# ecker-lab/TreeLearn

Hardware: AMD Instinct MI355X
Metric: Mpoints/sec through sparse U-Net fwd (0.1 m voxel, 40x40 m tile) (higher is better)
Workload: dtype bf16; 1 GPU; config2: single 40x40 m tile, voxel 0.1 m, 1890607 points/tile, 7-level 32-ch sparse U-Net fwd (30.1 M params, random init), 1 tile per GPU; points_per_tile=1890607, tiles_in_flight=4

## Files before the change

### include/treelearn_hip.h

```cpp
#ifndef TREELEARN_HIP_H
#define TREELEARN_HIP_H

#include <stdint.h>

#ifdef __cplusplus
extern "C" {
#endif

typedef void* tl_stream_t;

enum {
  TL_OK = 0,
  TL_ERR_ARG = -1,
  TL_ERR_LAUNCH = -2,
  TL_ERR_UNSUPPORTED = -3
};

enum { TL_F32 = 0, TL_BF16 = 1, TL_F16 = 2 };

int tl_version(void);
int tl_set_tuning(const char* key, int64_t value);
const char* tl_error_string(int code);


// ... 48 lines not shown
  int32_t* inv_packed;
} tl_level;

int tl_rulebooks_build(const tl_level* levels, int num_levels, int32_t* minus_one, int64_t minus_one_words,
                       const int32_t* pcoords, int64_t N, int64_t* v2p, tl_stream_t stream);

#define TL_BLK_HALO_MAX 126
typedef struct tl_blk {
  int32_t* o2n; int32_t* perm; int32_t* coords_new;
  int32_t* unit; int32_t* counter; int32_t* halo; uint32_t* lrb; int32_t* pmask;
  int64_t cap_units;
  int32_t halo_max;
  int32_t reserved;
  int32_t* nn;
} tl_blk;
int64_t tl_blk_ws_words(const int32_t dims[4]);
int tl_blk_build(const uint64_t* bitmap, const uint32_t* prefix, const int32_t dims[4], int64_t n, const tl_blk* out, uint32_t* ws,
                 int phases, tl_stream_t stream);

int tl_rulebook_compact(const int32_t* table, int64_t n, int32_t* compact, tl_stream_t stream);

typedef struct tl_conv_args {
  const void* in;        int64_t in_ld;
  const void* weight;
  const int32_t* table;
  int64_t n_out;         int64_t n_in;
  int32_t K;             int32_t Cin;     int32_t Cout;   int32_t dtype;
  const float* in_scale; const float* in_shift;  int32_t in_relu;  int32_t out_relu;
  const void* residual;  int64_t res_ld;
  const float* out_scale; const float* out_shift;
  void* out;             int64_t out_ld;
  void* out2; int64_t out2_ld; const float* out2_scale; const float* out2_shift; int32_t out2_relu;
  void* out3; int64_t out3_ld; const float* out3_scale; const float* out3_shift; int32_t out3_relu;
  const void* weight_frag;
  int32_t table_one_hot;
  const int32_t* table_compact;
  int32_t in_all_ones;
  int32_t epi_mode;
  double* red_part;
  int32_t* red_nparts;
  const void* bn_x;      int64_t bn_x_ld;
  const float* bn_mean;  const float* bn_rstd;  const float* bn_scale;  const float* bn_shift;  int32_t bn_relu;
  const int32_t* blk_unit; const int32_t* blk_counter; const int32_t* blk_halo; const uint32_t* blk_lrb; const int32_t* blk_pmask;
  const int32_t* table_scatter;
  const void* weight_x3;
} tl_conv_args;

#define TL_EPI_NONE 0
#define TL_EPI_STATS 1
#define TL_EPI_BN_BWD 2
int64_t tl_conv_red_parts(int64_t n_out);

int tl_conv_fwd(const tl_conv_args* args, tl_stream_t stream);

int tl_pack_weight(const float* w_ref, int Cout, int K, int Cin, void* w_packed, int dtype, tl_stream_t stream);
int64_t tl_pack_weight_x3_bytes(int Cout, int K, int Cin);
int tl_pack_weight_x3(const float* w_ref, int Cout, int K, int Cin, void* w_x3, tl_stream_t stream);
int tl_pack_weight_dgrad(const float* w_ref, int Cout, int K, int Cin, int flip, void* w_t, int dtype, tl_stream_t stream);
typedef struct tl_pack_desc {
  const float* src;
  void* dst;
  int32_t Cout, K, Cin, form;
} tl_pack_desc;
int tl_pack_weights_batch(const tl_pack_desc* descs, const int32_t* blocks, int64_t n_blocks, int dtype, tl_stream_t stream);
int tl_pack_weight_frag(const float* w_ref, int Cout, int K, int Cin, void* w_frag, int dtype, tl_stream_t stream);

int64_t tl_conv_wgrad_ws_floats(int64_t n_out, int K, int Cin, int Cout);
int tl_conv_wgrad(const void* x, int64_t x_ld, const void* gout, int64_t g_ld, int dtype, const int32_t* table, int64_t n_out,
                  int64_t n_in, int K, int Cin, int Cout, float* gw, float* ws, tl_stream_t stream);
int tl_conv_wgrad_ref(const void* x, int64_t x_ld, const void* gout, int64_t g_ld, int dtype, const int32_t* table, int64_t n_out,
                      int64_t n_in, int K, int Cin, int Cout, float* gw, float* ws, tl_stream_t stream);

int64_t tl_conv_wgrad_blk_ws_floats(void);
int tl_conv_wgrad_blk(const void* x, int64_t x_ld, const void* gout, int64_t g_ld, int dtype, const int32_t* blk_unit, const int32_t* blk_counter,
                      const int32_t* blk_halo, const uint32_t* blk_lrb, int64_t n, int Cin, int Cout, float* gw, int ref_layout, float* ws,
                      tl_stream_t stream);

int tl_head_mlp(const void* feats, int64_t feats_ld, int dtype, int C, const int64_t* v2p, int64_t N,
                const float* pro_scale, const float* pro_shift,
                const float* w1, const float* b1, const float* w2, const float* b2,
                float* backbone, float* logits, float* offsets, tl_stream_t stream);

int tl_affine_relu(const void* in, int64_t in_ld, void* out, int64_t out_ld, int64_t n, int C, int dtype,
                   const float* scale, const float* shift, int relu, tl_stream_t stream);

int64_t tl_bn_ws_doubles(int64_t n, int C);
int tl_bn_train_stats(const void* x, int64_t ld, int64_t n, int C, int dtype, const float* gamma, const float* beta, float eps,
                      float momentum, double* ws, float* mean, float* rstd, float* scale, float* shift, float* running_mean,
                      float* running_var, int64_t* num_batches_tracked, tl_stream_t stream);
int tl_bn_train_bwd(const void* x, int64_t ld, int x_dtype, const void* dy, int64_t dld, int dy_dtype, int64_t n, int C,
                    const float* mean, const float* rstd, const float* scale, const float* shift, int relu, double* ws,
                    float* dgamma, float* dbeta, void* dx, int64_t xld, const void* dx_add, int64_t dx_add_ld, tl_stream_t stream);

int tl_bn_train_finish(const double* part, int64_t nparts, int64_t n, int C, const float* gamma, const float* beta, float eps, float momentum, float* mean,
                       float* rstd, float* scale, float* shift, float* running_mean, float* running_var, int64_t* num_batches_tracked, tl_stream_t stream);
int tl_bn_train_bwd_from_parts(const void* x, int64_t ld, int x_dtype, const void* g, int64_t gld, int g_dtype, int64_t n, int C, const float* mean,
                               const float* rstd, const float* scale, const float* shift, const double* part, int64_t nparts, float* dgamma, float* dbeta,
                               void* dx, int64_t xld, const void* dx_add, int64_t dx_add_ld, tl_stream_t stream);

int tl_linear_small_f32(const void* x, int64_t x_ld, int dtype, const void* w, int Cin, int Cout, int64_t n, float* out, int64_t out_ld,
                        tl_stream_t stream);

int tl_gather_rows(const void* in, int64_t in_ld, int dtype, int C, int64_t n_rows, const int64_t* idx, int64_t N, void* out, int64_t out_ld, tl_stream_t stream);
int tl_scatter_add_rows(const void* g, int64_t g_ld, int dtype, int C, const int64_t* order, const int64_t* sorted_idx, int64_t N, int64_t n_rows, void* gin,
                        int64_t gin_ld, tl_stream_t stream);

// ... 159 lines not shown
```

### treelearn_amd/_hip.py

```python
import ctypes
import os

import torch

_HERE = os.path.dirname(os.path.abspath(__file__))
LIB_PATH = os.path.join(_HERE, "lib", "libtreelearn_hip.so")

TL_F32, TL_BF16, TL_F16 = 0, 1, 2
TL_OK, TL_ERR_ARG, TL_ERR_UNSUPPORTED = 0, -1, -3
TL_EPI_NONE, TL_EPI_STATS, TL_EPI_BN_BWD = 0, 1, 2
_c = ctypes
_vp, _i64, _i32, _f32 = _c.c_void_p, _c.c_int64, _c.c_int32, _c.c_float


class ConvArgs(_c.Structure):
    _fields_ = [
        ("in_", _vp), ("in_ld", _i64), ("weight", _vp), ("table", _vp),
        ("n_out", _i64), ("n_in", _i64), ("K", _i32), ("Cin", _i32), ("Cout", _i32), ("dtype", _i32),
        ("in_scale", _vp), ("in_shift", _vp), ("in_relu", _i32), ("out_relu", _i32),
        ("residual", _vp), ("res_ld", _i64), ("out_scale", _vp), ("out_shift", _vp),
        ("out", _vp), ("out_ld", _i64),
        ("out2", _vp), ("out2_ld", _i64), ("out2_scale", _vp), ("out2_shift", _vp), ("out2_relu", _i32),
        ("out3", _vp), ("out3_ld", _i64), ("out3_scale", _vp), ("out3_shift", _vp), ("out3_relu", _i32),
        ("weight_frag", _vp), ("table_one_hot", _i32), ("table_compact", _vp),
        ("in_all_ones", _i32), ("epi_mode", _i32), ("red_part", _vp), ("red_nparts", _c.POINTER(_i32)),
        ("bn_x", _vp), ("bn_x_ld", _i64), ("bn_mean", _vp), ("bn_rstd", _vp), ("bn_scale", _vp), ("bn_shift", _vp), ("bn_relu", _i32),
        ("blk_unit", _vp), ("blk_counter", _vp), ("blk_halo", _vp), ("blk_lrb", _vp), ("blk_pmask", _vp), ("table_scatter", _vp),
        ("weight_x3", _vp),
    ]


class TileBox(_c.Structure):
    _fields_ = [("outer", _c.c_float * 4), ("inner", _c.c_double * 4), ("center", _c.c_double * 2), ("half_inner", _c.c_float)]


class Level(_c.Structure):
    _fields_ = [("dims", _c.c_int32 * 4), ("n", _c.c_int64), ("bitmap", _c.c_void_p), ("prefix", _c.c_void_p), ("coords", _c.c_void_p),
                ("nbr", _c.c_void_p), ("compact", _c.c_void_p), ("child", _c.c_void_p), ("parent", _c.c_void_p), ("inv", _c.c_void_p),
                ("o2n", _c.c_void_p), ("inv_packed", _c.c_void_p)]


class Blk(_c.Structure):
    _fields_ = [("o2n", _vp), ("perm", _vp), ("coords_new", _vp), ("unit", _vp), ("counter", _vp), ("halo", _vp), ("lrb", _vp), ("pmask", _vp),
                ("cap_units", _i64), ("halo_max", _i32), ("reserved", _i32), ("nn", _vp)]


class HdbGrid(_c.Structure):
    _fields_ = [("lo", _c.c_double * 2), ("h", _c.c_double), ("levels", _c.c_int32), ("reserved", _c.c_int32)]


TL_MAX_LEVELS = 8
TL_ERR_ARENA, TL_ERR_REACH_ZERO, TL_ERR_EXTENT, TL_ERR_BLK = -4, -5, -6, -7


class Affine(_c.Structure):
    _fields_ = [("scale", _vp), ("shift", _vp)]


class Weight(_c.Structure):
    _fields_ = [("w", _vp), ("frag", _vp), ("K", _i32), ("Cout", _i32), ("Cin", _i32), ("reserved", _i32), ("x3", _vp)]


class ResDesc(_c.Structure):
    _fields_ = [("bn0", Affine), ("w1", Weight), ("bn3", Affine), ("w2", Weight), ("w1x1", Weight), ("w1_half", Weight * 2)]


class UBlockDesc(_c.Structure):
    _fields_ = [("C", _i32), ("deeper", _i32), ("blocks", ResDesc * 2), ("bn_down", Affine), ("wd", Weight), ("bn_up", Affine), ("wu", Weight),
                ("tail", ResDesc * 2), ("bn_cat_l", Affine), ("bn_cat_r", Affine)]


class NetDesc(_c.Structure):
    _fields_ = [("dtype", _i32), ("num_levels", _i32), ("voxel_size", _f32), ("has_shape", _i32), ("spatial_shape", _i32 * 3), ("blocked", _i32),
                ("in_channels", _i32), ("use_coords", _i32), ("use_feats", _i32), ("max_points_per_voxel", _i32), ("reserved0", _i32),
                ("w_in", Weight), ("u", UBlockDesc * TL_MAX_LEVELS), ("out_bn", Affine),
                ("head_w1", _vp), ("head_b1", _vp), ("head_w2", _vp), ("head_b2", _vp)]


class LaunchRec(_c.Structure):
    _fields_ = [("level", _i32), ("kind", _i32), ("K", _i32), ("Cin", _i32), ("Cout", _i32), ("residual", _i32), ("esize", _i32), ("split_part", _i32),
                ("split_cin", _i32), ("in_prologue", _i32), ("n_out", _i64), ("n_in", _i64), ("ms", _f32)]


class ForwardArgs(_c.Structure):
    _fields_ = [("xyz", _vp), ("batch_ids", _vp), ("N", _i64), ("B", _i32), ("reserved", _i32), ("point_feats", _vp), ("arena", _vp), ("arena_bytes", _i64),
                ("backbone", _vp), ("logits", _vp), ("offsets", _vp), ("side_stream", _vp), ("needed_bytes", _i64),
                ("level_n", _i64 * TL_MAX_LEVELS), ("blocked_used", _i32), ("launches", _i32)]


_I4 = _i32 * 4
_I3 = _i32 * 3

PROTOTYPES = {
    "tl_version": (_i32, []),
    "tl_error_string": (_c.c_char_p, [_i32]),
    "tl_set_tuning": (_i32, [_c.c_char_p, _i64]),
    "tl_voxel_point_coords": (_i32, [_vp, _vp, _i64, _i32, _f32, _vp, _vp, _vp, _vp]),
    "tl_voxel_point_coords_one": (_i32, [_vp, _vp, _i64, _f32, _vp, _vp, _vp, _c.POINTER(_i32), _vp]),
    "tl_bitmap_from_points": (_i32, [_vp, _i64, _I4, _vp, _vp]),
    "tl_bitmap_down": (_i32, [_vp, _I4, _I3, _vp, _I4, _vp]),
    "tl_scan_ws_words": (_i64, [_i64]),
    "tl_bitmap_scan": (_i32, [_vp, _i64, _vp, _vp, _vp, _vp]),
    "tl_expand_coords": (_i32, [_vp, _vp, _I4, _vp, _vp]),
    "tl_point_rank": (_i32, [_vp, _i64, _vp, _vp, _I4, _vp, _vp]),
    "tl_voxel_mean_feats": (_i32, [_vp, _i32, _vp, _i64, _i64, _i32, _vp, _vp, _vp]),
    "tl_voxel_feats": (_i32, [_vp, _vp, _i32, _vp, _i64, _i64, _i32, _i32, _i32, _i32, _vp, _vp, _vp]),
    "tl_rulebook_subm": (_i32, [_vp, _i64, _vp, _vp, _I4, _vp, _vp, _vp]),
    "tl_rulebook_down": (_i32, [_vp, _i64, _vp, _vp, _I4, _i64, _vp, _vp, _vp, _vp]),
    "tl_rulebook_compact": (_i32, [_vp, _i64, _vp, _vp]),
    "tl_pyramid_ws_words": (_i64, [_I4, _i32, _c.POINTER(_i64)]),
    "tl_pyramid_build": (_i32, [_vp, _i64, _I4, _I3, _i32, _vp, _vp, _vp, _vp, _vp]),
    "tl_rulebooks_build": (_i32, [_c.POINTER(Level), _i32, _vp, _i64, _vp, _i64, _vp, _vp]),
    "tl_blk_ws_words": (_i64, [_I4]),
    "tl_blk_build": (_i32, [_vp, _vp, _I4, _i64, _c.POINTER(Blk), _vp, _i32, _vp]),
    "tl_conv_fwd": (_i32, [_c.POINTER(ConvArgs), _vp]),
    "tl_conv_red_parts": (_i64, [_i64]),
    "tl_exec_create": (_vp, []),
    "tl_exec_destroy": (None, [_vp]),
    "tl_forward": (_i32, [_vp, _c.POINTER(NetDesc), _c.POINTER(ForwardArgs), _vp]),
    "tl_exec_check": (_i32, [_vp]),
    "tl_exec_profile": (_i32, [_vp, _i32]),
    "tl_exec_profile_read": (_i32, [_vp, _c.POINTER(LaunchRec), _i32]),
    "tl_bn_train_finish": (_i32, [_vp, _i64, _i64, _i32, _vp, _vp, _f32, _f32, _vp, _vp, _vp, _vp, _vp, _vp, _vp, _vp]),
    "tl_bn_train_bwd_from_parts": (_i32, [_vp, _i64, _i32, _vp, _i64, _i32, _i64, _i32, _vp, _vp, _vp, _vp, _vp, _i64, _vp, _vp, _vp, _i64, _vp, _i64, _vp]),
    "tl_pack_weight": (_i32, [_vp, _i32, _i32, _i32, _vp, _i32, _vp]),
    "tl_pack_weight_x3": (_i32, [_vp, _i32, _i32, _i32, _vp, _vp]),
    "tl_pack_weight_x3_bytes": (_i64, [_i32, _i32, _i32]),
    "tl_pack_weight_frag": (_i32, [_vp, _i32, _i32, _i32, _vp, _i32, _vp]),
    "tl_pack_weights_batch": (_i32, [_vp, _vp, _i64, _i32, _vp]),
    "tl_pack_weight_dgrad": (_i32, [_vp, _i32, _i32, _i32, _i32, _vp, _i32, _vp]),
    "tl_conv_wgrad_ws_floats": (_i64, [_i64, _i32, _i32, _i32]),
    "tl_conv_wgrad": (_i32, [_vp, _i64, _vp, _i64, _i32, _vp, _i64, _i64, _i32, _i32, _i32, _vp, _vp, _vp]),
    "tl_conv_wgrad_ref": (_i32, [_vp, _i64, _vp, _i64, _i32, _vp, _i64, _i64, _i32, _i32, _i32, _vp, _vp, _vp]),
    "tl_conv_wgrad_blk_ws_floats": (_i64, []),
    "tl_conv_wgrad_blk": (_i32, [_vp, _i64, _vp, _i64, _i32, _vp, _vp, _vp, _vp, _i64, _i32, _i32, _vp, _i32, _vp, _vp]),
    "tl_head_mlp": (_i32, [_vp, _i64, _i32, _i32, _vp, _i64, _vp, _vp, _vp, _vp, _vp, _vp, _vp, _vp, _vp, _vp]),
    "tl_affine_relu": (_i32, [_vp, _i64, _vp, _i64, _i64, _i32, _i32, _vp, _vp, _i32, _vp]),
    "tl_bn_ws_doubles": (_i64, [_i64, _i32]),
    "tl_bn_train_stats": (_i32, [_vp, _i64, _i64, _i32, _i32, _vp, _vp, _f32, _f32, _vp, _vp, _vp, _vp, _vp, _vp, _vp, _vp, _vp]),
    "tl_bn_train_bwd": (_i32, [_vp, _i64, _i32, _vp, _i64, _i32, _i64, _i32, _vp, _vp, _vp, _vp, _i32, _vp, _vp, _vp, _vp, _i64, _vp, _i64, _vp]),
    "tl_linear_small_f32": (_i32, [_vp, _i64, _i32, _vp, _i32, _i32, _i64, _vp, _i64, _vp]),
    "tl_gather_rows": (_i32, [_vp, _i64, _i32, _i32, _i64, _vp, _i64, _vp, _i64, _vp]),
    "tl_scatter_add_rows": (_i32, [_vp, _i64, _i32, _i32, _vp, _vp, _i64, _i64, _vp, _i64, _vp]),
    "tl_compact_ws_words": (_i64, [_i64]),
    "tl_compact_rows": (_i32, [_vp, _i32, _vp, _i64, _vp, _vp, _vp, _vp]),
    "tl_tile_crop_ws_words": (_i64, [_i64]),
    "tl_tile_crop": (_i32, [_vp, _vp, _vp, _i64, _i32, _vp, _vp, _vp, _vp, _vp, _vp, _vp, _vp, _vp, _vp]),
    "tl_cell_keys": (_i32, [_vp, _i64, _c.c_double, _c.c_double, _vp, _i32, _vp, _vp, _vp]),
    "tl_downsample_ws_words": (_i64, [_i64]),
    "tl_downsample_reduce": (_i32, [_vp, _vp, _vp, _i64, _vp, _vp, _vp, _vp, _vp, _vp]),
    "tl_downsample_reduce_r64": (_i32, [_vp, _vp, _vp, _i64, _vp, _vp, _vp, _vp, _vp, _vp]),
    "tl_group_mean": (_i32, [_vp, _i64, _i32, _vp, _vp, _vp, _vp, _vp, _vp, _vp]),
    "tl_verticality": (_i32, [_vp, _vp, _i64, _c.c_double, _vp, _vp, _vp]),
    "tl_cluster_ws_bytes": (_i64, [_i64]),
    "tl_cluster_grid": (_i32, [_vp, _i64, _c.c_double, _vp, _vp, _vp, _vp]),
    "tl_hdbscan_ws_bytes": (_i64, [_i64]),
    "tl_hdbscan_mst": (_i32, [_vp, _i64, _i32, _vp, _vp, _vp, _vp, _vp, _vp]),
    "tl_hdbscan_labels_host": (_i32, [_vp, _vp, _vp, _i64, _i32, _vp]),
    "tl_hdbscan_prim_order_host": (_i32, [_vp, _vp, _vp, _i64, _vp, _vp, _vp]),
    "tl_hdbscan_grid_plan_ws_bytes": (_i64, []),
    "tl_hdbscan_grid_plan": (_i32, [_vp, _i64, _vp, _vp, _vp]),
    "tl_hdbscan_grid_ws_bytes": (_i64, [_i64, _vp]),
    "tl_hdbscan_grid_ws_bytes_k": (_i64, [_i64, _vp, _i32]),
    "tl_hdbscan_mst_grid": (_i32, [_vp, _i64, _i32, _vp, _vp, _vp, _vp, _vp, _vp, _vp]),
    "tl_knn_vote": (_i32, [_vp, _vp, _i64, _vp, _i64, _i32, _vp, _vp]),
    "tl_knn_vote_grid": (_i32, [_vp, _vp, _vp, _i64, _vp, _vp, _i64, _c.c_float * 3, _f32, _I3, _vp, _i64, _i32, _vp, _vp]),
    "tl_eval_contingency": (_i32, [_vp, _vp, _i64, _i64, _i64, _i64, _vp, _vp]),
    "tl_eval_partition": (_i32, [_vp, _vp, _vp, _i64, _vp, _vp, _i64, _vp, _vp, _i64, _vp, _i64, _vp, _i32, _i32, _vp, _vp, _vp, _vp, _vp]),
# ... 81 lines not shown
```

### treelearn_amd/csrc/tl_common.h

```cpp
#pragma once
#include <hip/hip_runtime.h>
#include <stdint.h>
#include <atomic>
#include "../../include/treelearn_hip.h"

#define TL_CHECK_LAUNCH()                                   \
  do {                                                      \
    if (hipGetLastError() != hipSuccess) return TL_ERR_LAUNCH; \
  } while (0)

static inline hipStream_t tl_s(tl_stream_t s) { return reinterpret_cast<hipStream_t>(s); }

struct TlAttrOnce {
  std::atomic<uint64_t> done[4];
};
static inline bool tl_lds_attr(TlAttrOnce& once, const void* kernel, int bytes) {
  int dev = 0;
  if (hipGetDevice(&dev) != hipSuccess) return false;
  std::atomic<uint64_t>& w = once.done[(dev >> 6) & 3];
  const uint64_t bit = 1ull << (dev & 63);
  if (w.load(std::memory_order_acquire) & bit) return true;
  if (hipFuncSetAttribute(kernel, hipFuncAttributeMaxDynamicSharedMemorySize, bytes) != hipSuccess) return false;
  w.fetch_or(bit, std::memory_order_release);
  return true;
}

static inline int64_t tl_cdiv(int64_t a, int64_t b) { return (a + b - 1) / b; }

static inline unsigned tl_grid(int64_t work_items, int block) {
  int64_t g = tl_cdiv(work_items, block);
  if (g < 1) g = 1;
  if (g > 256 * 16) g = 256 * 16;
  return (unsigned)g;
}

struct TlDims {
  int B, X, Y, Z, Zw;
};
static inline TlDims tl_dims(const int32_t d[4]) {
  TlDims r{d[0], d[1], d[2], d[3], (d[3] + 63) >> 6};
  return r;
}
__host__ __device__ static inline int64_t tl_nwords(const TlDims& d) { return (int64_t)d.B * d.X * d.Y * d.Zw; }

__device__ __forceinline__ int64_t tl_col_word(const TlDims& d, int b, int x, int y) {
  return (((int64_t)b * d.X + x) * d.Y + y) * d.Zw;
}

__device__ __forceinline__ int tl_rank_at(const uint64_t* __restrict__ bm, const uint32_t* __restrict__ pf,
                                          int64_t wc, int z) {
  const int64_t w = wc + (z >> 6);
  const uint64_t word = bm[w];
  const uint64_t bit = 1ull << (z & 63);
  if (!(word & bit)) return -1;
  return (int)(pf[w] + __popcll(word & (bit - 1)));
}

bool tl_conv_one_hot_direct_enabled(int64_t n_out);
```

### treelearn_amd/csrc/tl_conv.hip

```cpp
#include "tl_conv_internal.h"
#include <atomic>
#include <string.h>

namespace {

template <typename T>
__global__ void __launch_bounds__(256) k_conv_generic(ConvP p) {
  const T* in = (const T*)p.in; const T* w = (const T*)p.w; const T* res = (const T*)p.res;
  const int64_t total = p.n_out * p.Cout;
  for (int64_t t = (int64_t)blockIdx.x * blockDim.x + threadIdx.x; t < total; t += (int64_t)gridDim.x * blockDim.x) {
    const int64_t o = t / p.Cout; const int j = (int)(t % p.Cout);
    float acc = 0.f;
    for (int k = 0; k < p.K; ++k) {
      const int64_t idx = p.table ? (int64_t)p.table[(int64_t)k * p.n_out + o] : o;
      if (idx < 0) continue;
      const T* x = in + idx * p.in_ld;
      const T* wr = w + ((int64_t)k * p.Cout + j) * p.Cin;
      for (int c = 0; c < p.Cin; ++c) {
        float v = ld_elem(x + c);
        if (p.in_scale) v = fmaf(v, p.in_scale[c], p.in_shift[c]);
        if (p.in_relu) v = fmaxf(v, 0.f);
        if (sizeof(T) == 2) v = __bfloat162float(__float2bfloat16(v));
        acc = fmaf(v, ld_elem(wr + c), acc);
      }
// ... 93 lines not shown
    while (true) {
      int nk = k, nch = ch + 1;
      unsigned nmask = mask;
      if (nch == nchunk) { nch = 0; nmask = mask & (mask - 1); nk = nmask ? __builtin_ctz(nmask) : -1; }
      const bool more = nk >= 0;
      if (more) issue(nk, nch);

      const float* a = As + buf * TM * LDA + (wv * 32 + fi) * LDA + fh * 4;
      float4 af[4];
#pragma unroll
      for (int j = 0; j < 4; ++j) af[j] = *reinterpret_cast<const float4*>(a + 8 * j);
#pragma unroll
      for (int nb = 0; nb < NB; ++nb) {
        const float* b = Bs + buf * NB * 32 * LDA + (nb * 32 + fi) * LDA + fh * 4;
        float4 bf[4];
#pragma unroll
        for (int j = 0; j < 4; ++j) bf[j] = *reinterpret_cast<const float4*>(b + 8 * j);
#pragma unroll
        for (int j = 0; j < 4; ++j) {
          acc[nb] = __builtin_amdgcn_mfma_f32_32x32x2f32(af[j].x, bf[j].x, acc[nb], 0, 0, 0);
          acc[nb] = __builtin_amdgcn_mfma_f32_32x32x2f32(af[j].y, bf[j].y, acc[nb], 0, 0, 0);
          acc[nb] = __builtin_amdgcn_mfma_f32_32x32x2f32(af[j].z, bf[j].z, acc[nb], 0, 0, 0);
          acc[nb] = __builtin_amdgcn_mfma_f32_32x32x2f32(af[j].w, bf[j].w, acc[nb], 0, 0, 0);
        }
      }
      if (!more) break;
      stage(buf ^ 1, nch);
      __syncthreads();
      buf ^= 1; k = nk; ch = nch; mask = nmask;
    }
  }

  const float* res = (const float*)p.res;
  const int col = lane & 31;
#pragma unroll
  for (int nb = 0; nb < NB; ++nb) {
    const int j = nb * 32 + col;
#pragma unroll
    for (int r = 0; r < 16; ++r) {
      const int64_t row = r0 + wv * 32 + (r & 3) + 8 * (r >> 2) + 4 * (lane >> 5);
      if (row >= p.n_out) continue;
      float v = acc[nb][r];
      if (res) v += res[row * p.res_ld + j];
      epi_store1<false>(p.out, p.out_ld, p.out_scale, p.out_shift, p.out_relu, row, j, v);
      if (p.out2) epi_store1<false>(p.out2, p.out2_ld, p.out2_scale, p.out2_shift, p.out2_relu, row, j, v);
      if (p.out3) epi_store1<false>(p.out3, p.out3_ld, p.out3_scale, p.out3_shift, p.out3_relu, row, j, v);
    }
  }
}

template <int NB>
int launch_mfma_f32(const ConvP& p, hipStream_t s) {
  const size_t lds = (size_t)p.K * TM * 4 + 16 + 2 * (size_t)TM * LDA * 4 + 2 * (size_t)NB * 32 * LDA * 4;
  static TlAttrOnce attr_once;
  if (!tl_lds_attr(attr_once, reinterpret_cast<const void*>(&k_conv_mfma_f32<NB>), 160 * 1024)) return TL_ERR_LAUNCH;
  k_conv_mfma_f32<NB><<<p.nblk, 256, lds, s>>>(p);
  return hipGetLastError() == hipSuccess ? TL_OK : TL_ERR_LAUNCH;
}

__global__ void k_pack_weight(const float* __restrict__ w, int Cout, int K, int Cin, void* __restrict__ o, int dtype) {
  const int64_t total = (int64_t)Cout * K * Cin;
  for (int64_t t = (int64_t)blockIdx.x * blockDim.x + threadIdx.x; t < total; t += (int64_t)gridDim.x * blockDim.x) {
    const int c = (int)(t % Cin); const int64_t r = t / Cin; const int j = (int)(r % Cout); const int k = (int)(r / Cout);
    const float v = w[((int64_t)j * K + k) * Cin + c];
    if (dtype == TL_F32) reinterpret_cast<float*>(o)[t] = v;
    else if (dtype == TL_F16) reinterpret_cast<_Float16*>(o)[t] = (_Float16)v;
    else reinterpret_cast<__hip_bfloat16*>(o)[t] = __float2bfloat16(v);
  }
}

__global__ void k_pack_weight_x3(const float* __restrict__ w, int Cout, int K, int Cin, uint16_t* __restrict__ o) {
  const int un_all = Cin / 32, halves = Cin >= 256 ? 2 : 1, un = un_all / halves;
  const int64_t per_half = (int64_t)Cout * K * un * 64, total = per_half * halves;
  for (int64_t t0 = (int64_t)blockIdx.x * blockDim.x + threadIdx.x; t0 < total; t0 += (int64_t)gridDim.x * blockDim.x) {
    const int hf = (int)(t0 / per_half); const int64_t t = t0 - hf * per_half;
    const int e = (int)(t & 63); const int64_t r = t >> 6; const int c = (int)(r % un); const int64_t r2 = r / un;
    const int n = (int)(r2 % Cout); const int k = (int)(r2 / Cout);
    const int half = e >> 5, piece = (e & 31) >> 3, q = e & 7, J = piece >> 1, fh = piece & 1;
    const int ch = 32 * (c + hf * un) + 16 * J + (q < 4 ? 4 * fh + q : 8 + 4 * fh + (q - 4));
    const float v = w[((int64_t)n * K + k) * Cin + ch];
    const __hip_bfloat16 hi = __float2bfloat16(v);
    const __hip_bfloat16 lo = __float2bfloat16(v - __bfloat162float(hi));
    o[t0] = half ? __builtin_bit_cast(uint16_t, lo) : __builtin_bit_cast(uint16_t, hi);
    if (halves == 1 && Cout % 32 == 0) {
      const int j = half ? 2 + J : J;
      const int lane = (n & 31) + 32 * fh, cbt = n >> 5, CBt = Cout >> 5;
      o[total + ((((((int64_t)k * CBt + cbt) * un + c) * 4 + j) * 64 + lane) * 8) + q] = half ? __builtin_bit_cast(uint16_t, lo) : __builtin_bit_cast(uint16_t, hi);
    }
  }
}

__global__ void k_pack_weight_dgrad(const float* __restrict__ w, int Cout, int K, int Cin, int flip, void* __restrict__ o, int dtype) {
  const int64_t total = (int64_t)Cout * K * Cin;
  for (int64_t t = (int64_t)blockIdx.x * blockDim.x + threadIdx.x; t < total; t += (int64_t)gridDim.x * blockDim.x) {
    const int co = (int)(t % Cout); const int64_t r = t / Cout; const int ci = (int)(r % Cin); const int k = (int)(r / Cin);
    const float v = w[((int64_t)co * K + (flip ? K - 1 - k : k)) * Cin + ci];
    if (dtype == TL_F32) reinterpret_cast<float*>(o)[t] = v;
    else if (dtype == TL_F16) reinterpret_cast<_Float16*>(o)[t] = (_Float16)v;
    else reinterpret_cast<__hip_bfloat16*>(o)[t] = __float2bfloat16(v);
  }
}

__global__ void k_pack_weight_frag(const float* __restrict__ w, int Cout, int K, int Cin, void* __restrict__ o, int dtype) {
  const int EB = dtype == TL_F32 ? 4 : 2, J = 32 * EB / 32, EPV = 16 / EB;
  const int CB = Cout / 32, CH = Cin / 32;
  const int64_t nvec = (int64_t)K * CB * CH * J * 64;
// ... 68 lines not shown
    float x[8];
    typedef _Float16 hx2 __attribute__((ext_vector_type(2)));
    if constexpr (T16 == 1) {
      const u32x4 q4 = __builtin_nontemporal_load(reinterpret_cast<const u32x4*>((const uint16_t*)in + r * in_ld + c0));
#pragma unroll
      for (int q = 0; q < 4; ++q) { x[2 * q] = bf16_lo(q4[q]); x[2 * q + 1] = bf16_hi(q4[q]); }
    } else if constexpr (T16 == 2) {
      const u32x4 q4 = *reinterpret_cast<const u32x4*>((const uint16_t*)in + r * in_ld + c0);
      const uint32_t w0 = q4[0], w1 = q4[1], w2 = q4[2], w3 = q4[3];
      const uint32_t ws[4] = {w0, w1, w2, w3};
#pragma unroll
      for (int q = 0; q < 4; ++q) { const hx2 h = __builtin_bit_cast(hx2, ws[q]); x[2 * q] = (float)h[0]; x[2 * q + 1] = (float)h[1]; }
    } else {
      const f32x4* s4 = reinterpret_cast<const f32x4*>((const float*)in + r * in_ld + c0);
      const f32x4 a = __builtin_nontemporal_load(s4), b = __builtin_nontemporal_load(s4 + 1);
#pragma unroll
      for (int q = 0; q < 4; ++q) { x[q] = a[q]; x[q + 4] = b[q]; }
    }
#pragma unroll
    for (int q = 0; q < 8; ++q) { x[q] = fmaf(x[q], sc[q], sh[q]); if (relu) x[q] = fmaxf(x[q], 0.f); }
    if constexpr (T16 == 1) {
      u32x4 o;
#pragma unroll
      for (int q = 0; q < 4; ++q) o[q] = pack_bf16x2(x[2 * q], x[2 * q + 1]);
      *reinterpret_cast<u32x4*>((uint16_t*)out + r * out_ld + c0) = o;
    } else if constexpr (T16 == 2) {
      u32x4 o;
#pragma unroll
      for (int q = 0; q < 4; ++q) { const hx2 h = {(_Float16)x[2 * q], (_Float16)x[2 * q + 1]}; o[q] = __builtin_bit_cast(uint32_t, h); }
      *reinterpret_cast<u32x4*>((uint16_t*)out + r * out_ld + c0) = o;
    } else {
      f32x4* d = reinterpret_cast<f32x4*>((float*)out + r * out_ld + c0);
      d[0] = f32x4{x[0], x[1], x[2], x[3]}; d[1] = f32x4{x[4], x[5], x[6], x[7]};
    }
  }
}

}

static int64_t g_small_rows = kSmallRows;
extern int g_small_mode;
extern int g_wgrad_dense;
extern int64_t g_wgrad_dense_min_rows;
extern int g_wgrad_rows;
extern int g_wgrad_dma;
static int g_stream = 1;
static int g_streamq = 1;
static int g_streamq_x3 = 1;
static int g_direct = 1;
static int g_direct_oh = 1;
static int g_blk = 1;
static int g_up = 1;

bool tl_conv_one_hot_direct_enabled(int64_t n_out) { return g_direct && g_direct_oh && n_out > g_small_rows; }

extern "C" {

int tl_set_tuning(const char* key, int64_t value) {
  if (!key) return TL_ERR_ARG;
  if (!strcmp(key, "direct")) { g_direct = (int)value; return TL_OK; }
  if (!strcmp(key, "blk")) { g_blk = (int)value; return TL_OK; }
  if (!strcmp(key, "up")) { g_up = (int)value; return TL_OK; }
  if (!strcmp(key, "direct_oh")) { g_direct_oh = (int)value; return TL_OK; }
  if (!strcmp(key, "stream")) { g_stream = (int)value; return TL_OK; }
  if (!strcmp(key, "streamq")) { g_streamq = (int)value; return TL_OK; }
  if (!strcmp(key, "streamq_x3")) { if (value != 0 && value != 1) return TL_ERR_ARG; g_streamq_x3 = (int)value; return TL_OK; }
  if (!strcmp(key, "small_rows")) { g_small_rows = value; return TL_OK; }
  if (!strcmp(key, "small_mode")) { g_small_mode = (int)value; return TL_OK; }
  if (!strcmp(key, "wgrad_dense")) { g_wgrad_dense = (int)value; return TL_OK; }
  if (!strcmp(key, "wgrad_rows")) { g_wgrad_rows = (int)value; return TL_OK; }
  if (!strcmp(key, "wgrad_dma")) { g_wgrad_dma = (int)value; return TL_OK; }
  if (!strcmp(key, "wgrad_dense_min_rows")) { g_wgrad_dense_min_rows = value; return TL_OK; }
  return TL_ERR_ARG;
}

int tl_conv_fwd(const tl_conv_args* a, tl_stream_t stream) {
  if (!a || !a->in || !a->weight || !a->out || a->n_out <= 0 || a->K <= 0 || a->K > 27 || a->Cin <= 0 || a->Cout <= 0) return TL_ERR_ARG;
  const bool has_blk = a->blk_unit && a->blk_counter && a->blk_halo && a->blk_lrb && a->K == 27;
  if (!a->table && a->K != 1 && !has_blk && !(a->in_all_ones && a->blk_pmask)) return TL_ERR_ARG;
  if ((a->in_scale == nullptr) != (a->in_shift == nullptr)) return TL_ERR_ARG;
  if ((a->out_scale == nullptr) != (a->out_shift == nullptr)) return TL_ERR_ARG;
  if (a->dtype != TL_F32 && a->dtype != TL_BF16 && a->dtype != TL_F16) return TL_ERR_ARG;
  const bool f16 = a->dtype == TL_F16;
  const int dt = f16 ? TL_BF16 : a->dtype;
  const auto L_direct = f16 ? tl_launch_conv_direct_f16 : tl_launch_conv_direct;
  const auto L_ones27 = f16 ? tl_launch_conv_ones27_f16 : tl_launch_conv_ones27;
  const auto L_stream = f16 ? tl_launch_conv_stream_f16 : tl_launch_conv_stream;
  const auto L_streamq = f16 ? tl_launch_conv_streamq_f16 : tl_launch_conv_streamq;
  const auto L_small = f16 ? tl_launch_conv_small_f16 : tl_launch_conv_small;
  const auto L_tinycin = f16 ? tl_launch_conv_tinycin_f16 : tl_launch_conv_tinycin;
  const auto L_blk = f16 ? tl_launch_conv_blk_f16 : tl_launch_conv_blk;
  const auto L_up = f16 ? tl_launch_conv_up_f16 : tl_launch_conv_up;
  ConvP p;
  p.in = a->in; p.in_ld = a->in_ld; p.w = a->weight; p.w_frag = a->weight_frag;
  p.w_x3 = (a->dtype == TL_F32 && a->Cin % 32 == 0 && ((uintptr_t)a->weight_x3) % 16 == 0) ? a->weight_x3 : nullptr; p.table = a->table; p.ctab = (a->K == 27) ? a->table_compact : nullptr; p.n_out = a->n_out; p.n_in = a->n_in;
  p.K = a->K; p.Cin = a->Cin; p.Cout = a->Cout; p.in_scale = a->in_scale; p.in_shift = a->in_shift;
  p.in_relu = a->in_relu; p.out_relu = a->out_relu; p.res = a->residual; p.res_ld = a->res_ld;
  p.out_scale = a->out_scale; p.out_shift = a->out_shift; p.out = a->out; p.out_ld = a->out_ld;
  p.out2 = a->out2; p.out2_ld = a->out2_ld; p.out2_scale = a->out2_scale; p.out2_shift = a->out2_shift; p.out2_relu = a->out2_relu;
  p.out3 = a->out3; p.out3_ld = a->out3_ld; p.out3_scale = a->out3_scale; p.out3_shift = a->out3_shift; p.out3_relu = a->out3_relu;
  if ((a->out2_scale == nullptr) != (a->out2_shift == nullptr) || (a->out3_scale == nullptr) != (a->out3_shift == nullptr)) return TL_ERR_ARG;
  p.nblk = (int)tl_cdiv(a->n_out, TM);
  p.one_hot = a->table != nullptr ? a->table_one_hot : 0;
  p.blk_unit = has_blk ? a->blk_unit : nullptr; p.blk_counter = a->blk_counter; p.blk_halo = a->blk_halo; p.blk_lrb = a->blk_lrb;
  p.blk_pmask = a->K == 27 ? a->blk_pmask : nullptr;
  p.epi_mode = a->epi_mode; p.red_part = a->red_part; p.red_nparts = a->red_nparts; p.bn_x = a->bn_x; p.bn_x_ld = a->bn_x_ld;
  p.bn_mean = a->bn_mean; p.bn_rstd = a->bn_rstd; p.bn_scale = a->bn_scale; p.bn_shift = a->bn_shift; p.bn_relu = a->bn_relu;
  const bool train = a->epi_mode != TL_EPI_NONE;
  if (train) {
    if ((a->epi_mode != TL_EPI_STATS && a->epi_mode != TL_EPI_BN_BWD) || !a->red_part || ((uintptr_t)a->red_part) % 8) return TL_ERR_ARG;
    if (a->epi_mode == TL_EPI_BN_BWD) {
      if (!a->bn_x || !a->bn_mean || !a->bn_rstd || !a->bn_scale || !a->bn_shift) return TL_ERR_ARG;
      if (a->bn_x_ld % 8 || ((uintptr_t)a->bn_x) % 16 || ((uintptr_t)a->bn_mean) % 16 || ((uintptr_t)a->bn_rstd) % 16 || ((uintptr_t)a->bn_scale) % 16 ||
          ((uintptr_t)a->bn_shift) % 16)
        return TL_ERR_UNSUPPORTED;
    }
    if (a->red_nparts) *a->red_nparts = 0;
  }
  hipStream_t s = tl_s(stream);
  if (p.one_hot == 2) {
    const bool shape = a->K == 8 && a->Cin == 64 && a->Cout == 32 && !train && !a->in_scale && !a->in_relu && g_direct && g_direct_oh;
    if (!shape || !(dt == TL_BF16 || (dt == TL_F32 && p.w_x3))) return TL_ERR_UNSUPPORTED;
    return L_direct(p, dt, s);
  }
  const bool vec_ok = (a->in_ld % 8 == 0) && (((uintptr_t)a->in) % 16 == 0) && (((uintptr_t)a->weight) % 16 == 0);
  const bool out_vec = (a->out_ld % 8 == 0) && (((uintptr_t)a->out) % 16 == 0) &&
                       (!a->out2 || (a->out2_ld % 8 == 0 && ((uintptr_t)a->out2) % 16 == 0)) && (!a->out3 || (a->out3_ld % 8 == 0 && ((uintptr_t)a->out3) % 16 == 0));
  if (a->in_all_ones && !train && (dt == TL_BF16 || (dt == TL_F32 && !f16)) && out_vec && (g_direct || !a->table) && ((uintptr_t)a->weight) % 4 == 0 && !a->residual) {
    const int rc = L_ones27(p, dt, s);
    if (rc != TL_ERR_UNSUPPORTED) return rc;
  }
  if (has_blk && dt == TL_BF16 && g_blk && vec_ok && out_vec && (!a->residual || (a->res_ld % 8 == 0 && ((uintptr_t)a->residual) % 16 == 0)) &&
      (!a->out_scale || (((uintptr_t)a->out_scale) % 4 == 0 && ((uintptr_t)a->out_shift) % 4 == 0)) && (!a->in_relu || a->in_scale)) {
    const int rc = L_blk(p, s);
    if (rc != TL_ERR_UNSUPPORTED) return rc;
  }
  if (has_blk && a->dtype == TL_F32 && p.w_x3 && g_blk && !train) {
    const int rc = tl_launch_conv_blk_x3(p, s);
    if (rc != TL_ERR_UNSUPPORTED) return rc;
  }
  if (!a->table && a->K != 1) return TL_ERR_UNSUPPORTED;
  if (a->table_scatter && p.one_hot && g_up && !train && dt == TL_BF16 && vec_ok && out_vec &&
      (!a->out_scale || (((uintptr_t)a->out_scale) % 16 == 0 && ((uintptr_t)a->out_shift) % 16 == 0))) {
    const int rc = L_up(p, a->table_scatter, s);
    if (rc != TL_ERR_UNSUPPORTED) return rc;
  }
  if (dt == TL_BF16 && a->Cin == 4 && a->Cout == 32 && g_direct && out_vec && ((uintptr_t)a->in) % 8 == 0 && ((uintptr_t)a->weight) % 16 == 0 &&
      (!a->residual || (a->res_ld % 8 == 0 && ((uintptr_t)a->residual) % 16 == 0))) {
    const int rc = L_direct(p, TL_BF16, s);
    if (rc != TL_ERR_UNSUPPORTED) return rc;
  }
  if (!train && a->Cin <= 8 && a->Cout % 8 == 0 && a->Cout <= 64 && !a->in_scale && !a->in_relu && out_vec) return L_tinycin(p, dt, s);
  if (!train && vec_ok && a->n_out <= g_small_rows && a->Cin % 32 == 0 && a->Cout % 32 == 0) return L_small(p, dt, s);
  if (train && a->n_out <= g_small_rows) return TL_ERR_UNSUPPORTED;
  const bool aligned = (a->in_ld % 4 == 0) && (((uintptr_t)a->in) % 16 == 0) && (((uintptr_t)a->weight) % 16 == 0) &&
                       (!a->in_scale || (((uintptr_t)a->in_scale) % 16 == 0 && ((uintptr_t)a->in_shift) % 16 == 0));
  if (p.w_x3 && a->Cin >= 256) {
    if (dt == TL_F32 && !train && g_stream && aligned && out_vec && a->Cin % 64 == 0 && a->Cout % 32 == 0 && !a->in_scale && !a->in_relu && !a->residual &&
        !a->out2 && !a->out3 && a->n_out > g_small_rows && (!a->out_scale || (((uintptr_t)a->out_scale) % 16 == 0 && ((uintptr_t)a->out_shift) % 16 == 0))) {
      ConvP p1 = p;
      p1.Cin = a->Cin / 2; p1.out_scale = nullptr; p1.out_shift = nullptr; p1.out_relu = 0;
      const int rc1 = L_stream(p1, TL_F32, s);
      if (rc1 == TL_OK) {
        ConvP p2 = p;
        p2.Cin = a->Cin / 2; p2.in = static_cast<const float*>(a->in) + a->Cin / 2;
        p2.w_x3 = static_cast<const char*>(p.w_x3) + (size_t)a->K * a->Cout * (a->Cin / 2) * 4;
        p2.res = a->out; p2.res_ld = a->out_ld;
        return L_stream(p2, TL_F32, s);
      }
      if (rc1 != TL_ERR_UNSUPPORTED) return rc1;
    }
    p.w_x3 = nullptr;
  }
  if (dt == TL_F32 && aligned && out_vec && a->Cin % 32 == 0 && a->Cout % 32 == 0 && !a->in_scale && !a->in_relu &&
      (!a->residual || (a->res_ld % 4 == 0 && ((uintptr_t)a->residual) % 16 == 0)) &&
      (!a->out_scale || (((uintptr_t)a->out_scale) % 16 == 0 && ((uintptr_t)a->out_shift) % 16 == 0))) {
    if (g_direct) { const int rc = L_direct(p, TL_F32, s); if (rc != TL_ERR_UNSUPPORTED) return rc; }
    if (g_stream && g_streamq && g_streamq_x3 && p.w_x3 && !train && a->n_out > g_small_rows) {
      const int rc = tl_launch_conv_streamq_x3(p, s);
      if (rc != TL_ERR_UNSUPPORTED) return rc;
    }
    if (g_stream) { const int rc = L_stream(p, TL_F32, s); if (rc != TL_ERR_UNSUPPORTED) return rc; }
  }
  if (train && dt == TL_F32) return TL_ERR_UNSUPPORTED;
  if (dt == TL_F32 && !f16 && vec_ok && a->n_out <= 4 * g_small_rows && a->Cin % 32 == 0 && a->Cout % 32 == 0 && !a->in_scale && !a->in_relu)
    return L_small(p, dt, s);
  if (dt == TL_F32 && aligned && a->Cin % KC == 0 && a->Cout % 32 == 0 && a->Cout <= 224) {
    switch (a->Cout / 32) {
      case 1: return launch_mfma_f32<1>(p, s);
      case 2: return launch_mfma_f32<2>(p, s);
      case 3: return launch_mfma_f32<3>(p, s);
      case 4: return launch_mfma_f32<4>(p, s);
      case 5: return launch_mfma_f32<5>(p, s);
      case 6: return launch_mfma_f32<6>(p, s);
      case 7: return launch_mfma_f32<7>(p, s);
    }
  }
  if (dt == TL_BF16 && aligned && vec_ok && out_vec && a->Cin % 32 == 0 && a->Cout % 32 == 0 && a->Cout <= 224 &&
      (!a->residual || (a->res_ld % 8 == 0 && ((uintptr_t)a->residual) % 16 == 0)) &&
      (!a->out_scale || (((uintptr_t)a->out_scale) % 16 == 0 && ((uintptr_t)a->out_shift) % 16 == 0)))
  {
    if (p.one_hot && g_direct && g_direct_oh && a->K == 8 && a->Cin == 64 && a->Cout == 32) {
      const int rc = L_direct(p, TL_BF16, s);
      if (rc != TL_ERR_UNSUPPORTED) return rc;
    }
    if (p.one_hot && g_stream && a->K == 8) {
      const int rc = L_stream(p, TL_BF16, s);
      if (rc != TL_ERR_UNSUPPORTED) return rc;
    }
    if (g_direct) {
      const int rc = L_direct(p, TL_BF16, s);
      if (rc != TL_ERR_UNSUPPORTED) return rc;
    }
    if (g_stream && g_streamq) {
      const int rc = L_streamq(p, s);
      if (rc != TL_ERR_UNSUPPORTED) return rc;
    }
    if (g_stream) {
      const int rc = L_stream(p, TL_BF16, s);
      if (rc != TL_ERR_UNSUPPORTED) return rc;
    }
    if (train) return TL_ERR_UNSUPPORTED;
    return f16 ? tl_launch_conv_bf16_f16(p, s) : tl_launch_conv_bf16(p, s);
  }
  if (train || f16) return TL_ERR_UNSUPPORTED;
  {
    const int rc = tl_launch_conv_tinycout(p, dt, s);
    if (rc != TL_ERR_UNSUPPORTED) return rc;
  }
  const unsigned g = tl_grid(a->n_out * a->Cout, 256);
  if (dt == TL_F32) k_conv_generic<float><<<g, 256, 0, s>>>(p);
  else k_conv_generic<__hip_bfloat16><<<g, 256, 0, s>>>(p);
  TL_CHECK_LAUNCH();
  return TL_OK;
}

int64_t tl_conv_red_parts(int64_t n_out) {
  const int64_t a = tl_cdiv(n_out > 0 ? n_out : 1, 256);
  return a > 2048 ? a : 2048;
}

int tl_pack_weight(const float* w_ref, int Cout, int K, int Cin, void* w_packed, int dtype, tl_stream_t stream) {
  if (!w_ref || !w_packed || Cout <= 0 || K <= 0 || Cin <= 0 || (dtype != TL_F32 && dtype != TL_BF16 && dtype != TL_F16)) return TL_ERR_ARG;
  k_pack_weight<<<tl_grid((int64_t)Cout * K * Cin, 256), 256, 0, tl_s(stream)>>>(w_ref, Cout, K, Cin, w_packed, dtype);
  TL_CHECK_LAUNCH();
  return TL_OK;
}

int64_t tl_pack_weight_x3_bytes(int Cout, int K, int Cin) {
  if (Cout <= 0 || K <= 0 || Cin <= 0 || Cin % 32) return -1;
  const int64_t one = (int64_t)K * Cout * Cin * 4;
  return (Cin < 256 && Cout % 32 == 0) ? 2 * one : one;
}

int tl_pack_weight_x3(const float* w_ref, int Cout, int K, int Cin, void* w_x3, tl_stream_t stream) {
  if (!w_ref || !w_x3 || Cout <= 0 || K <= 0 || Cin <= 0 || Cin % 32) return TL_ERR_ARG;
  k_pack_weight_x3<<<tl_grid((int64_t)Cout * K * Cin * 2, 256), 256, 0, tl_s(stream)>>>(w_ref, Cout, K, Cin, reinterpret_cast<uint16_t*>(w_x3));
  TL_CHECK_LAUNCH();
  return TL_OK;
}

int tl_pack_weight_dgrad(const float* w_ref, int Cout, int K, int Cin, int flip, void* w_t, int dtype, tl_stream_t stream) {
  if (!w_ref || !w_t || Cout <= 0 || K <= 0 || Cin <= 0 || (dtype != TL_F32 && dtype != TL_BF16 && dtype != TL_F16)) return TL_ERR_ARG;
  k_pack_weight_dgrad<<<tl_grid((int64_t)Cout * K * Cin, 256), 256, 0, tl_s(stream)>>>(w_ref, Cout, K, Cin, flip, w_t, dtype);
  TL_CHECK_LAUNCH();
  return TL_OK;
}

int tl_pack_weights_batch(const tl_pack_desc* descs, const int32_t* blocks, int64_t n_blocks, int dtype, tl_stream_t stream) {
  if (!descs || !blocks || n_blocks <= 0 || n_blocks > 0x7FFFFFFF || (dtype != TL_F32 && dtype != TL_BF16 && dtype != TL_F16)) return TL_ERR_ARG;
  k_pack_batch<<<(unsigned)n_blocks, 256, 0, tl_s(stream)>>>(descs, reinterpret_cast<const int2*>(blocks), dtype);
  TL_CHECK_LAUNCH();
  return TL_OK;
}

int tl_pack_weight_frag(const float* w_ref, int Cout, int K, int Cin, void* w_frag, int dtype, tl_stream_t stream) {
  if (!w_ref || !w_frag || Cout <= 0 || K <= 0 || Cin <= 0 || Cout % 32 || Cin % 32 || (dtype != TL_F32 && dtype != TL_BF16 && dtype != TL_F16)) return TL_ERR_ARG;
  k_pack_weight_frag<<<tl_grid((int64_t)Cout * K * Cin / 8, 256), 256, 0, tl_s(stream)>>>(w_ref, Cout, K, Cin, w_frag, dtype);
  TL_CHECK_LAUNCH();
  return TL_OK;
}

int tl_affine_relu(const void* in, int64_t in_ld, void* out, int64_t out_ld, int64_t n, int C, int dtype, const float* scale,
                   const float* shift, int relu, tl_stream_t stream) {
  if (!in || !out || n <= 0 || C <= 0 || (scale == nullptr) != (shift == nullptr)) return TL_ERR_ARG;
  if ((dtype == TL_F32 || dtype == TL_BF16 || dtype == TL_F16) && C % 8 == 0 && in_ld % 8 == 0 && out_ld % 8 == 0 && ((uintptr_t)in) % 16 == 0 && ((uintptr_t)out) % 16 == 0) {
    const int vpr = C / 8;
// ... 20 lines not shown
```

### treelearn_amd/csrc/tl_conv_bf16.hip

```cpp
#include "tl_conv_internal.h"
#include <atomic>

namespace {

constexpr int TM = 128;

template <int NB, int U, int D, bool BUF>
__global__ void __launch_bounds__(256) k_conv_bf16(ConvP p) {
  constexpr int KCB = 32 * U;
  constexpr int PITCH = KCB * 2 + 16;
  constexpr int VPR = KCB / 8;
  constexpr int RPP = 256 / VPR;
  constexpr int APASS = TM / RPP;
  constexpr int BROWS = NB * 32;
  constexpr int BPASS = (BROWS + RPP - 1) / RPP;
  constexpr int EP = NB * 32 + 4;

  extern __shared__ __attribute__((aligned(16))) char smem[];
  int* idx_s = reinterpret_cast<int*>(smem);
  int* taps_s = idx_s + p.K * TM;
  float* scale_s = reinterpret_cast<float*>(taps_s + 32);
  float* shift_s = scale_s + p.Cin;
  char* As = reinterpret_cast<char*>(shift_s + p.Cin);
  char* Bs = As + 2 * TM * PITCH;
// ... 154 lines not shown
#pragma unroll
    for (int d = 0; d < D; ++d) {
      stage(buf, ra[d], rb[d], vmask[d], chs[d]);
      __syncthreads();
      issue(ra[d], rb[d], vmask[d], chs[d]);
      compute(buf);
      buf ^= 1;
    }
  }
  const int rem = nsteps - s;
#pragma unroll
  for (int d = 0; d < D - 1; ++d) {
    if (d < rem) {
      stage(buf, ra[d], rb[d], vmask[d], chs[d]);
      __syncthreads();
      compute(buf);
      buf ^= 1;
    }
  }

  __syncthreads();
  float* ew = Es + wv * 32 * EP;
#pragma unroll
  for (int nb = 0; nb < NB; ++nb)
#pragma unroll
    for (int r = 0; r < 16; ++r) ew[((r & 3) + 8 * (r >> 2) + 4 * fh) * EP + nb * 32 + fi] = acc[nb][r];
  __syncthreads();
  constexpr int VROW = NB * 4;
  const char* res = (const char*)p.res;
  for (int e = lane; e < 32 * VROW; e += 64) {
    const int rr = e / VROW, cvv = e % VROW;
    const int64_t row = r0 + wv * 32 + rr;
    if (row >= p.n_out) continue;
    const f32x4 v0 = *reinterpret_cast<const f32x4*>(ew + rr * EP + cvv * 8), v1 = *reinterpret_cast<const f32x4*>(ew + rr * EP + cvv * 8 + 4);
    float v[8] = {v0[0], v0[1], v0[2], v0[3], v1[0], v1[1], v1[2], v1[3]};
    if (res) {
      const u32x4 rv = *reinterpret_cast<const u32x4*>(res + (row * p.res_ld + cvv * 8) * 2);
#pragma unroll
      for (int q = 0; q < 4; ++q) { v[2 * q] += bf16_lo(rv[q]); v[2 * q + 1] += bf16_hi(rv[q]); }
    }
    epi_store8<true>(p.out, p.out_ld, p.out_scale, p.out_shift, p.out_relu, row, cvv * 8, v);
    if (p.out2) epi_store8<true>(p.out2, p.out2_ld, p.out2_scale, p.out2_shift, p.out2_relu, row, cvv * 8, v);
    if (p.out3) epi_store8<true>(p.out3, p.out3_ld, p.out3_scale, p.out3_shift, p.out3_relu, row, cvv * 8, v);
  }
}

template <int NB, int U, int D, bool BUF>
int launch_b(const ConvP& p, hipStream_t s) {
  constexpr int PITCH = 32 * U * 2 + 16;
  const size_t main_b = 2 * (size_t)TM * PITCH + 2 * (size_t)NB * 32 * PITCH;
  const size_t epi_b = 4 * (size_t)32 * (NB * 32 + 4) * 4;
  const size_t lds = (size_t)p.K * TM * 4 + 128 + (size_t)p.Cin * 8 + (main_b > epi_b ? main_b : epi_b);
  if (lds > 160 * 1024) return TL_ERR_UNSUPPORTED;
  static TlAttrOnce attr_once;
  if (!tl_lds_attr(attr_once, reinterpret_cast<const void*>(&k_conv_bf16<NB, U, D, BUF>), 160 * 1024)) return TL_ERR_LAUNCH;
  k_conv_bf16<NB, U, D, BUF><<<p.nblk, 256, lds, s>>>(p);
  return hipGetLastError() == hipSuccess ? TL_OK : TL_ERR_LAUNCH;
}

template <int NB, int U, int D>
int launch(const ConvP& p, hipStream_t s) {
  const int64_t ld_b = p.in_ld * 2, in_bytes = (p.n_in - 1) * ld_b + (int64_t)p.Cin * 2;
  const bool buf = in_bytes > 0 && in_bytes + 2 * ld_b < 0xFFFFFFFFll;
  return buf ? launch_b<NB, U, D, true>(p, s) : launch_b<NB, U, D, false>(p, s);
}

}

int tl_launch_conv_bf16(const ConvP& p, hipStream_t s) {
  switch (p.Cout / 32) {
    case 1: return launch<1, 2, 2>(p, s);
    case 2: return launch<2, 2, 2>(p, s);
    case 3: return launch<3, 2, 2>(p, s);
    case 4: return launch<4, 2, 2>(p, s);
    case 5: return launch<5, 2, 2>(p, s);
    case 6: return launch<6, 2, 2>(p, s);
    case 7: return launch<7, 2, 2>(p, s);
  }
  return TL_ERR_UNSUPPORTED;
}
```

### treelearn_amd/csrc/tl_conv_blk.hip

```cpp
#include "tl_conv_internal.h"
#include <atomic>

namespace {

typedef __attribute__((address_space(3))) void* lds_ptr;
static __device__ __forceinline__ u32x4 lds_r128(unsigned a) { u32x4 v; asm volatile("ds_read_b128 %0, %1" : "=v"(v) : "v"(a)); return v; }
#define TL_LGKM(N) asm volatile("s_waitcnt lgkmcnt(%0)" ::"n"(N) : "memory")
#define TL_KEEP(x) asm volatile("" : "+v"(x))
typedef int i32x4 __attribute__((ext_vector_type(4)));
static __device__ __forceinline__ i32x4 s_load4(const void* ptr) { i32x4 v; asm volatile("s_load_dwordx4 %0, %1, 0x0" : "=s"(v) : "s"(ptr)); return v; }
#define TL_SWAIT(d) asm volatile("s_waitcnt lgkmcnt(0)" : "+s"(d) : : "memory")

constexpr int WS_B = 27 * 32 * 64;
constexpr int AFF_B = 4 * 2 * 32 * 4;
constexpr int STAGE_B = 192 * 64;
constexpr int HCH = 8;
struct RbRow { u32x4 a, b; uint32_t c; };
static __device__ __forceinline__ uint32_t rb_word(const RbRow& r, int w) { return w < 4 ? r.a[w] : (w < 8 ? r.b[w - 4] : r.c); }

typedef float f32x2 __attribute__((ext_vector_type(2)));
typedef short s16x2 __attribute__((ext_vector_type(2)));

template <int W, bool RES, int NV, bool TR = false, bool PRO = false>
__global__ void __launch_bounds__(W * 64) k_conv_blk(ConvP p) {
// ... 318 lines not shown
        for (int q = 0; q < 4; ++q) {
          sc[q] = __uint_as_float(s0[q]); sc[q + 4] = __uint_as_float(s1[q]);
          sh[q] = __uint_as_float(h0[q]); sh[q + 4] = __uint_as_float(h1[q]);
        }
      }
#pragma unroll
      for (int it = 0; it < 4; ++it) {
        float z[8];
#pragma unroll
        for (int q = 0; q < 8; ++q) z[q] = y[it][q];
        if (aff_on[v]) {
#pragma unroll
          for (int q = 0; q < 8; ++q) z[q] = fmaf(z[q], sc[q], sh[q]);
        }
        if (relu_on[v]) {
#pragma unroll
          for (int q = 0; q < 8; ++q) z[q] = fmaxf(z[q], 0.f);
        }
        const u32x4 o = {pack_bf16x2(z[0], z[1]), pack_bf16x2(z[2], z[3]), pack_bf16x2(z[4], z[5]), pack_bf16x2(z[6], z[7])};
        const int rr_ = (lane >> 2) + 16 * it;
        const unsigned off = rr_ < nown ? (unsigned)(row0 + rr_) * o_ldb[v] + (unsigned)((lane & 3) * 16) : 0xFFFFFFFFu;
        __builtin_amdgcn_raw_buffer_store_b128(__builtin_bit_cast(__attribute__((__vector_size__(4 * sizeof(unsigned)))) unsigned, o), ro[v], (int)off, 0, 0);
      }
    }
    }
    dc = d1; d1 = d2; d2 = desc_fin(d3r, u + 3 * nw);
  }
  if constexpr (TR) {
    double* Ds = reinterpret_cast<double*>(smem + WS_B + AFF_B + W * STAGE_B);
    double d0[8], d1_[8];
#pragma unroll
    for (int q = 0; q < 8; ++q) { d0[q] = (double)ts0[q]; d1_[q] = (double)ts1[q]; }
#pragma unroll
    for (int off = 4; off < 64; off <<= 1)
#pragma unroll
      for (int q = 0; q < 8; ++q) { d0[q] += __shfl_xor(d0[q], off, 64); d1_[q] += __shfl_xor(d1_[q], off, 64); }
    if (lane < 4) {
#pragma unroll
      for (int q = 0; q < 8; ++q) { Ds[(wv * 2 + 0) * 32 + lane * 8 + q] = d0[q]; Ds[(wv * 2 + 1) * 32 + lane * 8 + q] = d1_[q]; }
    }
    __syncthreads();
    if (tid < 64) {
      double t = 0.0;
      for (int w = 0; w < W; ++w) t += Ds[(w * 2 + (tid >> 5)) * 32 + (tid & 31)];
      p.red_part[(int64_t)blockIdx.x * 64 + tid] = t;
    }
  }
}

template <int W, bool RES, int NV, bool TR = false, bool PRO = false>
int launch_blk(const ConvP& p, hipStream_t s) {
  constexpr size_t lds = (size_t)WS_B + AFF_B + (size_t)W * STAGE_B + (TR ? (size_t)W * 2 * 32 * 8 : 0);
  static_assert(lds <= 160 * 1024, "LDS budget");
  static TlAttrOnce attr_once;
  if (!tl_lds_attr(attr_once, reinterpret_cast<const void*>(&k_conv_blk<W, RES, NV, TR, PRO>), 160 * 1024)) return TL_ERR_LAUNCH;
  k_conv_blk<W, RES, NV, TR, PRO><<<256, W * 64, lds, s>>>(p);
  if (TR && p.red_nparts) *p.red_nparts = 256;
  return hipGetLastError() == hipSuccess ? TL_OK : TL_ERR_LAUNCH;
}

}

int tl_launch_conv_blk(const ConvP& p, hipStream_t s) {
  if (!p.blk_unit || !p.blk_counter || !p.blk_halo || !p.blk_lrb) return TL_ERR_UNSUPPORTED;
  if (p.K != 27 || p.Cin != 32 || p.Cout != 32 || p.n_in != p.n_out) return TL_ERR_UNSUPPORTED;
  const bool pro = p.in_scale || p.in_relu;
  if (p.n_out >= (1 << 25)) return TL_ERR_UNSUPPORTED;
  auto big = [&](int64_t ld) { return (p.n_out - 1) * ld * 2 + 64 >= 0x7FFFFFFFll * 2; };
  if (big(p.in_ld) || big(p.out_ld) || (p.out2 && big(p.out2_ld)) || (p.out3 && big(p.out3_ld)) || (p.res && big(p.res_ld))) return TL_ERR_UNSUPPORTED;
  if (p.out3 && !p.out2) return TL_ERR_UNSUPPORTED;
  if (p.epi_mode != TL_EPI_NONE) {
    if (p.out2 || p.out_scale || p.out_relu || p.out_ld % 8 || ((uintptr_t)p.out) % 16) return TL_ERR_UNSUPPORTED;
    if (pro && p.epi_mode != TL_EPI_STATS) return TL_ERR_UNSUPPORTED;
    return pro ? launch_blk<8, false, 1, true, true>(p, s) : launch_blk<8, false, 1, true>(p, s);
  }
  const int nv = p.out3 ? 3 : p.out2 ? 2 : 1;
  if (pro) {
    if (nv != 1) return TL_ERR_UNSUPPORTED;
    return p.res ? launch_blk<8, true, 1, false, true>(p, s) : launch_blk<8, false, 1, false, true>(p, s);
  }
  if (p.res) {
    switch (nv) {
      case 1: return launch_blk<8, true, 1>(p, s);
      case 2: return launch_blk<8, true, 2>(p, s);
      default: return launch_blk<8, true, 3>(p, s);
    }
  }
  switch (nv) {
    case 1: return launch_blk<8, false, 1>(p, s);
    case 2: return launch_blk<8, false, 2>(p, s);
    default: return launch_blk<8, false, 3>(p, s);
  }
}
```

### treelearn_amd/csrc/tl_conv_blk_x3.hip

```cpp
#include "tl_conv_internal.h"
#include <atomic>

namespace {

typedef __attribute__((address_space(3))) void* lds_ptr;
static __device__ __forceinline__ u32x4 lds_r128(unsigned a) { u32x4 v; asm volatile("ds_read_b128 %0, %1" : "=v"(v) : "v"(a)); return v; }
#define TL_LGKM(N) asm volatile("s_waitcnt lgkmcnt(%0)" ::"n"(N) : "memory")
#define TL_KEEP(x) asm volatile("" : "+v"(x))
typedef int i32x4 __attribute__((ext_vector_type(4)));
typedef uint32_t u32x2 __attribute__((ext_vector_type(2)));
static __device__ __forceinline__ i32x4 s_load4(const void* ptr) { i32x4 v; asm volatile("s_load_dwordx4 %0, %1, 0x0" : "=s"(v) : "s"(ptr)); return v; }
#define TL_SWAIT(d) asm volatile("s_waitcnt lgkmcnt(0)" : "+s"(d) : : "memory")

constexpr int WS_B = 27 * 32 * 64;
constexpr int AFF_B = 4 * 2 * 32 * 4;
constexpr int STAGE_B = 192 * 64;
constexpr int HCH = 8;
struct RbRow { u32x4 a, b; uint32_t c; };
static __device__ __forceinline__ uint32_t rb_word(const RbRow& r, int w) { return w < 4 ? r.a[w] : (w < 8 ? r.b[w - 4] : r.c); }

struct X3P {
  int slice;
  int part;
  int chunk, nchunks;
// ... 264 lines not shown
    }
    if constexpr (RES) {
#pragma unroll
      for (int it = 0; it < 4; ++it) {
        TL_KEEP(rres[it][0]); TL_KEEP(rres[it][1]);
#pragma unroll
        for (int q = 0; q < 4; ++q) { y[it][q] += __uint_as_float(rres[it][0][q]); y[it][q + 4] += __uint_as_float(rres[it][1][q]); }
      }
    }
    stage_unit(d1, hcur);
#pragma unroll
    for (int v = 0; v < NV; ++v) {
      float sc[8], sh[8];
      if (aff_on[v]) {
        const u32x4 s0 = lds_r128(aff_a + (unsigned)(v * 256)), s1 = lds_r128(aff_a + (unsigned)(v * 256 + 16));
        const u32x4 h0 = lds_r128(aff_a + (unsigned)(v * 256 + 128)), h1 = lds_r128(aff_a + (unsigned)(v * 256 + 144));
        TL_LGKM(0);
#pragma unroll
        for (int q = 0; q < 4; ++q) {
          sc[q] = __uint_as_float(s0[q]); sc[q + 4] = __uint_as_float(s1[q]);
          sh[q] = __uint_as_float(h0[q]); sh[q + 4] = __uint_as_float(h1[q]);
        }
      }
#pragma unroll
      for (int it = 0; it < 4; ++it) {
        float z[8];
#pragma unroll
        for (int q = 0; q < 8; ++q) z[q] = y[it][q];
        if (aff_on[v]) {
#pragma unroll
          for (int q = 0; q < 8; ++q) z[q] = fmaf(z[q], sc[q], sh[q]);
        }
        if (relu_on[v]) {
#pragma unroll
          for (int q = 0; q < 8; ++q) z[q] = fmaxf(z[q], 0.f);
        }
        typedef __attribute__((__vector_size__(4 * sizeof(unsigned)))) unsigned uv4;
        const uv4 o0 = {__float_as_uint(z[0]), __float_as_uint(z[1]), __float_as_uint(z[2]), __float_as_uint(z[3])};
        const uv4 o1 = {__float_as_uint(z[4]), __float_as_uint(z[5]), __float_as_uint(z[6]), __float_as_uint(z[7])};
        const int rr_ = (lane >> 2) + 16 * it;
        const unsigned off = rr_ < nown ? (unsigned)(row0 + rr_) * o_ldb[v] + (unsigned)((lane & 3) * 32) : 0xFFFFFFFFu;
        __builtin_amdgcn_raw_buffer_store_b128(o0, ro[v], (int)off, 0, 0);
        __builtin_amdgcn_raw_buffer_store_b128(o1, ro[v], (int)(off == 0xFFFFFFFFu ? off : off + 16u), 0, 0);
      }
    }
    dc = d1; d1 = d2; d2 = desc_fin(d3r, u + 3 * nw);
  }
}

template <int W, bool RES, int NV>
int launch_x3(const ConvP& p, const X3P& xp, hipStream_t s) {
  constexpr size_t lds = (size_t)WS_B + AFF_B + (size_t)W * STAGE_B;
  static_assert(lds <= 160 * 1024, "LDS budget");
  static TlAttrOnce attr_once;
  if (!tl_lds_attr(attr_once, reinterpret_cast<const void*>(&k_conv_blk_x3<W, RES, NV>), 160 * 1024)) return TL_ERR_LAUNCH;
  k_conv_blk_x3<W, RES, NV><<<256, W * 64, lds, s>>>(p, xp);
  return hipGetLastError() == hipSuccess ? TL_OK : TL_ERR_LAUNCH;
}

}

int tl_launch_conv_blk_x3(const ConvP& p, hipStream_t s) {
  if (!p.blk_unit || !p.blk_counter || !p.blk_halo || !p.blk_lrb || !p.w_x3) return TL_ERR_UNSUPPORTED;
  if (p.K != 27 || p.Cin != 32 || p.Cout != 32 || p.n_in != p.n_out || p.epi_mode != TL_EPI_NONE || p.out3) return TL_ERR_UNSUPPORTED;
  if (p.n_out >= (1 << 25)) return TL_ERR_UNSUPPORTED;
  if (p.in_relu && !p.in_scale) return TL_ERR_UNSUPPORTED;
  auto big = [&](int64_t ld) { return (p.n_out - 1) * ld * 4 + 128 >= 0x7FFFFFFFll * 2; };
  if (big(p.in_ld) || big(p.out_ld) || (p.out2 && big(p.out2_ld)) || (p.res && big(p.res_ld))) return TL_ERR_UNSUPPORTED;
  auto al16 = [](const void* q, int64_t ld) { return ((uintptr_t)q) % 16 == 0 && ld % 4 == 0; };
  if (!al16(p.in, p.in_ld) || !al16(p.out, p.out_ld) || (p.out2 && !al16(p.out2, p.out2_ld)) || (p.res && !al16(p.res, p.res_ld)) || ((uintptr_t)p.w_x3) % 16) return TL_ERR_UNSUPPORTED;
  ConvP a = p;
  a.res = nullptr; a.res_ld = 0; a.out_scale = a.out_shift = nullptr; a.out_relu = 0; a.out2 = nullptr; a.out2_scale = a.out2_shift = nullptr; a.out2_relu = 0;
  ConvP b = p;
  b.in = static_cast<const float*>(p.in) + 16;
  if (p.in_scale) { b.in_scale = p.in_scale + 16; b.in_shift = p.in_shift + 16; }
  const int rc = launch_x3<8, false, 1>(a, X3P{0, 0, 0, 1}, s);
  if (rc != TL_OK) return rc;
  const X3P xb{1, 1, 0, 1};
  if (p.res) return p.out2 ? launch_x3<8, true, 2>(b, xb, s) : launch_x3<8, true, 1>(b, xb, s);
  return p.out2 ? launch_x3<8, false, 2>(b, xb, s) : launch_x3<8, false, 1>(b, xb, s);
}
```

### treelearn_amd/csrc/tl_conv_direct.hip

```cpp
#include "tl_conv_internal.h"
#include <atomic>

namespace {


template <bool BF16, int K, int NB, int UN, int G, int WAVES, bool CT = false, bool TR = false, bool OH = false, bool X3 = false>
__global__ void __launch_bounds__(WAVES * 64) k_conv_direct(ConvP p, int ntiles, int walk) {
  static_assert(!X3 || (!BF16 && !TR), "the split-bf16 contraction: fp32 rows, inference");
  constexpr int EB = BF16 ? 2 : 4;
  constexpr int UB = 32 * EB;
  constexpr int NJ = UB / 32;
  constexpr int SLOTS = UB / 16;
  constexpr int COUT = NB * 32;
  constexpr int NG = (K + G - 1) / G;
  constexpr int EP = COUT + 4;
  extern __shared__ __attribute__((aligned(16))) char smem[];
  char* Ws = smem;
  float* Es = reinterpret_cast<float*>(smem + (size_t)K * UN * COUT * UB);
  double* Ds = reinterpret_cast<double*>(smem + (size_t)K * UN * COUT * UB + (size_t)WAVES * 32 * EP * 4);

  const int tid = threadIdx.x, lane = tid & 63, wv = tid >> 6;
  const int fi = lane & 31, fh = lane >> 5;
  auto swz_of = [](int n) { return BF16 ? ((n >> 2) & 3) : ((n >> 1) & 7); };

// ... 362 lines not shown
      p.red_part[(int64_t)blockIdx.x * 64 + e] = t;
    }
  }
}

template <bool BF16>
__global__ void __launch_bounds__(256) k_conv_ones27(ConvP p) {
  __shared__ __attribute__((aligned(16))) float S[27][32];
  for (int e = threadIdx.x; e < 27 * 32; e += 256) {
    float t = 0.f;
    if constexpr (BF16) {
      const uint16_t* w = (const uint16_t*)p.w;
      for (int c = 0; c < p.Cin; ++c) t += bf16_lo((uint32_t)w[(int64_t)e * p.Cin + c]);
    } else {
      const float* w = (const float*)p.w;
      for (int c = 0; c < p.Cin; ++c) t += w[(int64_t)e * p.Cin + c];
    }
    S[e >> 5][e & 31] = t;
  }
  __syncthreads();
  const int32_t* mask = p.blk_pmask ? p.blk_pmask : p.ctab + (int64_t)9 * p.n_out;
  const int64_t total = p.n_out * 4;
  for (int64_t t = (int64_t)blockIdx.x * 256 + threadIdx.x; t < total; t += (int64_t)gridDim.x * 256) {
    const int64_t row = t >> 2; const int c0 = (int)(t & 3) * 8;
    uint32_t m = (uint32_t)mask[row];
    float v[8] = {0.f, 0.f, 0.f, 0.f, 0.f, 0.f, 0.f, 0.f};
    while (m) {
      const int k = __builtin_ctz(m); m &= m - 1;
      const f32x4 a = *reinterpret_cast<const f32x4*>(&S[k][c0]), b = *reinterpret_cast<const f32x4*>(&S[k][c0 + 4]);
#pragma unroll
      for (int q = 0; q < 4; ++q) { v[q] += a[q]; v[q + 4] += b[q]; }
    }
    epi_views8<BF16>(p, row, c0, v);
  }
}

template <bool BF16, int K, int NB, int UN, int G, int WAVES, bool CT = false, bool TR = false, bool OH = false, bool X3 = false>
int launch(const ConvP& p_, hipStream_t s) {
  ConvP p = p_;
  if constexpr (X3) {
    if (p.epi_mode != TL_EPI_NONE) return TL_ERR_UNSUPPORTED;
    p.w = p.w_x3;
  }
  if constexpr (!TR && BF16) {
    if (p.epi_mode != TL_EPI_NONE) return launch<BF16, K, NB, UN, G, WAVES, CT, true, OH>(p, s);
  } else if constexpr (!TR) {
    if (p.epi_mode != TL_EPI_NONE) return TL_ERR_UNSUPPORTED;
  }
  if constexpr (TR && NB >= 3) return TL_ERR_UNSUPPORTED;
  else {
  constexpr int UB = BF16 ? 64 : 128;
  const size_t lds = (size_t)K * UN * NB * 32 * UB + (size_t)WAVES * 32 * (NB * 32 + 4) * 4 + (TR ? (size_t)WAVES * 2 * NB * 32 * 8 : 0);
  if (lds > 160 * 1024) return TL_ERR_UNSUPPORTED;
  static TlAttrOnce attr_once;
  if (!tl_lds_attr(attr_once, reinterpret_cast<const void*>(&k_conv_direct<BF16, K, NB, UN, G, WAVES, CT, TR, OH, X3>), 160 * 1024)) return TL_ERR_LAUNCH;
  const int ntiles = (int)tl_cdiv(p.n_out, 32);
  const int per_cu = (int)((160 * 1024) / lds) < 1 ? 1 : (int)((160 * 1024) / lds);
  int grid = 256 * (per_cu > 2 ? 2 : per_cu);
  const int need = (int)tl_cdiv(ntiles, WAVES);
  if (grid > need) grid = need;
  k_conv_direct<BF16, K, NB, UN, G, WAVES, CT, TR, OH, X3><<<grid, WAVES * 64, lds, s>>>(p, ntiles, 0);
  if (p.red_nparts) *p.red_nparts = grid;
  return hipGetLastError() == hipSuccess ? TL_OK : TL_ERR_LAUNCH;
  }
}

template <bool BF16, int K, int G>
int dispatch(const ConvP& p, hipStream_t s) {
  const int nb = p.Cout / 32, un = p.Cin / 32;
  const size_t wbytes = (size_t)K * p.Cout * p.Cin * (BF16 ? 2 : 4);
  if constexpr (BF16 && K == 27) {
    if (p.ctab && nb == 1 && un == 1) return launch<true, 27, 1, 1, G, 16, true>(p, s);
    if (p.ctab && nb == 1 && un == 2) return launch<true, 27, 1, 2, G, 8, true>(p, s);
  }
  if constexpr (BF16 && K == 8) {
    if (p.one_hot && nb == 1 && un == 2) return launch<true, 8, 1, 2, G, 16, false, false, true>(p, s);
  }
  if constexpr (BF16 && K == 1) {
    if (nb == 2 && un == 4) return launch<true, 1, 2, 4, 1, 16>(p, s);
    if (nb == 3 && un == 6) return launch<true, 1, 3, 6, 1, 8>(p, s);
    if (nb == 4 && un == 8) return launch<true, 1, 4, 8, 1, 8>(p, s);
  }
  if constexpr (!BF16 && K == 1) {
    if (nb == 2 && un == 4 && p.epi_mode == TL_EPI_NONE) {
      if (p.w_x3) return launch<false, 1, 2, 4, 1, 8, false, false, false, true>(p, s);
      return launch<false, 1, 2, 4, 1, 8>(p, s);
    }
  }
  if constexpr (!BF16 && K == 8) {
    if (p.one_hot && p.w_x3 && p.epi_mode == TL_EPI_NONE && nb == 1 && un == 2) return launch<false, 8, 1, 2, G, 12, false, false, true, true>(p, s);
  }
#define TL_D(NB_, UN_)                                                                                               \
  if (nb == NB_ && un == UN_) {                                                                                      \
    if constexpr (BF16) return wbytes <= 64 * 1024 ? launch<true, K, NB_, UN_, G, 16>(p, s) : launch<true, K, NB_, UN_, G, 8>(p, s); \
    else {                                                                                                           \
      if (p.w_x3 && p.epi_mode == TL_EPI_NONE)        \
        return launch<false, K, NB_, UN_, (G > 2 ? 2 : G), (K == 27 && NB_ == 1 && UN_ == 1 ? 11 : 8), false, false, false, true>(p, s);         \
      return launch<false, K, NB_, UN_, (G > 2 ? 2 : G), 8>(p, s);                                                   \
    }                                                                                                                \
  }
  TL_D(1, 1) TL_D(1, 2) TL_D(2, 1) TL_D(2, 2) TL_D(2, 3) TL_D(3, 2) TL_D(1, 3) TL_D(3, 1)
#undef TL_D
  return TL_ERR_UNSUPPORTED;
}

}

int tl_launch_conv_ones27(const ConvP& p, int dtype, hipStream_t s) {
  if (p.K != 27 || p.Cout != 32 || (!p.ctab && !p.blk_pmask) || p.Cin <= 0 || p.Cin > 64 || p.in_scale || p.in_relu || p.epi_mode != TL_EPI_NONE) return TL_ERR_UNSUPPORTED;
  if (dtype == TL_BF16) k_conv_ones27<true><<<tl_grid(p.n_out * 4, 256), 256, 0, s>>>(p);
  else k_conv_ones27<false><<<tl_grid(p.n_out * 4, 256), 256, 0, s>>>(p);
  return hipGetLastError() == hipSuccess ? TL_OK : TL_ERR_LAUNCH;
}


int tl_launch_conv_direct(const ConvP& p, int dtype, hipStream_t s) {
  if (p.in_scale || p.in_relu) return TL_ERR_UNSUPPORTED;
  if (p.one_hot == 2 && !(p.K == 8 && p.Cin == 64 && p.Cout == 32 && p.epi_mode == TL_EPI_NONE && (dtype == TL_BF16 || p.w_x3))) return TL_ERR_UNSUPPORTED;
  const int eb = dtype == TL_BF16 ? 2 : 4;
  if (dtype == TL_BF16 && p.Cin == 4 && p.Cout == 32 && p.K <= 28 && p.table && p.in_ld % 4 == 0 && (int64_t)p.n_in * p.in_ld * 2 < 0xFFFF0000ll) {
    const int ntiles = (int)tl_cdiv(p.n_out, 32);
    int grid = (int)tl_cdiv(ntiles, 8);
    if (grid > 2048) grid = 2048;
    if (p.epi_mode != TL_EPI_NONE) {
      if (p.ctab && p.K == 27) k_conv_in4<8, true, true><<<grid, 512, 0, s>>>(p, ntiles);
      else k_conv_in4<8, false, true><<<grid, 512, 0, s>>>(p, ntiles);
    } else if (p.ctab && p.K == 27) k_conv_in4<8, true><<<grid, 512, 0, s>>>(p, ntiles);
    else k_conv_in4<8><<<grid, 512, 0, s>>>(p, ntiles);
    if (p.red_nparts) *p.red_nparts = grid;
    return hipGetLastError() == hipSuccess ? TL_OK : TL_ERR_LAUNCH;
  }
  if (p.Cin % 32 || p.Cout % 32) return TL_ERR_UNSUPPORTED;
  const int64_t ld_b = p.in_ld * eb, in_bytes = (p.n_in - 1) * ld_b + (int64_t)p.Cin * eb;
  if (!(in_bytes > 0 && in_bytes + 2 * ld_b < 0xFFFFFFFFll)) return TL_ERR_UNSUPPORTED;
  if ((size_t)p.K * p.Cout * p.Cin * eb > 112 * 1024) return TL_ERR_UNSUPPORTED;
  if (dtype == TL_BF16) {
    switch (p.K) {
      case 27: return dispatch<true, 27, 3>(p, s);
      case 8: return dispatch<true, 8, 2>(p, s);
      case 1: return dispatch<true, 1, 1>(p, s);
    }
  } else {
    switch (p.K) {
      case 27: return dispatch<false, 27, 3>(p, s);
      case 8: return dispatch<false, 8, 2>(p, s);
      case 1: return dispatch<false, 1, 1>(p, s);
    }
  }
  return TL_ERR_UNSUPPORTED;
}
```

### treelearn_amd/csrc/tl_conv_internal.h

```cpp
#pragma once
#include "tl_common.h"
#include <hip/hip_bf16.h>
#include "tl_half.h"

#ifdef TL_F16_BUILD
#define tl_launch_conv_direct tl_launch_conv_direct_f16
#define tl_launch_conv_ones27 tl_launch_conv_ones27_f16
#define tl_launch_conv_stream tl_launch_conv_stream_f16
#define tl_launch_conv_streamq tl_launch_conv_streamq_f16
#define tl_launch_conv_small tl_launch_conv_small_f16
#define tl_launch_conv_tinycin tl_launch_conv_tinycin_f16
#define tl_launch_conv_bf16 tl_launch_conv_bf16_f16
#define tl_launch_conv_blk tl_launch_conv_blk_f16
#define tl_launch_conv_up tl_launch_conv_up_f16
#define g_small_mode g_small_mode_f16
#endif

typedef float f32x16 __attribute__((ext_vector_type(16)));
typedef float f32x4 __attribute__((ext_vector_type(4)));
typedef uint32_t u32x4 __attribute__((ext_vector_type(4)));
typedef short s16x8 __attribute__((ext_vector_type(8)));

struct ConvP {
  const void* in; int64_t in_ld;
  const void* w;
  const void* w_frag;
  const void* w_x3;
  const int32_t* table;
  const int32_t* ctab;
  int64_t n_out, n_in;
  int K, Cin, Cout;
  const float* in_scale; const float* in_shift; int in_relu, out_relu;
  const void* res; int64_t res_ld;
  const float* out_scale; const float* out_shift;
  void* out; int64_t out_ld;
  void* out2; int64_t out2_ld; const float* out2_scale; const float* out2_shift; int out2_relu;
  void* out3; int64_t out3_ld; const float* out3_scale; const float* out3_shift; int out3_relu;
  int nblk;
  int epi_mode;
  double* red_part;
  int32_t* red_nparts;
  const void* bn_x; int64_t bn_x_ld;
  const float* bn_mean; const float* bn_rstd; const float* bn_scale; const float* bn_shift; int bn_relu;
  int one_hot;
  const int32_t* blk_unit; const int32_t* blk_counter; const int32_t* blk_halo; const uint32_t* blk_lrb; const int32_t* blk_pmask;
};

static __device__ __forceinline__ float ld_elem(const float* p) { return *p; }
static __device__ __forceinline__ float ld_elem(const __hip_bfloat16* p) { return h16_lo((uint32_t)*reinterpret_cast<const uint16_t*>(p)); }
static __device__ __forceinline__ void st_elem(float* p, float v) { *p = v; }
static __device__ __forceinline__ float ld_elem(const _Float16* p) { return (float)*p; }
static __device__ __forceinline__ void st_elem(_Float16* p, float v) { *p = (_Float16)v; }
static __device__ __forceinline__ void st_elem(__hip_bfloat16* p, float v) { *reinterpret_cast<uint16_t*>(p) = (uint16_t)(h16_pack2(v, 0.f) & 0xFFFFu); }

static __device__ __forceinline__ int xcd_tile(int b, int n) {
  const int q = n >> 3, r = n & 7, x = b & 7, i = b >> 3;
  return (x < r ? x * (q + 1) : r * (q + 1) + (x - r) * q) + i;
}


typedef __bf16 bf16x8 __attribute__((ext_vector_type(8)));

static __device__ __forceinline__ uint32_t pack_bf16x2(float lo, float hi) { return h16_pack2(lo, hi); }
static __device__ __forceinline__ float bf16_lo(uint32_t u) { return h16_lo(u); }
static __device__ __forceinline__ float bf16_hi(uint32_t u) { return h16_hi(u); }

template <bool BF16>
static __device__ __forceinline__ void epi_store1(void* base, int64_t ld, const float* sc, const float* sh, int relu, int64_t row, int j, float y) {
  if (sc) y = fmaf(y, sc[j], sh[j]);
  if (relu) y = fmaxf(y, 0.f);
  if constexpr (BF16) ((uint16_t*)base)[row * ld + j] = (uint16_t)(pack_bf16x2(y, 0.f) & 0xFFFFu);
  else ((float*)base)[row * ld + j] = y;
}
template <bool BF16>
static __device__ __forceinline__ void epi_store8(void* base, int64_t ld, const float* sc, const float* sh, int relu, int64_t row, int c0, const float (&y)[8]) {
  float v[8];
#pragma unroll
  for (int q = 0; q < 8; ++q) v[q] = y[q];
  if (sc) {
    const f32x4 a0 = *reinterpret_cast<const f32x4*>(sc + c0), a1 = *reinterpret_cast<const f32x4*>(sc + c0 + 4);
    const f32x4 b0 = *reinterpret_cast<const f32x4*>(sh + c0), b1 = *reinterpret_cast<const f32x4*>(sh + c0 + 4);
#pragma unroll
    for (int q = 0; q < 4; ++q) { v[q] = fmaf(v[q], a0[q], b0[q]); v[q + 4] = fmaf(v[q + 4], a1[q], b1[q]); }
  }
  if (relu) {
#pragma unroll
    for (int q = 0; q < 8; ++q) v[q] = fmaxf(v[q], 0.f);
  }
  if constexpr (BF16) {
    u32x4 o;
#pragma unroll
    for (int q = 0; q < 4; ++q) o[q] = pack_bf16x2(v[2 * q], v[2 * q + 1]);
    *reinterpret_cast<u32x4*>((uint16_t*)base + row * ld + c0) = o;
  } else {
    f32x4* d = reinterpret_cast<f32x4*>((float*)base + row * ld + c0);
    d[0] = f32x4{v[0], v[1], v[2], v[3]}; d[1] = f32x4{v[4], v[5], v[6], v[7]};
  }
}

// ... 228 lines not shown
```

### treelearn_amd/csrc/tl_conv_small.hip

```cpp
#include "tl_conv_internal.h"

namespace {

template <bool BF16, int NBB, int WV, bool FR, bool X3 = false>
__global__ void __launch_bounds__(WV * 64) k_conv_small(ConvP p, int ncolblk) {
  static_assert(!X3 || !BF16, "split-bf16: fp32 rows, weights in their own layout (FR: its fragment-order second copy)");
  constexpr int EB = BF16 ? 2 : 4, UB = 32 * EB, NJ = UB / 32;
  constexpr int PF = 4;
  constexpr int KMAX = 27;
  __shared__ float red[WV][16][64];
  __shared__ int Is[KMAX * 32];
  const int tid = threadIdx.x, lane = tid & 63, wv = tid >> 6;
  const int rt = blockIdx.x / ncolblk, cb = blockIdx.x % ncolblk;
  const int fi = lane & 31, fh = lane >> 5;
  const int col0 = cb * NBB * 32;
  const int nchunk = p.Cin / 32;
  const int nsteps = p.K * nchunk;
  const bool pro = p.in_scale != nullptr || p.in_relu;

  for (int e = tid; e < p.K * 32; e += WV * 64) {
    const int64_t r = (int64_t)rt * 32 + (e & 31);
    Is[e] = r < p.n_out ? (p.table ? p.table[(int64_t)(e >> 5) * p.n_out + r] : (int)r) : -1;
  }

// ... 112 lines not shown
      if constexpr (BF16) {
        if (p.res) v += bf16_lo((uint32_t)((const uint16_t*)p.res)[orow * p.res_ld + j]);
      } else {
        if (p.res) v += ((const float*)p.res)[orow * p.res_ld + j];
      }
      epi_store1<BF16>(p.out, p.out_ld, p.out_scale, p.out_shift, p.out_relu, orow, j, v);
      if (p.out2) epi_store1<BF16>(p.out2, p.out2_ld, p.out2_scale, p.out2_shift, p.out2_relu, orow, j, v);
      if (p.out3) epi_store1<BF16>(p.out3, p.out3_ld, p.out3_scale, p.out3_shift, p.out3_relu, orow, j, v);
    }
  }
}

template <typename T, int CIN>
__global__ void __launch_bounds__(256) k_conv_tinycin(ConvP p) {
  extern __shared__ __attribute__((aligned(16))) float wsh[];
  const T* w = (const T*)p.w; const T* in = (const T*)p.in; const T* res = (const T*)p.res;
  for (int e = threadIdx.x; e < p.K * CIN * p.Cout; e += 256) {
    const int j = e % p.Cout, c = (e / p.Cout) % CIN, k = e / (p.Cout * CIN);
    wsh[e] = ld_elem(w + ((int64_t)k * p.Cout + j) * p.Cin + c);
  }
  __syncthreads();
  const int ngrp = p.Cout / 8;
  const int64_t total = p.n_out * ngrp;
  for (int64_t t = (int64_t)blockIdx.x * 256 + threadIdx.x; t < total; t += (int64_t)gridDim.x * 256) {
    const int64_t o = t / ngrp; const int j0 = (int)(t % ngrp) * 8;
    float acc[8] = {0.f, 0.f, 0.f, 0.f, 0.f, 0.f, 0.f, 0.f};
    for (int k = 0; k < p.K; ++k) {
      const int64_t idx = p.table ? (int64_t)p.table[(int64_t)k * p.n_out + o] : o;
      if (idx < 0) continue;
      float x[CIN];
#pragma unroll
      for (int c = 0; c < CIN; ++c) x[c] = ld_elem(in + idx * p.in_ld + c);
#pragma unroll
      for (int c = 0; c < CIN; ++c) {
        const float4 w0 = *reinterpret_cast<const float4*>(&wsh[(k * CIN + c) * p.Cout + j0]);
        const float4 w1 = *reinterpret_cast<const float4*>(&wsh[(k * CIN + c) * p.Cout + j0 + 4]);
        acc[0] = fmaf(x[c], w0.x, acc[0]); acc[1] = fmaf(x[c], w0.y, acc[1]); acc[2] = fmaf(x[c], w0.z, acc[2]); acc[3] = fmaf(x[c], w0.w, acc[3]);
        acc[4] = fmaf(x[c], w1.x, acc[4]); acc[5] = fmaf(x[c], w1.y, acc[5]); acc[6] = fmaf(x[c], w1.z, acc[6]); acc[7] = fmaf(x[c], w1.w, acc[7]);
      }
    }
#pragma unroll
    for (int q = 0; q < 8; ++q) if (res) acc[q] += ld_elem(res + o * p.res_ld + j0 + q);
    constexpr bool BF = sizeof(T) == 2;
    epi_store8<BF>(p.out, p.out_ld, p.out_scale, p.out_shift, p.out_relu, o, j0, acc);
    if (p.out2) epi_store8<BF>(p.out2, p.out2_ld, p.out2_scale, p.out2_shift, p.out2_relu, o, j0, acc);
    if (p.out3) epi_store8<BF>(p.out3, p.out3_ld, p.out3_scale, p.out3_shift, p.out3_relu, o, j0, acc);
  }
}

template <typename T>
int launch_tiny(const ConvP& p, hipStream_t s) {
  const size_t lds = (size_t)p.K * p.Cin * p.Cout * 4;
  const unsigned g = tl_grid(p.n_out * (p.Cout / 8), 256);
  switch (p.Cin) {
    case 1: k_conv_tinycin<T, 1><<<g, 256, lds, s>>>(p); break;
    case 2: k_conv_tinycin<T, 2><<<g, 256, lds, s>>>(p); break;
    case 3: k_conv_tinycin<T, 3><<<g, 256, lds, s>>>(p); break;
    case 4: k_conv_tinycin<T, 4><<<g, 256, lds, s>>>(p); break;
    case 5: k_conv_tinycin<T, 5><<<g, 256, lds, s>>>(p); break;
    case 6: k_conv_tinycin<T, 6><<<g, 256, lds, s>>>(p); break;
    case 7: k_conv_tinycin<T, 7><<<g, 256, lds, s>>>(p); break;
    case 8: k_conv_tinycin<T, 8><<<g, 256, lds, s>>>(p); break;
    default: return TL_ERR_UNSUPPORTED;
  }
  return hipGetLastError() == hipSuccess ? TL_OK : TL_ERR_LAUNCH;
}

}

int g_small_mode = 0;

int tl_launch_conv_small(const ConvP& p, int dtype, hipStream_t s) {
  const int nrt = (int)tl_cdiv(p.n_out, 32);
  const bool eight = g_small_mode == 2 || (g_small_mode == 0 && nrt * (p.Cout / 32) <= 512 && p.K * (p.Cin / 32) >= 32);
  const int cbt = p.Cout / 32;
  const bool full = g_small_mode == 0 && dtype == TL_BF16 && (cbt == 3 || cbt == 5 || cbt == 7) && nrt >= 128 && p.w_frag != nullptr &&
                    ((uintptr_t)p.w_frag) % 16 == 0;
  if (full) {
    switch (cbt) {
      case 3: k_conv_small<true, 3, 4, true><<<nrt, 256, 0, s>>>(p, 1); break;
      case 5: k_conv_small<true, 5, 4, true><<<nrt, 256, 0, s>>>(p, 1); break;
      case 7: k_conv_small<true, 7, 4, true><<<nrt, 256, 0, s>>>(p, 1); break;
    }
    return hipGetLastError() == hipSuccess ? TL_OK : TL_ERR_LAUNCH;
  }
  const bool two = !eight && (p.Cout % 64 == 0);
  const int ncb = p.Cout / (two ? 64 : 32);
  const unsigned g = (unsigned)(nrt * ncb);
#define TL_SMALL(BF_, FR_)                                                                   \
  do {                                                                                         \
    if (eight) k_conv_small<BF_, 1, 8, FR_><<<g, 512, 0, s>>>(p, ncb);                         \
    else if (two) k_conv_small<BF_, 2, 4, FR_><<<g, 256, 0, s>>>(p, ncb);                      \
    else k_conv_small<BF_, 1, 4, FR_><<<g, 256, 0, s>>>(p, ncb);                               \
  } while (0)
  const bool fr = p.w_frag != nullptr && ((uintptr_t)p.w_frag) % 16 == 0 && g_small_mode != 3;
  const bool x3 = dtype == TL_F32 && p.w_x3 != nullptr && p.Cin < 256 && !p.in_scale && !p.in_relu;
  if (dtype == TL_BF16) { if (fr) TL_SMALL(true, true); else TL_SMALL(true, false); }
  else if (x3 && g_small_mode != 3 && p.Cout % 32 == 0) {
    if (eight) k_conv_small<false, 1, 8, true, true><<<g, 512, 0, s>>>(p, ncb);
    else if (two) k_conv_small<false, 2, 4, true, true><<<g, 256, 0, s>>>(p, ncb);
    else k_conv_small<false, 1, 4, true, true><<<g, 256, 0, s>>>(p, ncb);
  }
  else if (x3) {
    if (eight) k_conv_small<false, 1, 8, false, true><<<g, 512, 0, s>>>(p, ncb);
    else if (two) k_conv_small<false, 2, 4, false, true><<<g, 256, 0, s>>>(p, ncb);
    else k_conv_small<false, 1, 4, false, true><<<g, 256, 0, s>>>(p, ncb);
  }
  else { if (fr) TL_SMALL(false, true); else TL_SMALL(false, false); }
#undef TL_SMALL
  return hipGetLastError() == hipSuccess ? TL_OK : TL_ERR_LAUNCH;
}

int tl_launch_conv_tinycin(const ConvP& p, int dtype, hipStream_t s) {
  const bool out_ok = (dtype == TL_F32) ? (p.out_ld % 4 == 0 && ((uintptr_t)p.out) % 16 == 0) : (p.out_ld % 8 == 0 && ((uintptr_t)p.out) % 16 == 0);
  if (!out_ok) return TL_ERR_ARG;
  return dtype == TL_F32 ? launch_tiny<float>(p, s) : launch_tiny<__hip_bfloat16>(p, s);
}
```

### treelearn_amd/csrc/tl_conv_stream.hip

```cpp
#include "tl_conv_internal.h"
#include <atomic>

namespace {

constexpr int WAVES = 8;
constexpr int NT = WAVES * 64;

template <bool BF16, int K, int NB, int UN, int DA, int RB, int OCC, bool OH = false, bool X3 = false>
__global__ void __launch_bounds__(NT, OCC) k_conv_stream(ConvP p) {
  static_assert(!X3 || !BF16, "the split-bf16 contraction reads fp32 rows");
  constexpr int EB = BF16 ? 2 : 4, UB = 32 * EB, NJ = UB / 32, SLOTS = UB / 16;
  constexpr int COUT = NB * 32, CIN = UN * 32;
  constexpr int BROW = CIN * EB + 16;
  constexpr int BSLOTS = UN * SLOTS;
  constexpr int BVEC = COUT * BSLOTS;
  constexpr int BPT = (BVEC + NT - 1) / NT;
  constexpr int EP = 32 + 4;
  constexpr int WROWS = 32 * RB;
  extern __shared__ __attribute__((aligned(16))) char smem[];
  char* Bs = smem;
  float* Es = reinterpret_cast<float*>(smem);

  const int tid = threadIdx.x, lane = tid & 63, wv = tid >> 6;
  const int fi = lane & 31, fh = lane >> 5;
// ... 127 lines not shown
        }
    } else
#pragma unroll
    for (int c = 0; c < UN; ++c)
#pragma unroll
      for (int j = 0; j < NJ; ++j) {
#pragma unroll
        for (int nb = 0; nb < NB; ++nb) {
          const int slot = c * SLOTS + 2 * j + fh;
          const u32x4 bf = *reinterpret_cast<const u32x4*>(bl + nb * 32 * BROW + slot * 16);
#pragma unroll
          for (int rb = 0; rb < RB; ++rb) {
            if constexpr (OH) {
              const u32x4 z = {0u, 0u, 0u, 0u};
              mma16<BF16>(acc[rb][nb], idx[k][rb] >= 0 ? a1[rb][c][j] : z, bf);
            } else mma16<BF16>(acc[rb][nb], a[k % DA][rb][c][j], bf);
          }
        }
      }
    if constexpr (!OH) { if (k + DA < K) issue_a(k + DA, a[k % DA]); }
    if (k + 1 < K) __syncthreads();
  }

  __syncthreads();
  float* ew = Es + wv * 32 * EP;
  float red0[NB], red1[NB];
#pragma unroll
  for (int nb = 0; nb < NB; ++nb) { red0[nb] = 0.f; red1[nb] = 0.f; }
#pragma unroll
  for (int rb = 0; rb < RB; ++rb)
#pragma unroll
    for (int nb = 0; nb < NB; ++nb) {
#pragma unroll
      for (int r = 0; r < 16; ++r) ew[((r & 3) + 8 * (r >> 2) + 4 * fh) * EP + fi] = acc[rb][nb][r];
      __builtin_amdgcn_fence(__ATOMIC_RELEASE, "wavefront");
      __builtin_amdgcn_wave_barrier();
      epi_block32<BF16, EP>(p, ew, lane, r0 + rb * 32, nb * 32, red0[nb], red1[nb]);
      __builtin_amdgcn_fence(__ATOMIC_RELEASE, "wavefront");
      __builtin_amdgcn_wave_barrier();
    }
  if (p.epi_mode != TL_EPI_NONE) epi_finish_wg<WAVES, EP, NB>(p, Es, tid, red0, red1);
}

template <bool BF16, int K, int NB, int UN, int DA, int RB, bool OH = false, bool X3 = false>
int launch(ConvP p, hipStream_t s) {
  if constexpr (X3) p.w = p.w_x3;
  constexpr int EB = BF16 ? 2 : 4;
  constexpr int BPTL = (NB * 32 * UN * (BF16 ? 4 : 8) + NT - 1) / NT;
  constexpr int VG = RB * NB * 16 + DA * RB * UN * (BF16 ? 8 : 16) + (K <= 8 ? 8 : 27) * RB + 4 * BPTL * (DA > 2 ? DA - 1 : 1) + 20;
  constexpr int OCC = (OH && X3) ? 2 : ((VG <= 120 || (X3 && NB * UN <= 4)) ? 4 : 2);
  const size_t wt = 2 * (size_t)NB * 32 * (UN * 32 * EB + 16), ep = (size_t)WAVES * 32 * 36 * 4;
  const size_t lds = wt > ep ? wt : ep;
  if (lds > 160 * 1024) return TL_ERR_UNSUPPORTED;
  static TlAttrOnce attr_once;
  if (!tl_lds_attr(attr_once, reinterpret_cast<const void*>(&k_conv_stream<BF16, K, NB, UN, DA, RB, OCC, OH, X3>), 160 * 1024)) return TL_ERR_LAUNCH;
  p.nblk = (int)tl_cdiv(p.n_out, WAVES * 32 * RB);
  k_conv_stream<BF16, K, NB, UN, DA, RB, OCC, OH, X3><<<p.nblk, NT, lds, s>>>(p);
  if (p.red_nparts) *p.red_nparts = p.nblk;
  return hipGetLastError() == hipSuccess ? TL_OK : TL_ERR_LAUNCH;
}

template <bool BF16, int K>
int dispatch(const ConvP& p, hipStream_t s) {
  const int nb = p.Cout / 32, un = p.Cin / 32;
  if constexpr (BF16 && K == 8) {
    if (p.one_hot) {
      if (nb == 2 && un == 3) return launch<true, 8, 2, 3, 1, 1, true>(p, s);
      if (nb == 1 && un == 2) return launch<true, 8, 1, 2, 1, 1, true>(p, s);
      if (nb == 3 && un == 4) return launch<true, 8, 3, 4, 1, 1, true>(p, s);
    }
  }
  if constexpr (!BF16 && K == 8) {
    if (p.one_hot == 1 && p.w_x3 && p.epi_mode == TL_EPI_NONE) {
      if (nb == 2 && un == 3) return launch<false, 8, 2, 3, 1, 1, true, true>(p, s);
      if (nb == 3 && un == 4) return launch<false, 8, 3, 4, 1, 1, true, true>(p, s);
    }
  }
  if constexpr (BF16 && K == 8) {
    if (!p.one_hot && nb == 2 && un == 1) return launch<true, 8, 2, 1, 3, 2>(p, s);
  }
#define TL_S(NB_, UN_, DB_, RB_, DF_)                                                                \
  if (nb == NB_ && un == UN_) {                                                                      \
    if constexpr (BF16) return launch<true, K, NB_, UN_, DB_, RB_>(p, s);                            \
    else {                                                                                           \
      if (p.w_x3) return launch<false, K, NB_, UN_, 1, 1, false, true>(p, s);    \
      return launch<false, K, NB_, UN_, DF_, 1>(p, s);                                               \
    }                                                                                                \
  }
  TL_S(2, 2, 3, 1, 2) TL_S(2, 4, 2, 1, 1) TL_S(3, 3, 1, 2, 1) TL_S(3, 6, 1, 1, 1) TL_S(4, 4, 2, 1, 1) TL_S(2, 3, 3, 1, 1) TL_S(3, 2, 3, 1, 2)
  TL_S(3, 4, 2, 1, 1) TL_S(4, 3, 2, 1, 1) TL_S(1, 2, 3, 1, 2) TL_S(2, 1, 3, 1, 2) TL_S(1, 1, 3, 1, 2)
#undef TL_S
  return TL_ERR_UNSUPPORTED;
}

}

int tl_launch_conv_stream(const ConvP& p, int dtype, hipStream_t s) {
  if (p.in_scale || p.in_relu) return TL_ERR_UNSUPPORTED;
  const int eb = dtype == TL_BF16 ? 2 : 4;
  const int64_t ld_b = p.in_ld * eb, in_bytes = (p.n_in - 1) * ld_b + (int64_t)p.Cin * eb;
  if (!(in_bytes > 0 && in_bytes + 2 * ld_b < 0xFFFFFFFFll)) return TL_ERR_UNSUPPORTED;
  if (dtype == TL_BF16) {
    switch (p.K) {
      case 27: return dispatch<true, 27>(p, s);
      case 8: return dispatch<true, 8>(p, s);
    }
// ... 9 lines not shown
```

### treelearn_amd/csrc/tl_conv_streamq.hip

```cpp
#include "tl_conv_internal.h"
#include <atomic>
#include <type_traits>

namespace {

template <int CTRL>
static __device__ __forceinline__ uint32_t qperm(uint32_t v) {
  return (uint32_t)__builtin_amdgcn_mov_dpp((int)v, CTRL, 0xf, 0xf, true);
}

static __device__ __forceinline__ void quad_transpose(const u32x4 (&S)[4], u32x4 (&F)[4], bool o0, bool o1) {
  u32x4 T[4];
#pragma unroll
  for (int i1 = 0; i1 < 2; ++i1)
#pragma unroll
    for (int d = 0; d < 4; ++d) {
      const uint32_t P = S[2 * i1][d], Q = S[2 * i1 + 1][d];
      const uint32_t Pn = qperm<0xB1>(P), Qn = qperm<0xB1>(Q);
      T[2 * i1][d] = o0 ? Qn : P;
      T[2 * i1 + 1][d] = o0 ? Q : Pn;
    }
#pragma unroll
  for (int x0 = 0; x0 < 2; ++x0)
#pragma unroll
// ... 182 lines not shown
    __builtin_amdgcn_sched_barrier(0);
    u32x4 F[RB][PN][4];
#pragma unroll
    for (int rb = 0; rb < RB; ++rb)
#pragma unroll
      for (int pp = 0; pp < PN; ++pp) {
        quad_transpose(a[k % DA][rb][pp], F[rb][pp], o0, o1);
      }
    const char* bl = Bs + (k & 1) * COUT * BROW + fi * BROW + fh * 64;
#pragma unroll
    for (int pp = 0; pp < PN; ++pp)
#pragma unroll
      for (int s = 0; s < 4; ++s)
#pragma unroll
        for (int nb = 0; nb < NB; ++nb) {
          const u32x4 bf = *reinterpret_cast<const u32x4*>(bl + nb * 32 * BROW + (pp * 8 + s) * 16);
#pragma unroll
          for (int rb = 0; rb < RB; ++rb) {
            mma16<true>(acc[rb][nb], F[rb][pp][s], bf);
          }
        }
    if (k + DA < KV) { issue_a(k + DA, a[k % DA]); if (k + DA + 1 < KV) read_idx(k + DA + 1); }
    if (k + 1 < KV) __syncthreads();
  }
  }

  __syncthreads();
  float* ew = Es + wv * 32 * EP;
  float red0[NB], red1[NB];
#pragma unroll
  for (int nb = 0; nb < NB; ++nb) { red0[nb] = 0.f; red1[nb] = 0.f; }
#pragma unroll
  for (int rb = 0; rb < RB; ++rb)
#pragma unroll
    for (int nb = 0; nb < NB; ++nb) {
#pragma unroll
      for (int r = 0; r < 16; ++r) ew[(2 * (r >> 2) + fh + 8 * (r & 3)) * EP + fi] = acc[rb][nb][r];
      __builtin_amdgcn_fence(__ATOMIC_RELEASE, "wavefront");
      __builtin_amdgcn_wave_barrier();
      epi_block32<!X3, EP>(p, ew, lane, r0 + rb * 32, nb * 32, red0[nb], red1[nb]);
      __builtin_amdgcn_fence(__ATOMIC_RELEASE, "wavefront");
      __builtin_amdgcn_wave_barrier();
    }
  if (p.epi_mode != TL_EPI_NONE) epi_finish_wg<W, EP, NB>(p, Es, tid, red0, red1);
}

template <int K, int NB, int PN, int DA, int W = 8, int RB = 1, int SP = 1, bool X3 = false, bool UL = false>
int launch(ConvP p, hipStream_t s) {
  constexpr int OCC = 2;
  if constexpr (X3) p.w = p.w_x3;
  const size_t wt = 2 * (size_t)NB * 32 * (PN * 128 + 16) + (size_t)W * K * 32 * RB * 4, ep = (size_t)W * 32 * 36 * 4;
  const size_t lds = wt > ep ? wt : ep;
  if (lds > 160 * 1024) return TL_ERR_UNSUPPORTED;
  static TlAttrOnce attr_once;
  if (!tl_lds_attr(attr_once, reinterpret_cast<const void*>(&k_conv_streamq<K, NB, PN, DA, W, RB, OCC, SP, X3, UL>), 160 * 1024)) return TL_ERR_LAUNCH;
  p.nblk = (int)tl_cdiv(p.n_out, W * 32 * RB);
  k_conv_streamq<K, NB, PN, DA, W, RB, OCC, SP, X3, UL><<<p.nblk, W * 64, lds, s>>>(p);
  if (p.red_nparts) *p.red_nparts = p.nblk;
  return hipGetLastError() == hipSuccess ? TL_OK : TL_ERR_LAUNCH;
}

}

int tl_launch_conv_streamq(const ConvP& p, hipStream_t s) {
  if (p.in_scale || p.in_relu || p.Cin % 64 || p.Cout % 32) return TL_ERR_UNSUPPORTED;
  const int64_t ld_b = p.in_ld * 2, in_bytes = (p.n_in - 1) * ld_b + (int64_t)p.Cin * 2;
  if (!(in_bytes > 0 && in_bytes + 2 * ld_b < 0xFFFFFFFFll)) return TL_ERR_UNSUPPORTED;
  const int nb = p.Cout / 32, pn = p.Cin / 64;
  if (p.K == 27) {
    if (nb == 2 && pn == 1) return launch<27, 2, 1, 2>(p, s);
    if (nb == 2 && pn == 2) return launch<27, 2, 2, 2>(p, s);
    if (nb == 4 && pn == 2) return launch<27, 4, 2, 2>(p, s);
    if (nb == 4 && pn == 1) return launch<27, 4, 1, 2>(p, s);
    if (nb == 3 && pn == 3) return launch<27, 3, 3, 2>(p, s);
    if (nb == 4 && pn == 4) return launch<27, 4, 2, 2, 8, 1, 2>(p, s);
  } else if (p.K == 8) {
    if (nb == 3 && pn == 1) return launch<8, 3, 1, 2>(p, s);
  }
  return TL_ERR_UNSUPPORTED;
}

#ifndef TL_F16_BUILD
int tl_launch_conv_streamq_x3(const ConvP& p, hipStream_t s) {
  if (!p.w_x3 || p.in_scale || p.in_relu || p.Cin % 32 || p.Cout % 32 || p.K != 27 || p.epi_mode != TL_EPI_NONE || p.Cin >= 256) return TL_ERR_UNSUPPORTED;
  const int64_t ld_b = p.in_ld * 4, in_bytes = (p.n_in - 1) * ld_b + (int64_t)p.Cin * 4;
  if (!(in_bytes > 0 && in_bytes + 2 * ld_b < 0xFFFFFFFFll) || ((uintptr_t)p.w_x3) % 16) return TL_ERR_UNSUPPORTED;
  const int nb = p.Cout / 32, pn = p.Cin / 32;
  if (nb == 2 && pn == 2) return launch<27, 2, 2, 1, 8, 1, 1, true, true>(p, s);
  if (nb == 2 && pn == 4) return launch<27, 2, 2, 1, 8, 1, 2, true>(p, s);
  if (nb == 3 && pn == 6) return launch<27, 3, 3, 2, 8, 1, 2, true>(p, s);
  return TL_ERR_UNSUPPORTED;
}
#endif
```

### treelearn_amd/csrc/tl_conv_up.hip

```cpp
#include "tl_conv_internal.h"
#include <atomic>

namespace {

template <int NBI, int NBO, int WAVES>
__global__ void __launch_bounds__(WAVES * 64) k_conv_up(ConvP p, const int32_t* __restrict__ child, int ntiles) {
  constexpr int K = 8, KS = 2 * NBI;
  constexpr int EP = 36;
  constexpr int WB = K * NBO * NBI * 2 * 1024;
  extern __shared__ __attribute__((aligned(16))) char smem[];
  const int tid = threadIdx.x, lane = tid & 63, wv = tid >> 6;
  const int fi = lane & 31, fh = lane >> 5;
  {
    const u32x4* src = reinterpret_cast<const u32x4*>(p.w_frag);
    u32x4* dst = reinterpret_cast<u32x4*>(smem);
    for (int e = tid; e < WB / 16; e += WAVES * 64) dst[e] = src[e];
    __syncthreads();
  }
  float* ew = reinterpret_cast<float*>(smem + WB) + wv * 32 * EP;
  const unsigned in_ldb = (unsigned)(p.in_ld * 2);
  const __amdgpu_buffer_rsrc_t rx = __builtin_amdgcn_make_buffer_rsrc(const_cast<void*>(p.in), 0, (int)((p.n_in - 1) * (int64_t)in_ldb + NBI * 64), 0x00020000);
  const __amdgpu_buffer_rsrc_t rc = __builtin_amdgcn_make_buffer_rsrc(const_cast<int32_t*>(child), 0, (int)((int64_t)K * p.n_in * 4), 0x00020000);

  const int nw = (int)gridDim.x * WAVES;
// ... 12 lines not shown
        c[k][e0] = r < p.n_in ? __builtin_amdgcn_raw_buffer_load_b32(rc, (int)(((int64_t)k * p.n_in + r) * 4), 0, 0) : -1;
      }
  };
  if (t < ntiles) request(t, A, ch);
  for (; t < ntiles; t += nw) {
    u32x4 An[KS]; int chn[K][2];
    const int tn = t + nw;
    if (tn < ntiles) request(tn, An, chn);
#pragma unroll
    for (int k = 0; k < K; ++k) {
      const bool any = __builtin_amdgcn_ballot_w64(ch[k][0] >= 0 || ch[k][1] >= 0) != 0ull;
      if (!any) continue;
#pragma unroll
      for (int nb = 0; nb < NBO; ++nb) {
        f32x16 acc;
#pragma unroll
        for (int i = 0; i < 16; ++i) acc[i] = 0.f;
#pragma unroll
        for (int s_ = 0; s_ < KS; ++s_) {
          const int v = (((k * NBO + nb) * NBI + (s_ >> 1)) * 2 + (s_ & 1)) * 64 + lane;
          acc = h16_mfma(A[s_], *reinterpret_cast<const u32x4*>(smem + (size_t)v * 16), acc);
        }
#pragma unroll
        for (int r = 0; r < 16; ++r) ew[((r & 3) + 8 * (r >> 2) + 4 * fh) * EP + fi] = acc[r];
        __builtin_amdgcn_fence(__ATOMIC_RELEASE, "wavefront");
        __builtin_amdgcn_wave_barrier();
#pragma unroll
        for (int e0 = 0; e0 < 2; ++e0) {
          const int rr = (lane >> 2) + 16 * e0, cvv = lane & 3;
          const int orow = ch[k][e0];
          if (orow >= 0 && orow < (int)p.n_out) {
            const f32x4 v0 = *reinterpret_cast<const f32x4*>(ew + rr * EP + cvv * 8), v1 = *reinterpret_cast<const f32x4*>(ew + rr * EP + cvv * 8 + 4);
            float v[8] = {v0[0], v0[1], v0[2], v0[3], v1[0], v1[1], v1[2], v1[3]};
            epi_views8<true>(p, (int64_t)orow, nb * 32 + cvv * 8, v);
          }
        }
        __builtin_amdgcn_fence(__ATOMIC_RELEASE, "wavefront");
        __builtin_amdgcn_wave_barrier();
      }
    }
    if (tn < ntiles) {
#pragma unroll
      for (int s_ = 0; s_ < KS; ++s_) A[s_] = An[s_];
#pragma unroll
      for (int k = 0; k < K; ++k) { ch[k][0] = chn[k][0]; ch[k][1] = chn[k][1]; }
    }
  }
}

template <int NBI, int NBO, int WAVES>
int launch_up(const ConvP& p, const int32_t* child, hipStream_t s) {
  const size_t lds = (size_t)8 * NBO * NBI * 2 * 1024 + (size_t)WAVES * 32 * 36 * 4;
  static_assert(8 * NBO * NBI * 2 * 1024 + WAVES * 32 * 36 * 4 <= 160 * 1024, "weights + epilogue tiles must fit the LDS");
  static TlAttrOnce attr_once;
  if (!tl_lds_attr(attr_once, reinterpret_cast<const void*>(&k_conv_up<NBI, NBO, WAVES>), 160 * 1024)) return TL_ERR_LAUNCH;
  const int ntiles = (int)tl_cdiv(p.n_in, 32);
  const int per_cu = (int)((160 * 1024) / lds) < 1 ? 1 : (int)((160 * 1024) / lds);
  int grid = 256 * (per_cu > 4 ? 4 : per_cu);
  const int need = (int)tl_cdiv(ntiles, WAVES);
  if (grid > need) grid = need;
  k_conv_up<NBI, NBO, WAVES><<<grid, WAVES * 64, lds, s>>>(p, child, ntiles);
  return hipGetLastError() == hipSuccess ? TL_OK : TL_ERR_LAUNCH;
}

}

int tl_launch_conv_up(const ConvP& p, const int32_t* child, hipStream_t s) {
  if (!child || !p.w_frag || ((uintptr_t)p.w_frag) % 16 || p.K != 8 || p.in_scale || p.in_relu || p.res || p.epi_mode != TL_EPI_NONE) return TL_ERR_UNSUPPORTED;
  auto big = [&](int64_t rows, int64_t ld) { return (rows - 1) * ld * 2 + 512 >= 0x7FFFFFFFll; };
  if (big(p.n_in, p.in_ld) || big(p.n_out, p.out_ld) || (p.out2 && big(p.n_out, p.out2_ld)) || (p.out3 && big(p.n_out, p.out3_ld)) || (int64_t)8 * p.n_in * 4 >= 0x7FFFFFFFll)
    return TL_ERR_UNSUPPORTED;
  if (p.Cin == 96 && p.Cout == 64) return launch_up<3, 2, 12>(p, child, s);
  return TL_ERR_UNSUPPORTED;
}
```

### treelearn_amd/csrc/tl_exec.hip

```cpp
#include <string.h>
#include <vector>

#include "tl_common.h"
#include "tl_arena.h"

namespace {

constexpr int64_t kCompactMinRows = 65536;
constexpr int64_t kBlkMinRows = 16384;
constexpr int64_t kBlkMaxRows = (1 << 25) - 64;
constexpr size_t kHostBytes = 64 + (size_t)TL_POINT_COORDS_MAX_PARTS * 16;

struct Ten {
  int64_t off = -1;
  int64_t ld = 0, n = 0;
  int C = 0;
  int64_t own_off = -1, own_bytes = 0;
};

struct ViewReq {
  const Ten* dst = nullptr;
  tl_affine aff{nullptr, nullptr};
  int relu = 0;
};

struct Table {
  const int32_t* table = nullptr;
  const int32_t* compact = nullptr;
  const int32_t* scatter = nullptr;
  bool blk = false;
  int one_hot = 0;
};

struct LevelG {
  int32_t dims[4];
  int64_t n = 0;
  int64_t coords = -1, nbr = -1, ct = -1, child = -1, inv = -1, invp = -1;
};

}

struct tl_exec {
  int32_t* host = nullptr;
  hipEvent_t ev_main = nullptr, ev_side = nullptr, ev_flag = nullptr;
  bool flag_in_flight = false;
  bool profile = false;
  std::vector<hipEvent_t> pev;
  std::vector<tl_launch_rec> recs;
  hipStream_t prof_stream = nullptr;
};

namespace {

struct Run {
  tl_exec* ex;
  const tl_net_desc* net;
  tl_forward_args* a;
  hipStream_t s;
  Arena ar;
  int esize;
  int rc = TL_OK;
  int launches = 0;
  int nl;
  LevelG lv[TL_MAX_LEVELS];
  bool blocked = false;
  int64_t g0 = 0;
  int64_t o_unit = -1, o_counter = -1, o_halo = -1, o_lrb = -1, o_pmask = -1, o_nn = -1;

  const int32_t* gw(int64_t word_off) const { return word_off < 0 ? nullptr : reinterpret_cast<const int32_t*>(ar.at(g0 + 4 * word_off)); }

  Ten alloc(int64_t n, int C) {
    Ten t;
    t.n = n; t.C = C; t.ld = C; t.own_bytes = n * C * esize; t.own_off = t.off = ar.take(t.own_bytes);
    return t;
  }
  void release(Ten& t) {
    if (t.own_off >= 0) ar.give(t.own_off, t.own_bytes);
    t.own_off = -1;
  }
  Ten cols(const Ten& t, int c0, int C) const {
    Ten v;
    v.off = t.off + (int64_t)c0 * esize; v.ld = t.ld; v.n = t.n; v.C = C;
    return v;
  }

  Table subm(int li) const {
    Table t;
    if (li == 0 && blocked) { t.blk = true; return t; }
    t.table = gw(lv[li].nbr); t.compact = gw(lv[li].ct);
    return t;
  }
  Table down(int li) const { Table t; t.table = gw(lv[li].child); return t; }
  Table up(int li) const {
    Table t;
    t.scatter = gw(lv[li].child);
    if (lv[li].invp >= 0) { t.table = gw(lv[li].invp); t.one_hot = 2; }
    else { t.table = gw(lv[li].inv); t.one_hot = 1; }
    return t;
  }

  void conv(int level, int kind, const Ten& x, const tl_weight& w, const Table& tb, int64_t n_out, const ViewReq* views, int nviews, Ten* outs,
            const Ten* residual = nullptr, tl_affine in_aff = {nullptr, nullptr}, int in_relu = 0, int all_ones = 0, int split_part = -1, int split_cin = 0) {
    for (int i = 0; i < nviews; ++i) outs[i] = views[i].dst ? *views[i].dst : alloc(n_out, w.Cout);
    if (rc != TL_OK) return;
    ++launches;
    if (ar.dry) return;
    tl_conv_args c{};
    c.in = ar.at(x.off); c.in_ld = x.ld; c.weight = w.w; c.weight_frag = w.frag; c.weight_x3 = w.x3;
    c.table = tb.table; c.table_compact = tb.compact; c.table_one_hot = tb.one_hot; c.table_scatter = tb.scatter;
    if (tb.blk) {
      c.blk_unit = gw(o_unit); c.blk_counter = gw(o_counter); c.blk_halo = gw(o_halo);
      c.blk_lrb = reinterpret_cast<const uint32_t*>(gw(o_lrb)); c.blk_pmask = gw(o_pmask);
    }
    c.in_all_ones = all_ones;
    c.n_out = n_out; c.n_in = x.n; c.K = w.K; c.Cin = w.Cin; c.Cout = w.Cout; c.dtype = net->dtype;
    c.in_scale = in_aff.scale; c.in_shift = in_aff.shift; c.in_relu = in_relu;
    if (residual) { c.residual = ar.at(residual->off); c.res_ld = residual->ld; }
    c.out = ar.at(outs[0].off); c.out_ld = outs[0].ld; c.out_scale = views[0].aff.scale; c.out_shift = views[0].aff.shift; c.out_relu = views[0].relu;
    if (nviews > 1) { c.out2 = ar.at(outs[1].off); c.out2_ld = outs[1].ld; c.out2_scale = views[1].aff.scale; c.out2_shift = views[1].aff.shift; c.out2_relu = views[1].relu; }
    if (nviews > 2) { c.out3 = ar.at(outs[2].off); c.out3_ld = outs[2].ld; c.out3_scale = views[2].aff.scale; c.out3_shift = views[2].aff.shift; c.out3_relu = views[2].relu; }
    const bool prof = ex->profile;
    if (prof) {
      hipEvent_t e0 = nullptr, e1 = nullptr;
      if (hipEventCreate(&e0) != hipSuccess || hipEventCreate(&e1) != hipSuccess) { rc = TL_ERR_LAUNCH; return; }
      ex->pev.push_back(e0); ex->pev.push_back(e1);
      tl_launch_rec r{};
      r.level = level; r.kind = kind; r.K = w.K; r.Cin = w.Cin; r.Cout = w.Cout; r.residual = residual != nullptr; r.esize = esize;
      r.split_part = split_part; r.split_cin = split_cin; r.in_prologue = in_aff.scale != nullptr || in_relu; r.n_out = n_out; r.n_in = x.n;
      ex->recs.push_back(r);
      if (hipEventRecord(e0, s) != hipSuccess) rc = TL_ERR_LAUNCH;
    }
    const int r = tl_conv_fwd(&c, s);
    if (prof && hipEventRecord(ex->pev.back(), s) != hipSuccess) rc = TL_ERR_LAUNCH;
    if (r != TL_OK) rc = r;
  }

  static ViewReq RAW(const Ten* dst = nullptr) { ViewReq v; v.dst = dst; return v; }
  static ViewReq ACT(const tl_affine& aff, const Ten* dst = nullptr) { ViewReq v; v.dst = dst; v.aff = aff; v.relu = 1; return v; }

  void res_block(int li, const tl_res_desc& b, const Ten& x_raw, const Ten& x_act, const ViewReq* views, int nviews, Ten* outs) {
    const Table nb = subm(li);
    const int64_t n = lv[li].n;
    Ten t, res;
    const ViewReq v1 = ACT(b.bn3);
    conv(li, 0, x_act, b.w1, nb, n, &v1, 1, &t);
    const bool has1x1 = b.w1x1.w != nullptr;
    if (has1x1) { const ViewReq vr = RAW(); conv(li, 3, x_raw, b.w1x1, Table{}, n, &vr, 1, &res); }
    conv(li, 0, t, b.w2, nb, n, views, nviews, outs, has1x1 ? &res : &x_raw);
    release(t);
    if (has1x1) release(res);
  }

  void ublock(int li, Ten x_raw, Ten x_act, const ViewReq* views, int nviews, Ten* outs) {
    const tl_ublock_desc& u = net->u[li];
    const int64_t n = lv[li].n;
    const int C = u.C;
    Ten o2[3];
    { const ViewReq v[2] = {RAW(), ACT(u.blocks[1].bn0)}; res_block(li, u.blocks[0], x_raw, x_act, v, 2, o2); }
    release(x_raw); release(x_act);
    x_raw = o2[0]; x_act = o2[1];
    if (!u.deeper) {
      res_block(li, u.blocks[1], x_raw, x_act, views, nviews, outs);
      release(x_raw); release(x_act);
      return;
    }
    Ten cat_raw = alloc(n, 2 * C), cat_act = alloc(n, 2 * C);
    const Ten cr_l = cols(cat_raw, 0, C), cr_r = cols(cat_raw, C, C), ca_l = cols(cat_act, 0, C), ca_r = cols(cat_act, C, C);
    Ten o3[3];
    { const ViewReq v[3] = {RAW(&cr_l), ACT(u.bn_cat_l, &ca_l), ACT(u.bn_down)}; res_block(li, u.blocks[1], x_raw, x_act, v, 3, o3); }
    release(x_raw); release(x_act);
    Ten xd = o3[2], d[2];
    { const ViewReq v[2] = {RAW(), ACT(net->u[li + 1].blocks[0].bn0)}; conv(li, 1, xd, u.wd, down(li), lv[li + 1].n, v, 2, d); }
    release(xd);
// ... 5 lines not shown
    { const ViewReq v[2] = {RAW(), ACT(u.tail[1].bn0)}; res_block(li, u.tail[0], cat_raw, cat_act, v, 2, y); }
    release(cat_raw); release(cat_act);
    res_block(li, u.tail[1], y[0], y[1], views, nviews, outs);
    release(y[0]); release(y[1]);
  }

  void l1_block(const tl_res_desc& b, const Ten& x, const tl_affine& in_aff, const ViewReq* views, int nviews, Ten* outs) {
    const Table nb = subm(0);
    const int64_t n = lv[0].n;
    Ten t, res;
    const ViewReq v1 = ACT(b.bn3);
    conv(0, 0, x, b.w1, nb, n, &v1, 1, &t, nullptr, in_aff, 1);
    const bool has1x1 = b.w1x1.w != nullptr;
    if (has1x1) { const ViewReq vr = RAW(); conv(0, 3, x, b.w1x1, Table{}, n, &vr, 1, &res); }
    conv(0, 0, t, b.w2, nb, n, views, nviews, outs, has1x1 ? &res : &x);
    release(t);
    if (has1x1) release(res);
  }
  void l1_staged(Ten x_raw, const ViewReq* views, int nviews, Ten* outs) {
    const tl_ublock_desc& u = net->u[0];
    const int64_t n = lv[0].n;
    const int C = u.C;
    const Table nb = subm(0);
    Ten x1;
    { const ViewReq v = RAW(); l1_block(u.blocks[0], x_raw, u.blocks[0].bn0, &v, 1, &x1); }
    release(x_raw);
    Ten cat_raw = alloc(n, 2 * C);
    const Ten cr_l = cols(cat_raw, 0, C), cr_r = cols(cat_raw, C, C);
    Ten o2[2];
    { const ViewReq v[2] = {RAW(&cr_l), ACT(u.bn_down)}; l1_block(u.blocks[1], x1, u.blocks[1].bn0, v, 2, o2); }
    release(x1);
    Ten xd = o2[1], d[2];
    { const ViewReq v[2] = {RAW(), ACT(net->u[1].blocks[0].bn0)}; conv(0, 1, xd, u.wd, down(0), lv[1].n, v, 2, d); }
    release(xd);
    Ten e_act;
    { const ViewReq v = ACT(u.bn_up); ublock(1, d[0], d[1], &v, 1, &e_act); }
    { const ViewReq v = RAW(&cr_r); Ten o; conv(0, 2, e_act, u.wu, up(0), n, &v, 1, &o); }
    release(e_act);
    const tl_res_desc& b = u.tail[0];
    Ten part, t, res, y;
    { const ViewReq v = RAW(); conv(0, 0, cr_l, b.w1_half[0], nb, n, &v, 1, &part, nullptr, u.bn_cat_l, 1, 0, 0, 2 * C); }
    { const ViewReq v = ACT(b.bn3); conv(0, 0, cr_r, b.w1_half[1], nb, n, &v, 1, &t, &part, u.bn_cat_r, 1, 0, 1, 2 * C); }
    release(part);
    { const ViewReq v = RAW(); conv(0, 3, cat_raw, b.w1x1, Table{}, n, &v, 1, &res); }
    { const ViewReq v = RAW(); conv(0, 0, t, b.w2, nb, n, &v, 1, &y, &res); }
    release(t); release(res); release(cat_raw);
    l1_block(u.tail[1], y, u.tail[1].bn0, views, nviews, outs);
    release(y);
  }

  void network() {
    const int64_t n1 = lv[0].n;
    const bool feats = net->use_coords || net->use_feats;
    Ten ones = alloc(n1, net->in_channels);
    if (feats) {
      const int64_t ws_bytes = 4 * n1 * net->max_points_per_voxel, o_ws = ar.take(ws_bytes);
      if (!ar.dry) {
        const int r = tl_voxel_feats(a->xyz, a->point_feats, net->in_channels - 3, reinterpret_cast<const int64_t*>(gw(o_v2p)), a->N, n1, net->max_points_per_voxel,
                                     net->use_coords, net->use_feats, net->dtype, reinterpret_cast<int32_t*>(ar.at(o_ws)), ar.at(ones.off), s);
        if (r != TL_OK) rc = r;
      }
      ar.give(o_ws, ws_bytes);
    } else if (!ar.dry) {
      hipError_t e;
      if (net->dtype == TL_F32) e = hipMemsetD32Async((hipDeviceptr_t)ar.at(ones.off), 0x3F800000, n1 * net->in_channels, s);
      else e = hipMemsetD16Async((hipDeviceptr_t)ar.at(ones.off), net->dtype == TL_BF16 ? 0x3F80 : 0x3C00, n1 * net->in_channels, s);
      if (e != hipSuccess) rc = TL_ERR_LAUNCH;
    }
    Ten xs[2], x;
    const ViewReq out = RAW();
    if (blocked) {
      const ViewReq v = RAW();
      Table tin = subm(0);
      if (feats) { tin = Table{}; tin.table = gw(o_nn); }
      conv(0, 4, ones, net->w_in, tin, n1, &v, 1, xs, nullptr, {nullptr, nullptr}, 0, feats ? 0 : 1);
      release(ones);
      l1_staged(xs[0], &out, 1, &x);
    } else {
      const ViewReq v[2] = {RAW(), ACT(net->u[0].blocks[0].bn0)};
      conv(0, 4, ones, net->w_in, subm(0), n1, v, 2, xs, nullptr, {nullptr, nullptr}, 0, feats ? 0 : 1);
      release(ones);
      ublock(0, xs[0], xs[1], &out, 1, &x);
    }
    if (rc == TL_OK && !ar.dry) {
      const int r = tl_head_mlp(ar.at(x.off), x.ld, net->dtype, x.C, reinterpret_cast<const int64_t*>(gw(o_v2p)), a->N, net->out_bn.scale, net->out_bn.shift,
                                net->head_w1, net->head_b1, net->head_w2, net->head_b2, a->backbone, a->logits, a->offsets, s);
      if (r != TL_OK) rc = r;
    }
    release(x);
  }
  int64_t o_v2p = -1;
};

inline int64_t al64(int64_t w) { return (w + 63) & ~int64_t(63); }

inline bool weight_is(const tl_weight& w, int K, int Cin, int Cout) { return w.w && w.K == K && w.Cin == Cin && w.Cout == Cout; }
inline bool affine_ok(const tl_affine& a) { return a.scale && a.shift; }

inline bool res_ok(const tl_res_desc& b, int Cin, int C) {
  if (!affine_ok(b.bn0) || !affine_ok(b.bn3) || !weight_is(b.w1, 27, Cin, C) || !weight_is(b.w2, 27, C, C)) return false;
  if (Cin != C ? !weight_is(b.w1x1, 1, Cin, C) : b.w1x1.w != nullptr) return false;
  for (int h = 0; h < 2; ++h)
    if (b.w1_half[h].w && !(Cin == 2 * C && weight_is(b.w1_half[h], 27, C, C))) return false;
  return (b.w1_half[0].w == nullptr) == (b.w1_half[1].w == nullptr);
}

inline bool net_ok(const tl_net_desc* net) {
  const int nl = net->num_levels;
  if (!weight_is(net->w_in, 27, net->in_channels, net->u[0].C)) return false;
  if (net->u[0].C != 8 && net->u[0].C != 16 && net->u[0].C != 32 && net->u[0].C != 64) return false;
  if (!affine_ok(net->out_bn) || !net->head_w1 || !net->head_b1 || !net->head_w2 || !net->head_b2) return false;
  for (int l = 0; l < nl; ++l) {
    const tl_ublock_desc& u = net->u[l];
    if (u.C <= 0 || (u.deeper != 0) != (l + 1 < nl)) return false;
    if (!res_ok(u.blocks[0], u.C, u.C) || !res_ok(u.blocks[1], u.C, u.C)) return false;
    if (!u.deeper) continue;
    const int Cd = net->u[l + 1].C;
    if (!affine_ok(u.bn_down) || !affine_ok(u.bn_up) || !affine_ok(u.bn_cat_l) || !affine_ok(u.bn_cat_r)) return false;
    if (!weight_is(u.wd, 8, u.C, Cd) || !weight_is(u.wu, 8, Cd, u.C)) return false;
    if (!res_ok(u.tail[0], 2 * u.C, u.C) || !res_ok(u.tail[1], u.C, u.C)) return false;
  }
  return true;
}

}

extern "C" {

tl_exec* tl_exec_create(void) {
  tl_exec* ex = new (std::nothrow) tl_exec();
  if (!ex) return nullptr;
  if (hipHostMalloc(reinterpret_cast<void**>(&ex->host), kHostBytes, hipHostMallocDefault) != hipSuccess || (memset(ex->host, 0, kHostBytes), false) ||
      hipEventCreateWithFlags(&ex->ev_main, hipEventDisableTiming) != hipSuccess || hipEventCreateWithFlags(&ex->ev_side, hipEventDisableTiming) != hipSuccess ||
// ... 82 lines not shown
      for (int j = 0; j < 4; ++j) ex->host[j] = ex->host[j] > ex->host[16 + 4 * q + j] ? ex->host[j] : ex->host[16 + 4 * q + j];
  } else if (hipMemcpyAsync(ex->host, R.ar.at(o_maxc), 16, hipMemcpyDeviceToHost, s) != hipSuccess || hipStreamSynchronize(s) != hipSuccess) return TL_ERR_LAUNCH;
  ex->flag_in_flight = false;
  if (ex->host[3]) return TL_ERR_EXTENT;
  if (ex->host[8]) {
    ex->host[8] = 0;
    return TL_ERR_BLK;
  }
  const int32_t extent[3] = {ex->host[0] + 1, ex->host[1] + 1, ex->host[2] + 1};
  int32_t shape[TL_MAX_LEVELS][3];
  for (int j = 0; j < 3; ++j) {
    shape[0][j] = net->has_shape ? net->spatial_shape[j] : extent[j];
    if (extent[j] > shape[0][j]) return TL_ERR_EXTENT;
  }
  for (int l = 1; l < nl; ++l)
    for (int j = 0; j < 3; ++j) {
      shape[l][j] = shape[l - 1][j] / 2;
      if (shape[l][j] <= 0) return TL_ERR_REACH_ZERO;
    }

  int64_t nw[TL_MAX_LEVELS], woff[TL_MAX_LEVELS + 1];
  {
    int32_t d[4] = {a->B, extent[0], extent[1], extent[2]};
    woff[0] = 0;
    for (int l = 0; l < nl; ++l) {
      for (int j = 0; j < 4; ++j) R.lv[l].dims[j] = d[j];
      nw[l] = tl_nwords(tl_dims(d));
      woff[l + 1] = woff[l] + nw[l];
      for (int j = 1; j < 4; ++j) d[j] = (d[j] + 1) / 2;
    }
  }
  const int64_t tw = woff[nl];
  const int64_t n_ws = tl_pyramid_ws_words(R.lv[0].dims, nl, nullptr);
  if (n_ws < 0) return TL_ERR_ARG;
  const int64_t o_pyr = R.ar.take(4 * (3 * tw + 8 + n_ws));
  if (R.ar.peak > R.ar.cap) { a->needed_bytes = R.ar.peak * 2; return TL_ERR_ARENA; }
  char* p0 = R.ar.at(o_pyr);
  rc = tl_pyramid_build(pcoords, N, R.lv[0].dims, shape[0], nl, reinterpret_cast<uint64_t*>(p0), reinterpret_cast<uint32_t*>(p0 + 8 * tw),
                        reinterpret_cast<uint32_t*>(p0 + 12 * tw), reinterpret_cast<uint32_t*>(p0 + 12 * tw + 32), stream);
  if (rc != TL_OK) return rc;
  if (hipMemcpyAsync(ex->host, p0 + 12 * tw, 4 * nl, hipMemcpyDeviceToHost, s) != hipSuccess || hipStreamSynchronize(s) != hipSuccess) return TL_ERR_LAUNCH;
  for (int l = 0; l < nl; ++l) {
    R.lv[l].n = a->level_n[l] = (int64_t)(uint32_t)ex->host[l];
    if (R.lv[l].n <= 0) return TL_ERR_REACH_ZERO;
  }

  const int64_t n1 = R.lv[0].n;
  const tl_ublock_desc& u0 = net->u[0];
  const bool x3_l1 = u0.blocks[0].w1.x3 && u0.blocks[0].w2.x3 && u0.blocks[1].w1.x3 && u0.blocks[1].w2.x3 && u0.tail[0].w1_half[0].x3 && u0.tail[0].w1_half[1].x3 &&
                     u0.tail[0].w2.x3 && u0.tail[1].w1.x3 && u0.tail[1].w2.x3;
  R.blocked = net->blocked && (net->dtype != TL_F32 || x3_l1) && u0.C == 32 && u0.deeper && u0.tail[0].w1_half[0].w && u0.tail[0].w1_half[1].w &&
              n1 >= kBlkMinRows && n1 <= kBlkMaxRows;
  a->blocked_used = R.blocked;
  int64_t cur = 0;
  auto take = [&](int64_t words) { const int64_t o = cur; cur += al64(words); return o; };
  R.o_v2p = take(2 * N);
  for (int l = 0; l < nl; ++l) {
    LevelG& v = R.lv[l];
    const bool skip = R.blocked && l == 0;
    if (!skip) { v.coords = take(4 * v.n); v.nbr = take(27 * v.n); }
    if (!skip && v.n >= kCompactMinRows) v.ct = take(10 * v.n);
    if (l + 1 < nl) v.child = take(8 * R.lv[l + 1].n);
  }
  int64_t o_o2n = -1, o_perm = -1, o_cnew = -1, o_bws = -1;
  if (R.blocked) {
    const int64_t nbws = tl_blk_ws_words(R.lv[0].dims);
    o_o2n = take(n1); o_perm = take(n1); o_cnew = take(4 * n1); R.o_unit = take(4 * n1); R.o_counter = take(64); R.o_halo = take(32 * n1);
    R.o_lrb = take(9 * n1); R.o_pmask = take(n1); o_bws = take(nbws);
    if (feats) R.o_nn = take(27 * n1);
  }
  const bool packed0 = nl > 1 && net->u[0].C == 32 && net->u[1].C == 64 && (net->dtype != TL_F32 || net->u[0].wu.x3) && tl_conv_one_hot_direct_enabled(n1);
  const int64_t o_m1 = cur;
  for (int l = 0; l + 1 < nl; ++l) {
    if (l == 0 && packed0) R.lv[l].invp = take(R.lv[l].n);
    else R.lv[l].inv = take(8 * R.lv[l].n);
  }
  const int64_t o_m1_end = cur;
  R.g0 = R.ar.take(4 * cur);

  {
    Run D = R;
    D.ar.dry = true; D.ar.base = nullptr;
    D.network();
    a->needed_bytes = D.ar.peak;
    if (D.ar.peak > R.ar.cap) return TL_ERR_ARENA;
  }

  auto W = [&](int64_t word_off) { return word_off < 0 ? nullptr : reinterpret_cast<int32_t*>(R.ar.at(R.g0 + 4 * word_off)); };
  tl_level arr[TL_MAX_LEVELS];
  for (int l = 0; l < nl; ++l) {
    LevelG& v = R.lv[l];
    tl_level& t = arr[l];
    for (int j = 0; j < 4; ++j) t.dims[j] = v.dims[j];
    t.n = v.n;
    t.bitmap = reinterpret_cast<const uint64_t*>(p0 + 8 * woff[l]); t.prefix = reinterpret_cast<const uint32_t*>(p0 + 8 * tw + 4 * woff[l]);
    t.coords = W(v.coords); t.nbr = W(v.nbr); t.compact = W(v.ct); t.child = W(v.child); t.parent = nullptr; t.inv = W(v.inv); t.inv_packed = W(v.invp); t.o2n = nullptr;
  }
  hipStream_t side = s;
  struct Join {
    tl_exec* ex; hipStream_t s; hipStream_t* side; bool done = false;
    int join() {
      if (done || *side == s) return TL_OK;
      done = true;
      return (hipEventRecord(ex->ev_side, *side) == hipSuccess && hipStreamWaitEvent(s, ex->ev_side, 0) == hipSuccess) ? TL_OK : TL_ERR_LAUNCH;
    }
    ~Join() { (void)join(); }
  } joiner{ex, s, &side};
  if (R.blocked) {
    tl_blk bk{};
    bk.o2n = W(o_o2n); bk.perm = W(o_perm); bk.coords_new = W(o_cnew); bk.unit = W(R.o_unit); bk.counter = W(R.o_counter); bk.halo = W(R.o_halo);
    bk.lrb = reinterpret_cast<uint32_t*>(W(R.o_lrb)); bk.pmask = W(R.o_pmask); bk.cap_units = n1; bk.halo_max = TL_BLK_HALO_MAX; bk.nn = W(R.o_nn);
    rc = tl_blk_build(arr[0].bitmap, arr[0].prefix, R.lv[0].dims, n1, &bk, reinterpret_cast<uint32_t*>(W(o_bws)), 1, stream);
    if (rc != TL_OK) return rc;
    arr[0].o2n = bk.o2n;
    if (a->side_stream && tl_s(a->side_stream) != s) {
      side = tl_s(a->side_stream);
      if (hipEventRecord(ex->ev_main, s) != hipSuccess || hipStreamWaitEvent(side, ex->ev_main, 0) != hipSuccess) return TL_ERR_LAUNCH;
    }
    rc = tl_blk_build(arr[0].bitmap, arr[0].prefix, R.lv[0].dims, n1, &bk, reinterpret_cast<uint32_t*>(W(o_bws)), 2, reinterpret_cast<tl_stream_t>(side));
    if (rc != TL_OK) return rc;
  }
  rc = tl_rulebooks_build(arr, nl, W(o_m1), o_m1_end - o_m1, pcoords, N, reinterpret_cast<int64_t*>(W(R.o_v2p)), stream);
  if (rc != TL_OK) return rc;
  if (joiner.join() != TL_OK) return TL_ERR_LAUNCH;
  if (R.blocked) {
    if (hipMemcpyAsync(ex->host + 8, W(R.o_counter) + 1, 4, hipMemcpyDeviceToHost, s) != hipSuccess || hipEventRecord(ex->ev_flag, s) != hipSuccess) return TL_ERR_LAUNCH;
    ex->flag_in_flight = true;
  }
// ... 8 lines not shown
```

### treelearn_amd/csrc/tl_linear_small.hip

```cpp
#include "tl_conv_internal.h"
#include "tl_f16_train.h"

int tl_launch_wgrad_reduce(const float* ws, int64_t nparts, int64_t per, float* gw, hipStream_t s, int K = 1, int Cout = 0, int Cin = 0, int ref_layout = 0);

namespace {

template <bool BF16>
static __device__ __forceinline__ void load8(const void* base, int64_t elem, float (&v)[8]) {
  if constexpr (BF16) {
    const u32x4 q = *reinterpret_cast<const u32x4*>((const uint16_t*)base + elem);
#pragma unroll
    for (int i = 0; i < 4; ++i) { v[2 * i] = bf16_lo(q[i]); v[2 * i + 1] = bf16_hi(q[i]); }
  } else {
    const f32x4 a = *reinterpret_cast<const f32x4*>((const float*)base + elem), b = *reinterpret_cast<const f32x4*>((const float*)base + elem + 4);
#pragma unroll
    for (int i = 0; i < 4; ++i) { v[i] = a[i]; v[i + 4] = b[i]; }
  }
}

template <bool BF16, int CO, bool OF32 = false>
__global__ void __launch_bounds__(256) k_conv_tinycout(ConvP p) {
  extern __shared__ __attribute__((aligned(16))) float wsh[];
  for (int e = threadIdx.x; e < CO * p.Cin; e += 256)
    wsh[e] = BF16 ? bf16_lo((uint32_t)((const uint16_t*)p.w)[e]) : ((const float*)p.w)[e];
// ... 13 lines not shown
        for (int q = 0; q < 4; ++q) { acc[j] = fmaf(x[q], w0[q], acc[j]); acc[j] = fmaf(x[q + 4], w1[q], acc[j]); }
      }
    }
#pragma unroll
    for (int j = 0; j < CO; ++j) epi_store1<BF16 && !OF32>(p.out, p.out_ld, p.out_scale, p.out_shift, p.out_relu, o, j, acc[j]);
  }
}

template <bool BF16, int CO>
__global__ void __launch_bounds__(256) k_wgrad_tinycout(const void* __restrict__ x, int64_t x_ld, const void* __restrict__ g, int64_t g_ld, int64_t n, int Cin,
                                                        int64_t rpb, float* __restrict__ part) {
  extern __shared__ __attribute__((aligned(16))) float red[];
  const int cgs = Cin >> 3, rl = 256 / cgs;
  const int t = threadIdx.x, cg = t % cgs, lane = t / cgs;
  float acc[CO][8];
#pragma unroll
  for (int j = 0; j < CO; ++j)
#pragma unroll
    for (int q = 0; q < 8; ++q) acc[j][q] = 0.f;
  if (lane < rl) {
    const int64_t r0 = (int64_t)blockIdx.x * rpb, r1 = min(n, r0 + rpb);
#pragma unroll 2
    for (int64_t r = r0 + lane; r < r1; r += rl) {
      float xv[8], gv[CO];
      load8<BF16>(x, r * x_ld + cg * 8, xv);
#pragma unroll
      for (int j = 0; j < CO; ++j) gv[j] = BF16 ? bf16_lo((uint32_t)((const uint16_t*)g)[r * g_ld + j]) : ((const float*)g)[r * g_ld + j];
#pragma unroll
      for (int j = 0; j < CO; ++j)
#pragma unroll
        for (int q = 0; q < 8; ++q) acc[j][q] = fmaf(gv[j], xv[q], acc[j][q]);
    }
#pragma unroll
    for (int j = 0; j < CO; ++j)
#pragma unroll
      for (int q = 0; q < 8; ++q) red[((int64_t)lane * CO + j) * Cin + cg * 8 + q] = acc[j][q];
  }
  __syncthreads();
  for (int e = t; e < CO * Cin; e += 256) {
    float s = 0.f;
    for (int l = 0; l < rl; ++l) s += red[(int64_t)l * CO * Cin + e];
    part[(int64_t)blockIdx.x * CO * Cin + e] = s;
  }
}

}

int tl_launch_conv_tinycout(const ConvP& p, int dtype, hipStream_t s) {
  if (p.K != 1 || p.table || p.Cout < 1 || p.Cout > 8 || p.Cin % 8 || p.Cin > 1024 || p.res || p.out2 || p.out3 || p.in_scale || p.in_relu) return TL_ERR_UNSUPPORTED;
  const int eb = dtype == TL_BF16 ? 2 : 4;
  if (p.in_ld % 8 || ((uintptr_t)p.in) % 16 || ((uintptr_t)p.w) % eb) return TL_ERR_UNSUPPORTED;
  const unsigned g = tl_grid(p.n_out, 256);
  const size_t lds = (size_t)p.Cout * p.Cin * 4;
#define TL_TC(CO_)                                                                     \
  case CO_:                                                                            \
    if (dtype == TL_BF16) k_conv_tinycout<true, CO_><<<g, 256, lds, s>>>(p);           \
    else k_conv_tinycout<false, CO_><<<g, 256, lds, s>>>(p);                           \
    break;
  switch (p.Cout) { TL_TC(1) TL_TC(2) TL_TC(3) TL_TC(4) TL_TC(5) TL_TC(6) TL_TC(7) TL_TC(8) }
#undef TL_TC
  return hipGetLastError() == hipSuccess ? TL_OK : TL_ERR_LAUNCH;
}

int64_t tl_wgrad_tinycout_parts(int64_t n) {
  int64_t b = tl_cdiv(n, 2048);
  if (b > 1024) b = 1024;
  return b < 1 ? 1 : b;
}

int tl_launch_wgrad_tinycout(const void* x, int64_t x_ld, const void* g, int64_t g_ld, int dtype, int64_t n, int Cin, int Cout, float* gw, float* ws, hipStream_t s) {
  if (Cout < 1 || Cout > 4 || Cin % 8 || Cin > 256 || 256 % (Cin / 8) || (Cout * Cin) % 4 || x_ld % 8 || ((uintptr_t)x) % 16 || ((uintptr_t)ws) % 16 || ((uintptr_t)gw) % 16)
    return TL_ERR_UNSUPPORTED;
  const int64_t blocks = tl_wgrad_tinycout_parts(n), rpb = tl_cdiv(n, blocks);
  const int64_t used = tl_cdiv(n, rpb);
  const size_t lds = (size_t)(256 / (Cin / 8)) * Cout * Cin * 4;
  if (lds > 64 * 1024) return TL_ERR_UNSUPPORTED;
#define TL_TW(CO_)                                                                                                            \
  case CO_:                                                                                                                   \
    if (dtype == TL_BF16) k_wgrad_tinycout<true, CO_><<<(unsigned)used, 256, lds, s>>>(x, x_ld, g, g_ld, n, Cin, rpb, ws);     \
    else k_wgrad_tinycout<false, CO_><<<(unsigned)used, 256, lds, s>>>(x, x_ld, g, g_ld, n, Cin, rpb, ws);                     \
    break;
  switch (Cout) { TL_TW(1) TL_TW(2) TL_TW(3) TL_TW(4) }
#undef TL_TW
  if (hipGetLastError() != hipSuccess) return TL_ERR_LAUNCH;
  return tl_launch_wgrad_reduce(ws, used, (int64_t)Cout * Cin, gw, s);
}

extern "C" int tl_linear_small_f32(const void* x, int64_t x_ld, int dtype, const void* w, int Cin, int Cout, int64_t n, float* out, int64_t out_ld,
                                   tl_stream_t stream) {
#ifndef TL_F16_BUILD
  if (dtype == TL_F16) return tl_linear_small_f32_f16(x, x_ld, TL_BF16, w, Cin, Cout, n, out, out_ld, stream);
#endif
  if (!x || !w || !out || n <= 0 || Cin <= 0 || Cout < 1 || Cout > 8 || (dtype != TL_F32 && dtype != TL_BF16)) return TL_ERR_ARG;
  if (Cin % 8 || Cin > 1024 || x_ld % 8 || ((uintptr_t)x) % 16) return TL_ERR_UNSUPPORTED;
  ConvP p{};
  p.in = x; p.in_ld = x_ld; p.w = w; p.n_out = n; p.n_in = n; p.K = 1; p.Cin = Cin; p.Cout = Cout; p.out = out; p.out_ld = out_ld;
  const unsigned g = tl_grid(n, 256);
  const size_t lds = (size_t)Cout * Cin * 4;
  hipStream_t s = tl_s(stream);
#define TL_TF(CO_)                                                                             \
  case CO_:                                                                                    \
    if (dtype == TL_BF16) k_conv_tinycout<true, CO_, true><<<g, 256, lds, s>>>(p);             \
    else k_conv_tinycout<false, CO_, true><<<g, 256, lds, s>>>(p);                             \
    break;
  switch (Cout) { TL_TF(1) TL_TF(2) TL_TF(3) TL_TF(4) TL_TF(5) TL_TF(6) TL_TF(7) TL_TF(8) }
#undef TL_TF
// ... 3 lines not shown
```

### treelearn_amd/csrc/tl_voxel.hip

```cpp
#include "tl_common.h"

namespace {

constexpr int kBlock = 256;

__device__ __forceinline__ uint32_t enc_f32(float f) {
  uint32_t u = __float_as_uint(f);
  return u ^ ((u >> 31) ? 0xFFFFFFFFu : 0x80000000u);
}
__device__ __forceinline__ float dec_f32(uint32_t u) {
  return __uint_as_float((u & 0x80000000u) ? (u ^ 0x80000000u) : ~u);
}

__global__ void k_init_minmax(uint32_t* __restrict__ mm, int B, int32_t* __restrict__ maxc) {
  const int i = blockIdx.x * blockDim.x + threadIdx.x;
  if (i < B * 6) mm[i] = ((i % 6) < 3) ? 0xFFFFFFFFu : 0u;
  if (i < 4) maxc[i] = 0;
}

__global__ void __launch_bounds__(kBlock) k_minmax(const float* __restrict__ xyz, const int64_t* __restrict__ bid,
                                                   int64_t N_all, int B, uint32_t* __restrict__ mm) {
  uint32_t lo[3] = {0xFFFFFFFFu, 0xFFFFFFFFu, 0xFFFFFFFFu}, hi[3] = {0u, 0u, 0u};
  int cb = -1;
  auto flush = [&]() {
// ... 433 lines not shown
    int64_t row = pf[i];
    while (w) {
      const int bit = __ffsll((unsigned long long)w) - 1;
      reinterpret_cast<int4*>(coords)[row++] = make_int4(b, x, y, zw * 64 + bit);
      w &= w - 1;
    }
  }
}

__global__ void __launch_bounds__(kBlock) k_expand_coords(const uint64_t* __restrict__ bm, const uint32_t* __restrict__ pf, TlDims d,
                                                          int32_t* __restrict__ coords) {
  expand_coords_body(bm, pf, d, coords, (int64_t)blockIdx.x * blockDim.x + threadIdx.x, (int64_t)gridDim.x * blockDim.x);
}

__global__ void __launch_bounds__(kBlock) k_point_rank(const int32_t* __restrict__ pc, int64_t N, const uint64_t* __restrict__ bm,
                                                       const uint32_t* __restrict__ pf, TlDims d, int64_t* __restrict__ v2p,
                                                       const int32_t* __restrict__ o2n) {
  for (int64_t i = (int64_t)blockIdx.x * blockDim.x + threadIdx.x; i < N; i += (int64_t)gridDim.x * blockDim.x) {
    const int4 c = reinterpret_cast<const int4*>(pc)[i];
    int r = -1;
    if (c.x >= 0 && c.x < d.B && c.y < d.X && c.z < d.Y && c.w < d.Z) r = tl_rank_at(bm, pf, tl_col_word(d, c.x, c.y, c.z), c.w);
    if (o2n && r >= 0) r = o2n[r];
    v2p[i] = r;
  }
}

__device__ __forceinline__ void rulebook_subm_body(const int32_t* __restrict__ coords, int64_t M, const uint64_t* __restrict__ bm,
                                                   const uint32_t* __restrict__ pf, const TlDims& d, int32_t* __restrict__ nbr,
                                                   int32_t* __restrict__ compact, int64_t first, int64_t stride) {
  for (int64_t i = first; i < M; i += stride) {
    const int4 c = reinterpret_cast<const int4*>(coords)[i];
    uint32_t cmask = 0;
#pragma unroll
    for (int dx = -1; dx <= 1; ++dx) {
#pragma unroll
      for (int dy = -1; dy <= 1; ++dy) {
        const int x = c.y + dx, y = c.z + dy;
        const int tap0 = (dx + 1) * 9 + (dy + 1) * 3;
        int r0 = -1, r1 = -1, r2 = -1;
        if (x >= 0 && x < d.X && y >= 0 && y < d.Y) {
          const int64_t wc = tl_col_word(d, c.x, x, y);
          const int z = c.w;
          const int64_t w = wc + (z >> 6);
          const uint64_t word = bm[w];
          const uint32_t base = pf[w];
          const int bit = z & 63;
          const uint64_t below = (1ull << bit) - 1;
          if (word & (1ull << bit)) r1 = (int)(base + __popcll(word & below));
          if (bit > 0) { if (word & (1ull << (bit - 1))) r0 = (int)(base + __popcll(word & (below >> 1))); }
          else if (z > 0) r0 = tl_rank_at(bm, pf, wc, z - 1);
          if (bit < 63) { if (word & (2ull << bit)) r2 = (int)(base + __popcll(word & ((below << 1) | 1ull))); }
          else if (z + 1 < d.Z) r2 = tl_rank_at(bm, pf, wc, z + 1);
        }
        nbr[(int64_t)(tap0 + 0) * M + i] = r0;
        nbr[(int64_t)(tap0 + 1) * M + i] = r1;
        nbr[(int64_t)(tap0 + 2) * M + i] = r2;
        if (compact) {
          compact[(int64_t)(tap0 / 3) * M + i] = r0 >= 0 ? r0 : (r1 >= 0 ? r1 : r2);
          cmask |= ((r0 >= 0 ? 1u : 0u) | (r1 >= 0 ? 2u : 0u) | (r2 >= 0 ? 4u : 0u)) << tap0;
        }
      }
    }
    if (compact) compact[(int64_t)9 * M + i] = (int32_t)cmask;
  }
}

__global__ void __launch_bounds__(kBlock) k_rulebook_subm(const int32_t* __restrict__ coords, int64_t M, const uint64_t* __restrict__ bm,
                                                          const uint32_t* __restrict__ pf, TlDims d, int32_t* __restrict__ nbr,
                                                          int32_t* __restrict__ compact) {
  rulebook_subm_body(coords, M, bm, pf, d, nbr, compact, (int64_t)blockIdx.x * blockDim.x + threadIdx.x, (int64_t)gridDim.x * blockDim.x);
}

__device__ __forceinline__ void rulebook_down_body(const int32_t* __restrict__ cc, int64_t Mc, const uint64_t* __restrict__ fbm,
                                                   const uint32_t* __restrict__ fpf, const TlDims& f, int64_t Mf, int32_t* __restrict__ child,
                                                   int32_t* __restrict__ parent, int32_t* __restrict__ inv, int64_t first, int64_t stride,
                                                   const int32_t* __restrict__ fo2n = nullptr, int32_t* __restrict__ invp = nullptr) {
  for (int64_t q = first; q < Mc; q += stride) {
    const int4 c = reinterpret_cast<const int4*>(cc)[q];
#pragma unroll
    for (int k = 0; k < 8; ++k) {
      const int x = 2 * c.y + (k >> 2), y = 2 * c.z + ((k >> 1) & 1), z = 2 * c.w + (k & 1);
      int r = -1;
      if (x < f.X && y < f.Y && z < f.Z) r = tl_rank_at(fbm, fpf, tl_col_word(f, c.x, x, y), z);
      if (fo2n && r >= 0) r = fo2n[r];
      child[(int64_t)k * Mc + q] = r;
      if (r >= 0) {
        if (parent) parent[r] = (int)q;
        if (inv) inv[(int64_t)k * Mf + r] = (int)q;
        if (invp) invp[r] = (int)((q << 3) | k);
      }
    }
  }
}

__global__ void __launch_bounds__(kBlock) k_rulebook_down(const int32_t* __restrict__ cc, int64_t Mc, const uint64_t* __restrict__ fbm,
                                                          const uint32_t* __restrict__ fpf, TlDims f, int64_t Mf,
                                                          int32_t* __restrict__ child, int32_t* __restrict__ parent, int32_t* __restrict__ inv,
                                                          const int32_t* __restrict__ fo2n, int32_t* __restrict__ invp) {
  rulebook_down_body(cc, Mc, fbm, fpf, f, Mf, child, parent, inv, (int64_t)blockIdx.x * blockDim.x + threadIdx.x, (int64_t)gridDim.x * blockDim.x, fo2n, invp);
}

struct LevelPack {
  int nl;
  int first[kPyrMaxLevels + 1];
  TlDims d[kPyrMaxLevels];
  int64_t n[kPyrMaxLevels];
  const uint64_t* bm[kPyrMaxLevels];
  const uint32_t* pf[kPyrMaxLevels];
  int32_t* coords[kPyrMaxLevels];
// ... 152 lines not shown
  if (!bitmap || !prefix || !total || !ws || nwords <= 0) return TL_ERR_ARG;
  const int64_t nb = tl_cdiv(nwords, kScanTile);
  hipStream_t s = tl_s(stream);
  k_scan_partials<<<(unsigned)nb, kBlock, 0, s>>>(bitmap, nwords, ws);
  k_scan_blocks<<<1, kBlock, 0, s>>>(ws, nb, total);
  k_scan_final<<<(unsigned)nb, kBlock, 0, s>>>(bitmap, nwords, ws, prefix);
  TL_CHECK_LAUNCH();
  return TL_OK;
}

int tl_expand_coords(const uint64_t* bitmap, const uint32_t* prefix, const int32_t dims[4], int32_t* coords, tl_stream_t stream) {
  if (!bitmap || !prefix || !dims || !coords) return TL_ERR_ARG;
  const TlDims d = tl_dims(dims);
  k_expand_coords<<<tl_grid(tl_nwords(d), kBlock), kBlock, 0, tl_s(stream)>>>(bitmap, prefix, d, coords);
  TL_CHECK_LAUNCH();
  return TL_OK;
}

int tl_point_rank(const int32_t* pcoords, int64_t N, const uint64_t* bitmap, const uint32_t* prefix, const int32_t dims[4],
                  int64_t* v2p, tl_stream_t stream) {
  if (!pcoords || !bitmap || !prefix || !dims || !v2p || N <= 0) return TL_ERR_ARG;
  k_point_rank<<<tl_grid(N, kBlock), kBlock, 0, tl_s(stream)>>>(pcoords, N, bitmap, prefix, tl_dims(dims), v2p, nullptr);
  TL_CHECK_LAUNCH();
  return TL_OK;
}

int tl_voxel_mean_feats(const float* pf, int C, const int64_t* v2p, int64_t N, int64_t M, int P, int32_t* ws, float* out,
                        tl_stream_t stream) {
  if (!pf || !v2p || !ws || !out || C <= 0 || C > 64 || N <= 0 || M <= 0 || P <= 0 || N > 0x7FFFFFFE) return TL_ERR_ARG;
  hipStream_t s = tl_s(stream);
  k_fill_i32<<<tl_grid(M * P, kBlock), kBlock, 0, s>>>(ws, M * P, 0x7FFFFFFF);
  for (int r = 0; r < P; ++r) k_first_points<<<tl_grid(N, kBlock), kBlock, 0, s>>>(v2p, N, P, r, ws);
  k_mean_feats<<<tl_grid(M * C, kBlock), kBlock, 0, s>>>(pf, C, M, P, ws, out);
  TL_CHECK_LAUNCH();
  return TL_OK;
}

int tl_voxel_feats(const float* xyz, const float* feats, int F, const int64_t* v2p, int64_t N, int64_t M, int P, int use_coords, int use_feats,
                   int dtype, int32_t* ws, void* out, tl_stream_t stream) {
  if (!xyz || !feats || !v2p || !ws || !out || F <= 0 || F > 5 || N <= 0 || M <= 0 || P <= 0 || N > 0x7FFFFFFE) return TL_ERR_ARG;
  hipStream_t s = tl_s(stream);
  k_fill_i32<<<tl_grid(M * P, kBlock), kBlock, 0, s>>>(ws, M * P, 0x7FFFFFFF);
  for (int r = 0; r < P; ++r) k_first_points<<<tl_grid(N, kBlock), kBlock, 0, s>>>(v2p, N, P, r, ws);
  if (dtype == TL_F32) k_voxel_feats<float><<<tl_grid(M, kBlock), kBlock, 0, s>>>(xyz, feats, F, M, P, ws, use_coords, use_feats, static_cast<float*>(out));
  else if (dtype == TL_BF16) k_voxel_feats<__bf16><<<tl_grid(M, kBlock), kBlock, 0, s>>>(xyz, feats, F, M, P, ws, use_coords, use_feats, static_cast<__bf16*>(out));
  else if (dtype == TL_F16) k_voxel_feats<_Float16><<<tl_grid(M, kBlock), kBlock, 0, s>>>(xyz, feats, F, M, P, ws, use_coords, use_feats, static_cast<_Float16*>(out));
  else return TL_ERR_ARG;
  TL_CHECK_LAUNCH();
  return TL_OK;
}

int tl_rulebook_subm(const int32_t* coords, int64_t M, const uint64_t* bitmap, const uint32_t* prefix, const int32_t dims[4],
                     int32_t* nbr, int32_t* compact, tl_stream_t stream) {
  if (!coords || !bitmap || !prefix || !dims || !nbr || M <= 0) return TL_ERR_ARG;
  k_rulebook_subm<<<tl_grid(M, kBlock), kBlock, 0, tl_s(stream)>>>(coords, M, bitmap, prefix, tl_dims(dims), nbr, compact);
  TL_CHECK_LAUNCH();
  return TL_OK;
}

int tl_rulebook_down(const int32_t* ccoords, int64_t Mc, const uint64_t* fbitmap, const uint32_t* fprefix, const int32_t fdims[4],
                     int64_t Mf, int32_t* child, int32_t* parent, int32_t* inv, tl_stream_t stream) {
  if (!ccoords || !fbitmap || !fprefix || !fdims || !child || !parent || !inv || Mc <= 0 || Mf <= 0) return TL_ERR_ARG;
  hipStream_t s = tl_s(stream);
  if (hipMemsetAsync(parent, 0xFF, Mf * 4, s) != hipSuccess) return TL_ERR_LAUNCH;
  if (hipMemsetAsync(inv, 0xFF, Mf * 8 * 4, s) != hipSuccess) return TL_ERR_LAUNCH;
  k_rulebook_down<<<tl_grid(Mc, kBlock), kBlock, 0, s>>>(ccoords, Mc, fbitmap, fprefix, tl_dims(fdims), Mf, child, parent, inv, nullptr, nullptr);
  TL_CHECK_LAUNCH();
  return TL_OK;
}

int64_t tl_pyramid_ws_words(const int32_t dims0[4], int num_levels, int64_t* level_word_offsets) {
  if (!dims0 || num_levels < 1 || num_levels > kPyrMaxLevels) return -1;
  int32_t d[4] = {dims0[0], dims0[1], dims0[2], dims0[3]};
  int64_t off = 0, ws = 0;
  for (int l = 0; l < num_levels; ++l) {
    const int64_t nw = tl_nwords(tl_dims(d));
    if (level_word_offsets) level_word_offsets[l] = off;
    off += nw;
    ws += tl_scan_ws_words(nw);
    for (int j = 1; j < 4; ++j) d[j] = (d[j] + 1) / 2;
  }
  if (level_word_offsets) level_word_offsets[num_levels] = off;
  {
    int32_t d0[4] = {dims0[0], dims0[1], dims0[2], dims0[3]};
    ws += 4 + 16 * tl_nwords(tl_dims(d0));
  }
  return ws;
}

int tl_pyramid_build(const int32_t* pcoords, int64_t N, const int32_t dims0[4], const int32_t shape0[3], int num_levels,
                     uint64_t* bitmaps, uint32_t* prefixes, uint32_t* counts, uint32_t* ws, tl_stream_t stream) {
  if (!pcoords || !dims0 || !shape0 || !bitmaps || !prefixes || !counts || !ws || N <= 0 || num_levels < 1 || num_levels > kPyrMaxLevels)
    return TL_ERR_ARG;
  hipStream_t s = tl_s(stream);
  TlDims d[kPyrMaxLevels];
  int out[kPyrMaxLevels][3];
  int64_t off[kPyrMaxLevels + 1];
  int32_t dd[4] = {dims0[0], dims0[1], dims0[2], dims0[3]};
  int sh[3] = {shape0[0], shape0[1], shape0[2]};
  off[0] = 0;
  for (int l = 0; l < num_levels; ++l) {
    d[l] = tl_dims(dd);
    for (int j = 0; j < 3; ++j) out[l][j] = sh[j];
    off[l + 1] = off[l] + tl_nwords(d[l]);
    for (int j = 1; j < 4; ++j) dd[j] = (dd[j] + 1) / 2;
    for (int j = 0; j < 3; ++j) sh[j] /= 2;
  }
  {
    int64_t scan_ws = 0;
    for (int l2 = 0; l2 < num_levels; ++l2) scan_ws += tl_scan_ws_words(tl_nwords(d[l2]));
    uint8_t* bytes = reinterpret_cast<uint8_t*>((reinterpret_cast<uintptr_t>(ws + scan_ws) + 15) & ~uintptr_t(15));
    const int64_t nw0 = tl_nwords(d[0]);
    if (hipMemsetAsync(bytes, 0, nw0 * 64, s) != hipSuccess) return TL_ERR_LAUNCH;
    k_set_bytes<<<tl_grid(N, kBlock), kBlock, 0, s>>>(pcoords, N, d[0], bytes);
    k_bytes_to_bits<<<tl_grid(nw0, kBlock), kBlock, 0, s>>>(bytes, nw0, bitmaps);
  }
  int l = 0;
  ScanPack sp;
  sp.first[0] = 0;
  for (; l < num_levels; ++l) {
    const int64_t nw = tl_nwords(d[l]);
    if (l > 0 && nw <= kPyrSmallWords) break;
    if (l > 0)
      k_bitmap_down<<<tl_grid(nw, kBlock), kBlock, 0, s>>>(bitmaps + off[l - 1], d[l - 1], out[l][0], out[l][1], out[l][2], bitmaps + off[l], d[l]);
    sp.off[l] = off[l]; sp.nw[l] = nw; sp.first[l + 1] = sp.first[l] + (int)tl_cdiv(nw, kScanTile);
  }
  sp.nl = l;
  k_scan_partials_multi<<<(unsigned)sp.first[l], kBlock, 0, s>>>(bitmaps, sp, ws);
  k_scan_blocks_multi<<<1, kBlock, 0, s>>>(ws, sp, counts);
  k_scan_final_multi<<<(unsigned)sp.first[l], kBlock, 0, s>>>(bitmaps, sp, ws, prefixes);
  if (l < num_levels) {
    PyrSmall p;
    p.nl = num_levels - l; p.first = l;
    p.d[0] = d[l - 1]; p.off[0] = off[l - 1];
    for (int j = 0; j < p.nl; ++j) {
      p.d[j + 1] = d[l + j]; p.off[j + 1] = off[l + j];
      for (int k = 0; k < 3; ++k) p.out[j][k] = out[l + j][k];
    }
    k_pyramid_small<<<1, kPyrBlock, 0, s>>>(bitmaps, prefixes, counts, p);
  }
  TL_CHECK_LAUNCH();
  return TL_OK;
}

int tl_rulebooks_build(const tl_level* lv, int num_levels, int32_t* minus_one, int64_t minus_one_words,
                       const int32_t* pcoords, int64_t N, int64_t* v2p, tl_stream_t stream) {
  if (!lv || num_levels < 1 || num_levels > kPyrMaxLevels) return TL_ERR_ARG;
  for (int l = 0; l < num_levels; ++l) {
    if (!lv[l].bitmap || !lv[l].prefix || lv[l].n <= 0) return TL_ERR_ARG;
    if ((!lv[l].coords || !lv[l].nbr) && !lv[l].o2n) return TL_ERR_ARG;
    if (lv[l].nbr && !lv[l].coords) return TL_ERR_ARG;
    if (l > 0 && !lv[l].coords) return TL_ERR_ARG;
    if (l + 1 < num_levels && (!lv[l].child || (!lv[l].inv && !lv[l].inv_packed))) return TL_ERR_ARG;
    if (lv[l].inv_packed && lv[l].n >= (1ll << 28)) return TL_ERR_ARG;
  }
  hipStream_t s = tl_s(stream);
  auto inside = [&](const int32_t* q, int64_t words) { return minus_one && q >= minus_one && q + words <= minus_one + minus_one_words; };
  if (minus_one && minus_one_words > 0 && hipMemsetAsync(minus_one, 0xFF, minus_one_words * 4, s) != hipSuccess) return TL_ERR_LAUNCH;
  for (int l = 0; l + 1 < num_levels; ++l) {
    if (lv[l].parent && !inside(lv[l].parent, lv[l].n) && hipMemsetAsync(lv[l].parent, 0xFF, lv[l].n * 4, s) != hipSuccess) return TL_ERR_LAUNCH;
    if (lv[l].inv && !inside(lv[l].inv, lv[l].n * 8) && hipMemsetAsync(lv[l].inv, 0xFF, lv[l].n * 32, s) != hipSuccess) return TL_ERR_LAUNCH;
    if (lv[l].inv_packed && !inside(lv[l].inv_packed, lv[l].n) && hipMemsetAsync(lv[l].inv_packed, 0xFF, lv[l].n * 4, s) != hipSuccess) return TL_ERR_LAUNCH;
  }
  int small = num_levels;
  for (int l = num_levels - 1; l >= 1; --l) {
    if (tl_nwords(tl_dims(lv[l].dims)) <= kPyrSmallWords && lv[l].n <= 64 * kPyrSmallWords && !lv[l].compact && !lv[l].o2n && !lv[l - 1].o2n &&
        !lv[l].inv_packed && !lv[l - 1].inv_packed) small = l; else break;
  }
  if (num_levels - small < 2) small = num_levels;
  for (int l = 0; l < small; ++l) {
    const TlDims d = tl_dims(lv[l].dims);
    if (lv[l].coords) k_expand_coords<<<tl_grid(tl_nwords(d), kBlock), kBlock, 0, s>>>(lv[l].bitmap, lv[l].prefix, d, lv[l].coords);
    if (lv[l].nbr) k_rulebook_subm<<<tl_grid(lv[l].n, kBlock), kBlock, 0, s>>>(lv[l].coords, lv[l].n, lv[l].bitmap, lv[l].prefix, d, lv[l].nbr, lv[l].compact);
  }
  LevelPack p;
  p.nl = num_levels - small;
  if (p.nl > 0) {
    for (int j = 0; j < p.nl; ++j) {
      const tl_level& v = lv[small + j];
      p.d[j] = tl_dims(v.dims); p.n[j] = v.n; p.bm[j] = v.bitmap; p.pf[j] = v.prefix; p.coords[j] = v.coords; p.nbr[j] = v.nbr;
      p.child[j] = v.child; p.parent[j] = v.parent; p.inv[j] = v.inv;
    }
    p.first[0] = 0;
    for (int j = 0; j < p.nl; ++j) p.first[j + 1] = p.first[j] + (int)tl_cdiv(tl_nwords(p.d[j]), kBlock);
    k_expand_coords_multi<<<p.first[p.nl], kBlock, 0, s>>>(p);
    for (int j = 0; j < p.nl; ++j) p.first[j + 1] = p.first[j] + (int)tl_cdiv(p.n[j], kBlock);
    k_rulebook_subm_multi<<<p.first[p.nl], kBlock, 0, s>>>(p);
  }
  for (int l = 0; l + 1 < num_levels && l < small; ++l) {
    const tl_level &f = lv[l], &c = lv[l + 1];
    k_rulebook_down<<<tl_grid(c.n, kBlock), kBlock, 0, s>>>(c.coords, c.n, f.bitmap, f.prefix, tl_dims(f.dims), f.n, f.child, f.parent, f.inv, f.o2n, f.inv_packed);
  }
  if (p.nl > 1) {
    p.nl -= 1;
    for (int j = 0; j < p.nl; ++j) p.first[j + 1] = p.first[j] + (int)tl_cdiv(p.n[j + 1], kBlock);
    k_rulebook_down_multi<<<p.first[p.nl], kBlock, 0, s>>>(p);
  }
  if (v2p) {
    if (!pcoords || N <= 0) return TL_ERR_ARG;
    k_point_rank<<<tl_grid(N, kBlock), kBlock, 0, s>>>(pcoords, N, lv[0].bitmap, lv[0].prefix, tl_dims(lv[0].dims), v2p, lv[0].o2n);
  }
  TL_CHECK_LAUNCH();
  return TL_OK;
}

int tl_rulebook_compact(const int32_t* table, int64_t n, int32_t* compact, tl_stream_t stream) {
  if (!table || !compact || n <= 0) return TL_ERR_ARG;
  k_table_compact<<<tl_grid(n, kBlock), kBlock, 0, tl_s(stream)>>>(table, n, compact);
  TL_CHECK_LAUNCH();
  return TL_OK;
}

}
```

Baseline: 256.9 Mpoints/s.

## Build only the rulebook forms each conv kernel needs via a dry dispatch pass

Adds a query mode to conv dispatch that records which kernel family and table form (row, column, packed, scatter, blocked) each launch would use. A dry pre-pass over the network collects those needs, so only the required neighbour tables (row nbr, compact column, packed or row inverse maps) are allocated and written. It also skips filling the all-ones input tensor when the chosen first-layer kernel never reads it. This cuts rulebook construction writes and memory traffic, at the cost of an extra host-side dry pass and more complex argument validation.

```diff
diff --git a/include/treelearn_hip.h b/include/treelearn_hip.h
--- a/include/treelearn_hip.h
+++ b/include/treelearn_hip.h
@@ -124,6 +124,14 @@
 int64_t tl_conv_red_parts(int64_t n_out);
 
 int tl_conv_fwd(const tl_conv_args* args, tl_stream_t stream);
+
+#define TL_FORM_NONE 0
+#define TL_FORM_ROW 1
+#define TL_FORM_COLUMN 2
+#define TL_FORM_SCATTER 4
+#define TL_FORM_PACKED 8
+#define TL_FORM_BLOCKED 16
+int tl_conv_query(const tl_conv_args* args, int32_t* family, int32_t* form);
 
 int tl_pack_weight(const float* w_ref, int Cout, int K, int Cin, void* w_packed, int dtype, tl_stream_t stream);
 int64_t tl_pack_weight_x3_bytes(int Cout, int K, int Cin);
diff --git a/treelearn_amd/_hip.py b/treelearn_amd/_hip.py
--- a/treelearn_amd/_hip.py
+++ b/treelearn_amd/_hip.py
@@ -9,6 +9,7 @@
 TL_F32, TL_BF16, TL_F16 = 0, 1, 2
 TL_OK, TL_ERR_ARG, TL_ERR_UNSUPPORTED = 0, -1, -3
 TL_EPI_NONE, TL_EPI_STATS, TL_EPI_BN_BWD = 0, 1, 2
+TL_FORM_NONE, TL_FORM_ROW, TL_FORM_COLUMN, TL_FORM_SCATTER, TL_FORM_PACKED, TL_FORM_BLOCKED = 0, 1, 2, 4, 8, 16
 _c = ctypes
 _vp, _i64, _i32, _f32 = _c.c_void_p, _c.c_int64, _c.c_int32, _c.c_float
 
@@ -114,6 +115,7 @@
     "tl_blk_ws_words": (_i64, [_I4]),
     "tl_blk_build": (_i32, [_vp, _vp, _I4, _i64, _c.POINTER(Blk), _vp, _i32, _vp]),
     "tl_conv_fwd": (_i32, [_c.POINTER(ConvArgs), _vp]),
+    "tl_conv_query": (_i32, [_c.POINTER(ConvArgs), _c.POINTER(_i32), _c.POINTER(_i32)]),
     "tl_conv_red_parts": (_i64, [_i64]),
     "tl_exec_create": (_vp, []),
     "tl_exec_destroy": (None, [_vp]),
diff --git a/treelearn_amd/csrc/tl_common.h b/treelearn_amd/csrc/tl_common.h
--- a/treelearn_amd/csrc/tl_common.h
+++ b/treelearn_amd/csrc/tl_common.h
@@ -56,4 +56,5 @@
   return (int)(pf[w] + __popcll(word & (bit - 1)));
 }
 
+bool tl_conv_family_reads_no_operand(int family);
 bool tl_conv_one_hot_direct_enabled(int64_t n_out);
diff --git a/treelearn_amd/csrc/tl_conv.hip b/treelearn_amd/csrc/tl_conv.hip
--- a/treelearn_amd/csrc/tl_conv.hip
+++ b/treelearn_amd/csrc/tl_conv.hip
@@ -169,6 +169,7 @@
 template <int NB>
 int launch_mfma_f32(const ConvP& p, hipStream_t s) {
   const size_t lds = (size_t)p.K * TM * 4 + 16 + 2 * (size_t)TM * LDA * 4 + 2 * (size_t)NB * 32 * LDA * 4;
+  TL_SITE(p, TL_FAM_MFMA_F32, tl_form_table(p));
   static TlAttrOnce attr_once;
   if (!tl_lds_attr(attr_once, reinterpret_cast<const void*>(&k_conv_mfma_f32<NB>), 160 * 1024)) return TL_ERR_LAUNCH;
   k_conv_mfma_f32<NB><<<p.nblk, 256, lds, s>>>(p);
@@ -343,6 +344,7 @@
 static int g_blk = 1;
 static int g_up = 1;
 
+bool tl_conv_family_reads_no_operand(int family) { return family == TL_FAM_ONES27; }
 bool tl_conv_one_hot_direct_enabled(int64_t n_out) { return g_direct && g_direct_oh && n_out > g_small_rows; }
 
 extern "C" {
@@ -365,10 +367,13 @@
   return TL_ERR_ARG;
 }
 
-int tl_conv_fwd(const tl_conv_args* a, tl_stream_t stream) {
-  if (!a || !a->in || !a->weight || !a->out || a->n_out <= 0 || a->K <= 0 || a->K > 27 || a->Cin <= 0 || a->Cout <= 0) return TL_ERR_ARG;
+}
+
+static int conv_dispatch(const tl_conv_args* a, hipStream_t s, ConvSel* sel) {
+  if (!a || (!a->in && !a->in_all_ones) || !a->weight || !a->out || a->n_out <= 0 || a->K <= 0 || a->K > 27 || a->Cin <= 0 || a->Cout <= 0) return TL_ERR_ARG;
   const bool has_blk = a->blk_unit && a->blk_counter && a->blk_halo && a->blk_lrb && a->K == 27;
-  if (!a->table && a->K != 1 && !has_blk && !(a->in_all_ones && a->blk_pmask)) return TL_ERR_ARG;
+  if (!a->table && a->K != 1 && !has_blk && !(a->in_all_ones && a->blk_pmask) && !(a->K == 27 && a->table_compact) && !(a->table_one_hot == 1 && a->table_scatter))
+    return TL_ERR_ARG;
   if ((a->in_scale == nullptr) != (a->in_shift == nullptr)) return TL_ERR_ARG;
   if ((a->out_scale == nullptr) != (a->out_shift == nullptr)) return TL_ERR_ARG;
   if (a->dtype != TL_F32 && a->dtype != TL_BF16 && a->dtype != TL_F16) return TL_ERR_ARG;
@@ -383,6 +388,7 @@
   const auto L_blk = f16 ? tl_launch_conv_blk_f16 : tl_launch_conv_blk;
   const auto L_up = f16 ? tl_launch_conv_up_f16 : tl_launch_conv_up;
   ConvP p;
+  p.sel = sel; p.scatter = a->table_scatter;
   p.in = a->in; p.in_ld = a->in_ld; p.w = a->weight; p.w_frag = a->weight_frag;
   p.w_x3 = (a->dtype == TL_F32 && a->Cin % 32 == 0 && ((uintptr_t)a->weight_x3) % 16 == 0) ? a->weight_x3 : nullptr; p.table = a->table; p.ctab = (a->K == 27) ? a->table_compact : nullptr; p.n_out = a->n_out; p.n_in = a->n_in;
   p.K = a->K; p.Cin = a->Cin; p.Cout = a->Cout; p.in_scale = a->in_scale; p.in_shift = a->in_shift;
@@ -392,7 +398,7 @@
   p.out3 = a->out3; p.out3_ld = a->out3_ld; p.out3_scale = a->out3_scale; p.out3_shift = a->out3_shift; p.out3_relu = a->out3_relu;
   if ((a->out2_scale == nullptr) != (a->out2_shift == nullptr) || (a->out3_scale == nullptr) != (a->out3_shift == nullptr)) return TL_ERR_ARG;
   p.nblk = (int)tl_cdiv(a->n_out, TM);
-  p.one_hot = a->table != nullptr ? a->table_one_hot : 0;
+  p.one_hot = (a->table != nullptr || (a->table_one_hot == 1 && a->table_scatter)) ? a->table_one_hot : 0;
   p.blk_unit = has_blk ? a->blk_unit : nullptr; p.blk_counter = a->blk_counter; p.blk_halo = a->blk_halo; p.blk_lrb = a->blk_lrb;
   p.blk_pmask = a->K == 27 ? a->blk_pmask : nullptr;
   p.epi_mode = a->epi_mode; p.red_part = a->red_part; p.red_nparts = a->red_nparts; p.bn_x = a->bn_x; p.bn_x_ld = a->bn_x_ld;
@@ -408,7 +414,6 @@
     }
     if (a->red_nparts) *a->red_nparts = 0;
   }
-  hipStream_t s = tl_s(stream);
   if (p.one_hot == 2) {
     const bool shape = a->K == 8 && a->Cin == 64 && a->Cout == 32 && !train && !a->in_scale && !a->in_relu && g_direct && g_direct_oh;
     if (!shape || !(dt == TL_BF16 || (dt == TL_F32 && p.w_x3))) return TL_ERR_UNSUPPORTED;
@@ -421,6 +426,7 @@
     const int rc = L_ones27(p, dt, s);
     if (rc != TL_ERR_UNSUPPORTED) return rc;
   }
+  if (!a->in) return TL_ERR_ARG;
   if (has_blk && dt == TL_BF16 && g_blk && vec_ok && out_vec && (!a->residual || (a->res_ld % 8 == 0 && ((uintptr_t)a->residual) % 16 == 0)) &&
       (!a->out_scale || (((uintptr_t)a->out_scale) % 4 == 0 && ((uintptr_t)a->out_shift) % 4 == 0)) && (!a->in_relu || a->in_scale)) {
     const int rc = L_blk(p, s);
@@ -430,7 +436,7 @@
     const int rc = tl_launch_conv_blk_x3(p, s);
     if (rc != TL_ERR_UNSUPPORTED) return rc;
   }
-  if (!a->table && a->K != 1) return TL_ERR_UNSUPPORTED;
+  if (!a->table && a->K != 1 && !p.ctab && !(p.one_hot == 1 && p.scatter)) return TL_ERR_UNSUPPORTED;
   if (a->table_scatter && p.one_hot && g_up && !train && dt == TL_BF16 && vec_ok && out_vec &&
       (!a->out_scale || (((uintptr_t)a->out_scale) % 16 == 0 && ((uintptr_t)a->out_shift) % 16 == 0))) {
     const int rc = L_up(p, a->table_scatter, s);
@@ -520,10 +526,24 @@
     if (rc != TL_ERR_UNSUPPORTED) return rc;
   }
   const unsigned g = tl_grid(a->n_out * a->Cout, 256);
+  TL_SITE(p, TL_FAM_GENERIC, tl_form_table(p));
   if (dt == TL_F32) k_conv_generic<float><<<g, 256, 0, s>>>(p);
   else k_conv_generic<__hip_bfloat16><<<g, 256, 0, s>>>(p);
   TL_CHECK_LAUNCH();
   return TL_OK;
+}
+
+extern "C" {
+
+int tl_conv_fwd(const tl_conv_args* a, tl_stream_t stream) { return conv_dispatch(a, tl_s(stream), nullptr); }
+
+int tl_conv_query(const tl_conv_args* a, int32_t* family, int32_t* form) {
+  if (!family || !form) return TL_ERR_ARG;
+  ConvSel sel;
+  sel.probe = true;
+  const int rc = conv_dispatch(a, nullptr, &sel);
+  *family = sel.family; *form = sel.form;
+  return rc;
 }
 
 int64_t tl_conv_red_parts(int64_t n_out) {
diff --git a/treelearn_amd/csrc/tl_conv_bf16.hip b/treelearn_amd/csrc/tl_conv_bf16.hip
--- a/treelearn_amd/csrc/tl_conv_bf16.hip
+++ b/treelearn_amd/csrc/tl_conv_bf16.hip
@@ -230,6 +230,7 @@
   const size_t epi_b = 4 * (size_t)32 * (NB * 32 + 4) * 4;
   const size_t lds = (size_t)p.K * TM * 4 + 128 + (size_t)p.Cin * 8 + (main_b > epi_b ? main_b : epi_b);
   if (lds > 160 * 1024) return TL_ERR_UNSUPPORTED;
+  TL_SITE(p, TL_FAM_BF16, tl_form_table(p));
   static TlAttrOnce attr_once;
   if (!tl_lds_attr(attr_once, reinterpret_cast<const void*>(&k_conv_bf16<NB, U, D, BUF>), 160 * 1024)) return TL_ERR_LAUNCH;
   k_conv_bf16<NB, U, D, BUF><<<p.nblk, 256, lds, s>>>(p);
diff --git a/treelearn_amd/csrc/tl_conv_blk.hip b/treelearn_amd/csrc/tl_conv_blk.hip
--- a/treelearn_amd/csrc/tl_conv_blk.hip
+++ b/treelearn_amd/csrc/tl_conv_blk.hip
@@ -394,6 +394,7 @@
 int launch_blk(const ConvP& p, hipStream_t s) {
   constexpr size_t lds = (size_t)WS_B + AFF_B + (size_t)W * STAGE_B + (TR ? (size_t)W * 2 * 32 * 8 : 0);
   static_assert(lds <= 160 * 1024, "LDS budget");
+  TL_SITE(p, TL_FAM_BLK, TL_FORM_BLOCKED);
   static TlAttrOnce attr_once;
   if (!tl_lds_attr(attr_once, reinterpret_cast<const void*>(&k_conv_blk<W, RES, NV, TR, PRO>), 160 * 1024)) return TL_ERR_LAUNCH;
   k_conv_blk<W, RES, NV, TR, PRO><<<256, W * 64, lds, s>>>(p);
diff --git a/treelearn_amd/csrc/tl_conv_blk_x3.hip b/treelearn_amd/csrc/tl_conv_blk_x3.hip
--- a/treelearn_amd/csrc/tl_conv_blk_x3.hip
+++ b/treelearn_amd/csrc/tl_conv_blk_x3.hip
@@ -340,6 +340,7 @@
 int launch_x3(const ConvP& p, const X3P& xp, hipStream_t s) {
   constexpr size_t lds = (size_t)WS_B + AFF_B + (size_t)W * STAGE_B;
   static_assert(lds <= 160 * 1024, "LDS budget");
+  TL_SITE(p, TL_FAM_BLK_X3, TL_FORM_BLOCKED);
   static TlAttrOnce attr_once;
   if (!tl_lds_attr(attr_once, reinterpret_cast<const void*>(&k_conv_blk_x3<W, RES, NV>), 160 * 1024)) return TL_ERR_LAUNCH;
   k_conv_blk_x3<W, RES, NV><<<256, W * 64, lds, s>>>(p, xp);
diff --git a/treelearn_amd/csrc/tl_conv_direct.hip b/treelearn_amd/csrc/tl_conv_direct.hip
--- a/treelearn_amd/csrc/tl_conv_direct.hip
+++ b/treelearn_amd/csrc/tl_conv_direct.hip
@@ -438,6 +438,7 @@
   constexpr int UB = BF16 ? 64 : 128;
   const size_t lds = (size_t)K * UN * NB * 32 * UB + (size_t)WAVES * 32 * (NB * 32 + 4) * 4 + (TR ? (size_t)WAVES * 2 * NB * 32 * 8 : 0);
   if (lds > 160 * 1024) return TL_ERR_UNSUPPORTED;
+  TL_SITE(p, TL_FAM_DIRECT, (K == 27 && CT) ? TL_FORM_COLUMN : tl_form_table(p));
   static TlAttrOnce attr_once;
   if (!tl_lds_attr(attr_once, reinterpret_cast<const void*>(&k_conv_direct<BF16, K, NB, UN, G, WAVES, CT, TR, OH, X3>), 160 * 1024)) return TL_ERR_LAUNCH;
   const int ntiles = (int)tl_cdiv(p.n_out, 32);
@@ -494,6 +495,7 @@
 
 int tl_launch_conv_ones27(const ConvP& p, int dtype, hipStream_t s) {
   if (p.K != 27 || p.Cout != 32 || (!p.ctab && !p.blk_pmask) || p.Cin <= 0 || p.Cin > 64 || p.in_scale || p.in_relu || p.epi_mode != TL_EPI_NONE) return TL_ERR_UNSUPPORTED;
+  TL_SITE(p, TL_FAM_ONES27, p.blk_pmask ? TL_FORM_BLOCKED : TL_FORM_COLUMN);
   if (dtype == TL_BF16) k_conv_ones27<true><<<tl_grid(p.n_out * 4, 256), 256, 0, s>>>(p);
   else k_conv_ones27<false><<<tl_grid(p.n_out * 4, 256), 256, 0, s>>>(p);
   return hipGetLastError() == hipSuccess ? TL_OK : TL_ERR_LAUNCH;
@@ -504,10 +506,11 @@
   if (p.in_scale || p.in_relu) return TL_ERR_UNSUPPORTED;
   if (p.one_hot == 2 && !(p.K == 8 && p.Cin == 64 && p.Cout == 32 && p.epi_mode == TL_EPI_NONE && (dtype == TL_BF16 || p.w_x3))) return TL_ERR_UNSUPPORTED;
   const int eb = dtype == TL_BF16 ? 2 : 4;
-  if (dtype == TL_BF16 && p.Cin == 4 && p.Cout == 32 && p.K <= 28 && p.table && p.in_ld % 4 == 0 && (int64_t)p.n_in * p.in_ld * 2 < 0xFFFF0000ll) {
+  if (dtype == TL_BF16 && p.Cin == 4 && p.Cout == 32 && p.K <= 28 && (p.table || (p.ctab && p.K == 27)) && p.in_ld % 4 == 0 && (int64_t)p.n_in * p.in_ld * 2 < 0xFFFF0000ll) {
     const int ntiles = (int)tl_cdiv(p.n_out, 32);
     int grid = (int)tl_cdiv(ntiles, 8);
     if (grid > 2048) grid = 2048;
+    TL_SITE(p, TL_FAM_IN4, tl_form_ctab(p));
     if (p.epi_mode != TL_EPI_NONE) {
       if (p.ctab && p.K == 27) k_conv_in4<8, true, true><<<grid, 512, 0, s>>>(p, ntiles);
       else k_conv_in4<8, false, true><<<grid, 512, 0, s>>>(p, ntiles);
diff --git a/treelearn_amd/csrc/tl_conv_internal.h b/treelearn_amd/csrc/tl_conv_internal.h
--- a/treelearn_amd/csrc/tl_conv_internal.h
+++ b/treelearn_amd/csrc/tl_conv_internal.h
@@ -20,6 +20,12 @@
 typedef float f32x4 __attribute__((ext_vector_type(4)));
 typedef uint32_t u32x4 __attribute__((ext_vector_type(4)));
 typedef short s16x8 __attribute__((ext_vector_type(8)));
+
+enum {
+  TL_FAM_ONES27 = 1, TL_FAM_DIRECT, TL_FAM_IN4, TL_FAM_BLK, TL_FAM_BLK_X3, TL_FAM_UP, TL_FAM_TINYCIN, TL_FAM_SMALL, TL_FAM_STREAM, TL_FAM_STREAMQ,
+  TL_FAM_MFMA_F32, TL_FAM_BF16, TL_FAM_TINYCOUT, TL_FAM_GENERIC
+};
+struct ConvSel { int family = 0, form = 0; bool probe = false; };
 
 struct ConvP {
   const void* in; int64_t in_ld;
@@ -44,7 +50,31 @@
   const float* bn_mean; const float* bn_rstd; const float* bn_scale; const float* bn_shift; int bn_relu;
   int one_hot;
   const int32_t* blk_unit; const int32_t* blk_counter; const int32_t* blk_halo; const uint32_t* blk_lrb; const int32_t* blk_pmask;
+  const int32_t* scatter;
+  ConvSel* sel;
 };
+
+static inline int tl_form_table(const ConvP& p) { return p.table ? (p.one_hot == 2 ? TL_FORM_PACKED : TL_FORM_ROW) : (p.K == 1 ? TL_FORM_NONE : TL_FORM_ROW); }
+static inline int tl_form_ctab(const ConvP& p) { return (p.K == 27 && p.ctab) ? TL_FORM_COLUMN : tl_form_table(p); }
+static inline bool tl_form_offered(const ConvP& p, int form) {
+  switch (form) {
+    case TL_FORM_ROW: return p.table && p.one_hot != 2;
+    case TL_FORM_PACKED: return p.table && p.one_hot == 2;
+    case TL_FORM_COLUMN: return p.ctab != nullptr;
+    case TL_FORM_SCATTER: return p.scatter != nullptr;
+    case TL_FORM_BLOCKED: return p.blk_pmask != nullptr || p.blk_unit != nullptr;
+    default: return true;
+  }
+}
+#define TL_SITE(p, fam, frm)                                            \
+  do {                                                                  \
+    const int form_ = (frm);                                            \
+    if (!tl_form_offered((p), form_)) return TL_ERR_ARG;                \
+    if ((p).sel) {                                                      \
+      (p).sel->family = (fam); (p).sel->form = form_;                   \
+      if ((p).sel->probe) return TL_OK;                                 \
+    }                                                                   \
+  } while (0)
 
 static __device__ __forceinline__ float ld_elem(const float* p) { return *p; }
 static __device__ __forceinline__ float ld_elem(const __hip_bfloat16* p) { return h16_lo((uint32_t)*reinterpret_cast<const uint16_t*>(p)); }
diff --git a/treelearn_amd/csrc/tl_conv_small.hip b/treelearn_amd/csrc/tl_conv_small.hip
--- a/treelearn_amd/csrc/tl_conv_small.hip
+++ b/treelearn_amd/csrc/tl_conv_small.hip
@@ -188,6 +188,8 @@
 int launch_tiny(const ConvP& p, hipStream_t s) {
   const size_t lds = (size_t)p.K * p.Cin * p.Cout * 4;
   const unsigned g = tl_grid(p.n_out * (p.Cout / 8), 256);
+  if (p.Cin < 1 || p.Cin > 8) return TL_ERR_UNSUPPORTED;
+  TL_SITE(p, TL_FAM_TINYCIN, tl_form_table(p));
   switch (p.Cin) {
     case 1: k_conv_tinycin<T, 1><<<g, 256, lds, s>>>(p); break;
     case 2: k_conv_tinycin<T, 2><<<g, 256, lds, s>>>(p); break;
@@ -207,6 +209,7 @@
 int g_small_mode = 0;
 
 int tl_launch_conv_small(const ConvP& p, int dtype, hipStream_t s) {
+  TL_SITE(p, TL_FAM_SMALL, tl_form_table(p));
   const int nrt = (int)tl_cdiv(p.n_out, 32);
   const bool eight = g_small_mode == 2 || (g_small_mode == 0 && nrt * (p.Cout / 32) <= 512 && p.K * (p.Cin / 32) >= 32);
   const int cbt = p.Cout / 32;
diff --git a/treelearn_amd/csrc/tl_conv_stream.hip b/treelearn_amd/csrc/tl_conv_stream.hip
--- a/treelearn_amd/csrc/tl_conv_stream.hip
+++ b/treelearn_amd/csrc/tl_conv_stream.hip
@@ -203,6 +203,7 @@
   const size_t wt = 2 * (size_t)NB * 32 * (UN * 32 * EB + 16), ep = (size_t)WAVES * 32 * 36 * 4;
   const size_t lds = wt > ep ? wt : ep;
   if (lds > 160 * 1024) return TL_ERR_UNSUPPORTED;
+  TL_SITE(p, TL_FAM_STREAM, tl_form_ctab(p));
   static TlAttrOnce attr_once;
   if (!tl_lds_attr(attr_once, reinterpret_cast<const void*>(&k_conv_stream<BF16, K, NB, UN, DA, RB, OCC, OH, X3>), 160 * 1024)) return TL_ERR_LAUNCH;
   p.nblk = (int)tl_cdiv(p.n_out, WAVES * 32 * RB);
diff --git a/treelearn_amd/csrc/tl_conv_streamq.hip b/treelearn_amd/csrc/tl_conv_streamq.hip
--- a/treelearn_amd/csrc/tl_conv_streamq.hip
+++ b/treelearn_amd/csrc/tl_conv_streamq.hip
@@ -258,6 +258,7 @@
   const size_t wt = 2 * (size_t)NB * 32 * (PN * 128 + 16) + (size_t)W * K * 32 * RB * 4, ep = (size_t)W * 32 * 36 * 4;
   const size_t lds = wt > ep ? wt : ep;
   if (lds > 160 * 1024) return TL_ERR_UNSUPPORTED;
+  TL_SITE(p, TL_FAM_STREAMQ, tl_form_ctab(p));
   static TlAttrOnce attr_once;
   if (!tl_lds_attr(attr_once, reinterpret_cast<const void*>(&k_conv_streamq<K, NB, PN, DA, W, RB, OCC, SP, X3, UL>), 160 * 1024)) return TL_ERR_LAUNCH;
   p.nblk = (int)tl_cdiv(p.n_out, W * 32 * RB);
diff --git a/treelearn_amd/csrc/tl_conv_up.hip b/treelearn_amd/csrc/tl_conv_up.hip
--- a/treelearn_amd/csrc/tl_conv_up.hip
+++ b/treelearn_amd/csrc/tl_conv_up.hip
@@ -88,6 +88,7 @@
 int launch_up(const ConvP& p, const int32_t* child, hipStream_t s) {
   const size_t lds = (size_t)8 * NBO * NBI * 2 * 1024 + (size_t)WAVES * 32 * 36 * 4;
   static_assert(8 * NBO * NBI * 2 * 1024 + WAVES * 32 * 36 * 4 <= 160 * 1024, "weights + epilogue tiles must fit the LDS");
+  TL_SITE(p, TL_FAM_UP, TL_FORM_SCATTER);
   static TlAttrOnce attr_once;
   if (!tl_lds_attr(attr_once, reinterpret_cast<const void*>(&k_conv_up<NBI, NBO, WAVES>), 160 * 1024)) return TL_ERR_LAUNCH;
   const int ntiles = (int)tl_cdiv(p.n_in, 32);
diff --git a/treelearn_amd/csrc/tl_exec.hip b/treelearn_amd/csrc/tl_exec.hip
--- a/treelearn_amd/csrc/tl_exec.hip
+++ b/treelearn_amd/csrc/tl_exec.hip
@@ -30,7 +30,10 @@
   const int32_t* scatter = nullptr;
   bool blk = false;
   int one_hot = 0;
+  int kind = -1, level = 0;
 };
+
+const int32_t* const kOffered = reinterpret_cast<const int32_t*>(uintptr_t(256));
 
 struct LevelG {
   int32_t dims[4];
@@ -64,6 +67,10 @@
   int nl;
   LevelG lv[TL_MAX_LEVELS];
   bool blocked = false;
+  bool needs_pass = false, packed0 = false;
+  int need_subm[TL_MAX_LEVELS] = {}, need_up[TL_MAX_LEVELS] = {};
+  int last_family = 0;
+  bool skip_ones = false;
   int64_t g0 = 0;
   int64_t o_unit = -1, o_counter = -1, o_halo = -1, o_lrb = -1, o_pmask = -1, o_nn = -1;
 
@@ -86,13 +93,17 @@
 
   Table subm(int li) const {
     Table t;
+    t.kind = 0; t.level = li;
     if (li == 0 && blocked) { t.blk = true; return t; }
+    if (needs_pass) { t.table = kOffered; t.compact = lv[li].n >= kCompactMinRows ? kOffered : nullptr; return t; }
     t.table = gw(lv[li].nbr); t.compact = gw(lv[li].ct);
     return t;
   }
-  Table down(int li) const { Table t; t.table = gw(lv[li].child); return t; }
+  Table down(int li) const { Table t; t.kind = 1; t.level = li; t.table = needs_pass ? kOffered : gw(lv[li].child); return t; }
   Table up(int li) const {
     Table t;
+    t.kind = 2; t.level = li;
+    if (needs_pass) { t.scatter = t.table = kOffered; t.one_hot = (li == 0 && packed0) ? 2 : 1; return t; }
     t.scatter = gw(lv[li].child);
     if (lv[li].invp >= 0) { t.table = gw(lv[li].invp); t.one_hot = 2; }
     else { t.table = gw(lv[li].inv); t.one_hot = 1; }
@@ -104,11 +115,13 @@
     for (int i = 0; i < nviews; ++i) outs[i] = views[i].dst ? *views[i].dst : alloc(n_out, w.Cout);
     if (rc != TL_OK) return;
     ++launches;
-    if (ar.dry) return;
+    if (ar.dry && !needs_pass) return;
     tl_conv_args c{};
-    c.in = ar.at(x.off); c.in_ld = x.ld; c.weight = w.w; c.weight_frag = w.frag; c.weight_x3 = w.x3;
+    c.in = x.off < 0 ? nullptr : ar.at(x.off); c.in_ld = x.ld; c.weight = w.w; c.weight_frag = w.frag; c.weight_x3 = w.x3;
     c.table = tb.table; c.table_compact = tb.compact; c.table_one_hot = tb.one_hot; c.table_scatter = tb.scatter;
-    if (tb.blk) {
+    if (tb.blk && needs_pass) {
+      c.blk_unit = c.blk_counter = c.blk_halo = c.blk_pmask = kOffered; c.blk_lrb = reinterpret_cast<const uint32_t*>(kOffered);
+    } else if (tb.blk) {
       c.blk_unit = gw(o_unit); c.blk_counter = gw(o_counter); c.blk_halo = gw(o_halo);
       c.blk_lrb = reinterpret_cast<const uint32_t*>(gw(o_lrb)); c.blk_pmask = gw(o_pmask);
     }
@@ -119,6 +132,15 @@
     c.out = ar.at(outs[0].off); c.out_ld = outs[0].ld; c.out_scale = views[0].aff.scale; c.out_shift = views[0].aff.shift; c.out_relu = views[0].relu;
     if (nviews > 1) { c.out2 = ar.at(outs[1].off); c.out2_ld = outs[1].ld; c.out2_scale = views[1].aff.scale; c.out2_shift = views[1].aff.shift; c.out2_relu = views[1].relu; }
     if (nviews > 2) { c.out3 = ar.at(outs[2].off); c.out3_ld = outs[2].ld; c.out3_scale = views[2].aff.scale; c.out3_shift = views[2].aff.shift; c.out3_relu = views[2].relu; }
+    if (needs_pass) {
+      int32_t family = 0, form = 0;
+      const int r = tl_conv_query(&c, &family, &form);
+      if (r != TL_OK) { rc = r; return; }
+      if (tb.kind == 0) need_subm[tb.level] |= form;
+      if (tb.kind == 2) need_up[tb.level] |= form;
+      last_family = family;
+      return;
+    }
     const bool prof = ex->profile;
     if (prof) {
       hipEvent_t e0 = nullptr, e1 = nullptr;
@@ -230,7 +252,9 @@
   void network() {
     const int64_t n1 = lv[0].n;
     const bool feats = net->use_coords || net->use_feats;
-    Ten ones = alloc(n1, net->in_channels);
+    Ten ones;
+    ones.n = n1; ones.C = ones.ld = net->in_channels;
+    if (!skip_ones) ones = alloc(n1, net->in_channels);
     if (feats) {
       const int64_t ws_bytes = 4 * n1 * net->max_points_per_voxel, o_ws = ar.take(ws_bytes);
       if (!ar.dry) {
@@ -239,7 +263,7 @@
         if (r != TL_OK) rc = r;
       }
       ar.give(o_ws, ws_bytes);
-    } else if (!ar.dry) {
+    } else if (!ar.dry && !skip_ones) {
       hipError_t e;
       if (net->dtype == TL_F32) e = hipMemsetD32Async((hipDeviceptr_t)ar.at(ones.off), 0x3F800000, n1 * net->in_channels, s);
       else e = hipMemsetD16Async((hipDeviceptr_t)ar.at(ones.off), net->dtype == TL_BF16 ? 0x3F80 : 0x3C00, n1 * net->in_channels, s);
@@ -250,13 +274,15 @@
     if (blocked) {
       const ViewReq v = RAW();
       Table tin = subm(0);
-      if (feats) { tin = Table{}; tin.table = gw(o_nn); }
+      if (feats) { tin = Table{}; tin.table = needs_pass ? kOffered : gw(o_nn); }
       conv(0, 4, ones, net->w_in, tin, n1, &v, 1, xs, nullptr, {nullptr, nullptr}, 0, feats ? 0 : 1);
+      if (needs_pass) skip_ones = !feats && tl_conv_family_reads_no_operand(last_family);
       release(ones);
       l1_staged(xs[0], &out, 1, &x);
     } else {
       const ViewReq v[2] = {RAW(), ACT(net->u[0].blocks[0].bn0)};
       conv(0, 4, ones, net->w_in, subm(0), n1, v, 2, xs, nullptr, {nullptr, nullptr}, 0, feats ? 0 : 1);
+      if (needs_pass) skip_ones = !feats && tl_conv_family_reads_no_operand(last_family);
       release(ones);
       ublock(0, xs[0], xs[1], &out, 1, &x);
     }
@@ -445,14 +471,26 @@
   R.blocked = net->blocked && (net->dtype != TL_F32 || x3_l1) && u0.C == 32 && u0.deeper && u0.tail[0].w1_half[0].w && u0.tail[0].w1_half[1].w &&
               n1 >= kBlkMinRows && n1 <= kBlkMaxRows;
   a->blocked_used = R.blocked;
+  R.packed0 = nl > 1 && net->u[0].C == 32 && net->u[1].C == 64 && (net->dtype != TL_F32 || net->u[0].wu.x3) && tl_conv_one_hot_direct_enabled(n1);
+  {
+    Run D = R;
+    D.needs_pass = true; D.ar.dry = true; D.ar.base = reinterpret_cast<char*>(uintptr_t(256));
+    D.network();
+    if (D.rc != TL_OK) return D.rc;
+    R.skip_ones = D.skip_ones;
+    for (int l = 0; l < nl; ++l) { R.need_subm[l] = D.need_subm[l]; R.need_up[l] = D.need_up[l]; }
+  }
   int64_t cur = 0;
   auto take = [&](int64_t words) { const int64_t o = cur; cur += al64(words); return o; };
   R.o_v2p = take(2 * N);
   for (int l = 0; l < nl; ++l) {
     LevelG& v = R.lv[l];
     const bool skip = R.blocked && l == 0;
-    if (!skip) { v.coords = take(4 * v.n); v.nbr = take(27 * v.n); }
-    if (!skip && v.n >= kCompactMinRows) v.ct = take(10 * v.n);
+    if (!skip) {
+      v.coords = take(4 * v.n);
+      if (R.need_subm[l] & TL_FORM_ROW) v.nbr = take(27 * v.n);
+      if (R.need_subm[l] & TL_FORM_COLUMN) v.ct = take(10 * v.n);
+    }
     if (l + 1 < nl) v.child = take(8 * R.lv[l + 1].n);
   }
   int64_t o_o2n = -1, o_perm = -1, o_cnew = -1, o_bws = -1;
@@ -462,11 +500,10 @@
     R.o_lrb = take(9 * n1); R.o_pmask = take(n1); o_bws = take(nbws);
     if (feats) R.o_nn = take(27 * n1);
   }
-  const bool packed0 = nl > 1 && net->u[0].C == 32 && net->u[1].C == 64 && (net->dtype != TL_F32 || net->u[0].wu.x3) && tl_conv_one_hot_direct_enabled(n1);
   const int64_t o_m1 = cur;
   for (int l = 0; l + 1 < nl; ++l) {
-    if (l == 0 && packed0) R.lv[l].invp = take(R.lv[l].n);
-    else R.lv[l].inv = take(8 * R.lv[l].n);
+    if (R.need_up[l] & TL_FORM_PACKED) R.lv[l].invp = take(R.lv[l].n);
+    if (R.need_up[l] & TL_FORM_ROW) R.lv[l].inv = take(8 * R.lv[l].n);
   }
   const int64_t o_m1_end = cur;
   R.g0 = R.ar.take(4 * cur);
diff --git a/treelearn_amd/csrc/tl_linear_small.hip b/treelearn_amd/csrc/tl_linear_small.hip
--- a/treelearn_amd/csrc/tl_linear_small.hip
+++ b/treelearn_amd/csrc/tl_linear_small.hip
@@ -89,6 +89,7 @@
   if (p.in_ld % 8 || ((uintptr_t)p.in) % 16 || ((uintptr_t)p.w) % eb) return TL_ERR_UNSUPPORTED;
   const unsigned g = tl_grid(p.n_out, 256);
   const size_t lds = (size_t)p.Cout * p.Cin * 4;
+  TL_SITE(p, TL_FAM_TINYCOUT, TL_FORM_NONE);
 #define TL_TC(CO_)                                                                     \
   case CO_:                                                                            \
     if (dtype == TL_BF16) k_conv_tinycout<true, CO_><<<g, 256, lds, s>>>(p);           \
diff --git a/treelearn_amd/csrc/tl_voxel.hip b/treelearn_amd/csrc/tl_voxel.hip
--- a/treelearn_amd/csrc/tl_voxel.hip
+++ b/treelearn_amd/csrc/tl_voxel.hip
@@ -509,9 +509,11 @@
           if (bit < 63) { if (word & (2ull << bit)) r2 = (int)(base + __popcll(word & ((below << 1) | 1ull))); }
           else if (z + 1 < d.Z) r2 = tl_rank_at(bm, pf, wc, z + 1);
         }
-        nbr[(int64_t)(tap0 + 0) * M + i] = r0;
-        nbr[(int64_t)(tap0 + 1) * M + i] = r1;
-        nbr[(int64_t)(tap0 + 2) * M + i] = r2;
+        if (nbr) {
+          nbr[(int64_t)(tap0 + 0) * M + i] = r0;
+          nbr[(int64_t)(tap0 + 1) * M + i] = r1;
+          nbr[(int64_t)(tap0 + 2) * M + i] = r2;
+        }
         if (compact) {
           compact[(int64_t)(tap0 / 3) * M + i] = r0 >= 0 ? r0 : (r1 >= 0 ? r1 : r2);
           cmask |= ((r0 >= 0 ? 1u : 0u) | (r1 >= 0 ? 2u : 0u) | (r2 >= 0 ? 4u : 0u)) << tap0;
@@ -770,7 +772,7 @@
 
 int tl_rulebook_subm(const int32_t* coords, int64_t M, const uint64_t* bitmap, const uint32_t* prefix, const int32_t dims[4],
                      int32_t* nbr, int32_t* compact, tl_stream_t stream) {
-  if (!coords || !bitmap || !prefix || !dims || !nbr || M <= 0) return TL_ERR_ARG;
+  if (!coords || !bitmap || !prefix || !dims || (!nbr && !compact) || M <= 0) return TL_ERR_ARG;
   k_rulebook_subm<<<tl_grid(M, kBlock), kBlock, 0, tl_s(stream)>>>(coords, M, bitmap, prefix, tl_dims(dims), nbr, compact);
   TL_CHECK_LAUNCH();
   return TL_OK;
@@ -866,10 +868,10 @@
   if (!lv || num_levels < 1 || num_levels > kPyrMaxLevels) return TL_ERR_ARG;
   for (int l = 0; l < num_levels; ++l) {
     if (!lv[l].bitmap || !lv[l].prefix || lv[l].n <= 0) return TL_ERR_ARG;
-    if ((!lv[l].coords || !lv[l].nbr) && !lv[l].o2n) return TL_ERR_ARG;
-    if (lv[l].nbr && !lv[l].coords) return TL_ERR_ARG;
+    if ((!lv[l].coords || (!lv[l].nbr && !lv[l].compact)) && !lv[l].o2n) return TL_ERR_ARG;
+    if ((lv[l].nbr || lv[l].compact) && !lv[l].coords) return TL_ERR_ARG;
     if (l > 0 && !lv[l].coords) return TL_ERR_ARG;
-    if (l + 1 < num_levels && (!lv[l].child || (!lv[l].inv && !lv[l].inv_packed))) return TL_ERR_ARG;
+    if (l + 1 < num_levels && !lv[l].child) return TL_ERR_ARG;
     if (lv[l].inv_packed && lv[l].n >= (1ll << 28)) return TL_ERR_ARG;
   }
   hipStream_t s = tl_s(stream);
@@ -882,14 +884,14 @@
   }
   int small = num_levels;
   for (int l = num_levels - 1; l >= 1; --l) {
-    if (tl_nwords(tl_dims(lv[l].dims)) <= kPyrSmallWords && lv[l].n <= 64 * kPyrSmallWords && !lv[l].compact && !lv[l].o2n && !lv[l - 1].o2n &&
+    if (tl_nwords(tl_dims(lv[l].dims)) <= kPyrSmallWords && lv[l].n <= 64 * kPyrSmallWords && !lv[l].compact && lv[l].nbr && !lv[l].o2n && !lv[l - 1].o2n &&
         !lv[l].inv_packed && !lv[l - 1].inv_packed) small = l; else break;
   }
   if (num_levels - small < 2) small = num_levels;
   for (int l = 0; l < small; ++l) {
     const TlDims d = tl_dims(lv[l].dims);
     if (lv[l].coords) k_expand_coords<<<tl_grid(tl_nwords(d), kBlock), kBlock, 0, s>>>(lv[l].bitmap, lv[l].prefix, d, lv[l].coords);
-    if (lv[l].nbr) k_rulebook_subm<<<tl_grid(lv[l].n, kBlock), kBlock, 0, s>>>(lv[l].coords, lv[l].n, lv[l].bitmap, lv[l].prefix, d, lv[l].nbr, lv[l].compact);
+    if (lv[l].nbr || lv[l].compact) k_rulebook_subm<<<tl_grid(lv[l].n, kBlock), kBlock, 0, s>>>(lv[l].coords, lv[l].n, lv[l].bitmap, lv[l].prefix, d, lv[l].nbr, lv[l].compact);
   }
   LevelPack p;
   p.nl = num_levels - small;
```

Result: no change. 258.2 Mpoints/s (median of 5 runs) (+0.5%).
